# MingXiangL/AttentionShift

Measured on AMD Instinct MI355X. Metric: images/sec (1024^2, ViT-B) hot path: backbone attention fwd + attention-shift pseudo-labels, higher is better.
Workload: dtype bf16

## Files before the change

attentionshift_amd/_lib.py:

```python
import ctypes
import os

_HERE = os.path.dirname(os.path.abspath(__file__))
LIB_PATH = os.path.join(_HERE, "libattnshift_hip.so")

AS_F32, AS_BF16 = 0, 1

_c_void_p, _c_int, _c_float, _c_size_t = ctypes.c_void_p, ctypes.c_int, ctypes.c_float, ctypes.c_size_t
_c_double = ctypes.c_double

SIGNATURES = {
    "as_version": (_c_int, []),
    "as_last_error": (ctypes.c_char_p, []),
    "as_npad": (_c_int, [_c_int]),
    "as_linear_fwd": (_c_int, [_c_void_p] * 4 + [_c_int] * 5 + [_c_void_p]),
    "as_linear_small_fwd": (_c_int, [_c_void_p, _c_int, _c_void_p, _c_void_p, _c_void_p] + [_c_int] * 5 + [_c_void_p]),
    "as_linear_sk_workspace_bytes": (_c_size_t, [_c_int] * 3),
    "as_linear_sk_fwd": (_c_int, [_c_void_p] * 4 + [_c_int] * 5 + [_c_void_p, _c_size_t, _c_void_p]),
    "as_linear_gelu_fwd": (_c_int, [_c_void_p] * 5 + [_c_int] * 4 + [_c_void_p]),
    "as_linear_dgelu_fwd": (_c_int, [_c_void_p] * 4 + [_c_int] * 4 + [_c_void_p]),
    "as_deconv2x2_fwd": (_c_int, [_c_void_p] * 4 + [_c_int] * 6 + [_c_void_p]),
    "as_qkv_fwd": (_c_int, [_c_void_p] * 6 + [_c_int] * 5 + [_c_void_p]),
    "as_sdpa_fwd_workspace_bytes": (_c_size_t, [_c_int] * 4),
    "as_sdpa_fwd": (_c_int, [_c_void_p] * 6 + [_c_size_t] + [_c_int] * 4 + [_c_void_p]),
    "as_sdpa_bwd_workspace_bytes": (_c_size_t, [_c_int] * 4),
    "as_sdpa_bwd": (_c_int, [_c_void_p] * 8 + [_c_size_t] + [_c_int] * 4 + [_c_void_p]),
    "as_attn_bwd_workspace_bytes": (_c_size_t, [_c_int] * 5),
    "as_attn_bwd": (_c_int, [_c_void_p] * 15 + [_c_size_t] + [_c_int] * 5 + [_c_void_p]),
    "as_window_attn_fwd": (_c_int, [_c_void_p] * 5 + [_c_int] * 8 + [_c_void_p]),
    "as_add_layernorm_bwd_workspace_bytes": (_c_size_t, [_c_int] * 2),
    "as_add_layernorm_bwd": (_c_int, [_c_void_p] * 4 + [ctypes.c_float] + [_c_void_p] * 5 + [_c_size_t] + [_c_int] * 3 + [_c_void_p]),
    "as_add_layernorm": (_c_int, [_c_void_p] * 4 + [ctypes.c_float] + [_c_void_p] * 2 + [_c_int] * 3 + [_c_void_p]),
    "as_add_layernorm_scaled": (_c_int, [_c_void_p] * 4 + [ctypes.c_float] + [_c_void_p] * 2 + [_c_int] * 3 + [_c_void_p, _c_int, _c_void_p]),
    "as_add_layernorm_bwd_scaled": (_c_int, [_c_void_p] * 4 + [ctypes.c_float] + [_c_void_p] * 5 + [_c_size_t] + [_c_int] * 3
                                    + [_c_void_p, _c_int, _c_void_p]),
    "as_linear_splitk_workspace_bytes": (ctypes.c_size_t, [_c_int] * 3),
    "as_linear_splitk_fwd": (_c_int, [_c_void_p] * 3 + [_c_int] * 5 + [_c_void_p, ctypes.c_size_t, _c_void_p]),
    "as_linear_bwd_workspace_bytes": (ctypes.c_size_t, [_c_int] * 3),
    "as_linear_bwd": (_c_int, [_c_void_p] * 6 + [_c_int] * 5 + [_c_void_p, ctypes.c_size_t, _c_void_p]),
    "as_linear_bwd_dgelu": (_c_int, [_c_void_p] * 7 + [_c_int] * 5 + [_c_void_p, ctypes.c_size_t, _c_void_p]),
    "as_assemble_tokens": (_c_int, [_c_void_p] * 3 + [_c_int] * 5 + [_c_void_p]),
    "as_maxpool_nhwc": (_c_int, [_c_void_p] * 2 + [_c_int] * 5 + [ctypes.c_longlong, _c_void_p]),
    "as_mask_count": (_c_int, [_c_void_p] * 2 + [_c_int] * 2 + [_c_void_p]),
    "as_window_attn_bwd_workspace_bytes": (_c_size_t, [_c_int] * 5),
    "as_window_attn_bwd": (_c_int, [_c_void_p] * 8 + [_c_size_t] + [_c_int] * 8 + [_c_void_p]),
    "as_attn_fwd": (_c_int, [_c_void_p] * 12 + [_c_size_t] + [_c_int] * 5 + [_c_void_p]),
    "as_attn_mean_rows": (_c_int, [_c_void_p] * 4 + [_c_int] * 6 + [_c_void_p]),
    "as_rollout_rfrag_bytes": (_c_size_t, [_c_int] * 3),
    "as_rollout_pack": (_c_int, [_c_void_p] * 2 + [_c_int] * 4 + [_c_void_p]),
    "as_rollout_top": (_c_int, [_c_void_p] * 5 + [_c_int] * 5 + [_c_void_p]),
    "as_rollout_step_workspace_bytes": (_c_size_t, [_c_int] * 3),
    "as_rollout_step": (_c_int, [_c_void_p] * 8 + [_c_size_t] + [_c_int] * 5 + [_c_void_p]),
    "as_ccl_2d": (_c_int, [_c_void_p] * 2 + [_c_int] * 3 + [_c_void_p]),
    "as_cam_boxes_workspace_bytes": (_c_size_t, [_c_int] * 4),
    "as_cam_boxes": (_c_int, [_c_void_p] * 2 + [_c_float] * 2 + [_c_int] * 4 + [_c_void_p] * 5 + [_c_size_t, _c_void_p]),
    "as_cam_sample_masks_workspace_bytes": (_c_size_t, [_c_int] * 4),
    "as_cam_sample_masks": (_c_int, [_c_void_p] * 3 + [_c_int] * 4 + [_c_float] * 2 + [_c_void_p] * 3 + [_c_size_t, _c_void_p]),
    "as_mask_candidates_workspace_bytes": (_c_size_t, [_c_int] * 3),
    "as_mask_candidates": (_c_int, [_c_void_p] * 3 + [_c_float] * 3 + [_c_int] + [_c_void_p] * 5 + [_c_size_t]
                           + [_c_int] * 3 + [_c_void_p]),
    "as_part_select": (_c_int, [_c_void_p] * 7 + [_c_int] * 5 + [_c_void_p] * 8 + [_c_void_p]),
    "as_part_stats": (_c_int, [_c_void_p] * 3 + [_c_float] + [_c_void_p] * 4 + [_c_int] * 3 + [_c_void_p]),
    "as_filter_parts": (_c_int, [_c_void_p] * 2 + [_c_float] * 2 + [_c_void_p] + [_c_int] * 3 + [_c_void_p]),
    "as_draw_distinct": (_c_int, [_c_void_p, _c_int, _c_int] + [_c_void_p] * 5 + [_c_int] * 3 + [_c_void_p]),
    "as_mt_sample_ranks": (_c_int, [_c_void_p] * 4 + [_c_int] * 2 + [_c_void_p]),
    "as_mt_perm_ranks": (_c_int, [_c_void_p] * 4 + [_c_int] * 2 + [_c_void_p]),
    "as_small_attn_fwd": (_c_int, [_c_void_p] * 3 + [_c_int] * 5 + [_c_void_p]),
    "as_small_attn_bwd_workspace_bytes": (_c_size_t, [_c_int] * 3),
    "as_small_attn_bwd": (_c_int, [_c_void_p] * 6 + [_c_size_t] + [_c_int] * 5 + [_c_void_p]),
    "as_roi_align_fwd": (_c_int, [_c_void_p] * 3 + [_c_int] * 6 + [_c_float] + [_c_int] * 2 + [_c_void_p]),
    "as_roi_align_bwd": (_c_int, [_c_void_p] * 3 + [_c_int] * 6 + [_c_float] + [_c_int] * 2 + [_c_void_p]),
    "as_chamfer_2d_fwd": (_c_int, [_c_void_p] * 6 + [_c_int] * 3 + [_c_void_p]),
    "as_chamfer_2d_bwd": (_c_int, [_c_void_p] * 8 + [_c_int] * 3 + [_c_void_p]),
    "as_merge_plan": (_c_int, [_c_void_p] * 4 + [_c_int] * 2 + [_c_void_p]),
    "as_semantic_prestage": (_c_int, [_c_void_p, _c_float] + [_c_int] * 5 + [_c_void_p] * 4),
    "as_cosine_shift_workspace_bytes": (_c_size_t, [_c_int] * 6),
    "as_cosine_shift": (_c_int, [_c_void_p] * 5 + [_c_double] * 2 + [_c_int] + [_c_void_p] * 4 + [_c_size_t]
                        + [_c_int] * 6 + [_c_void_p]),
    "as_cosine_shift_strided": (_c_int, [_c_void_p, ctypes.c_longlong] + [_c_void_p] * 4 + [_c_double] * 2 + [_c_int] + [_c_void_p] * 4
                                + [_c_size_t] + [_c_int] * 6 + [_c_void_p]),
    "as_refine_similarity_workspace_bytes": (_c_size_t, [_c_int] * 3),
    "as_refine_similarity": (_c_int, [_c_void_p] * 3 + [_c_int] * 3 + [_c_float, _c_int] + [_c_void_p] * 3
                             + [_c_size_t] + [_c_int] * 3 + [_c_void_p]),
    "as_instance_maps_workspace_bytes": (_c_size_t, [_c_int] * 2),
    "as_crop_threshold_erode_workspace_bytes": (_c_size_t, [_c_int] * 3),
    "as_crop_threshold_erode": (_c_int, [_c_void_p] * 2 + [_c_float, _c_int, _c_int] + [_c_void_p] * 3 + [_c_size_t]
                                + [_c_int] * 3 + [_c_void_p]),
    "as_rank_select_workspace_bytes": (_c_size_t, [_c_int] * 2),
    "as_rank_select": (_c_int, [_c_void_p] * 4 + [_c_size_t] + [_c_int] * 3 + [_c_void_p]),
    "as_rank_select_xy": (_c_int, [_c_void_p] * 4 + [_c_size_t] + [_c_int] * 5 + [_c_void_p]),
    "as_merge_parts": (_c_int, [_c_void_p] * 2 + [_c_float] + [_c_void_p] * 3 + [_c_int] * 4 + [_c_void_p]),
    "as_select_median_boxes": (_c_int, [_c_void_p] * 2 + [_c_int] * 2 + [_c_void_p] * 8 + [_c_int, _c_void_p]),
    "as_rank_draw_xy": (_c_int, [_c_void_p, _c_int] + [_c_void_p] * 4 + [_c_int, _c_int, ctypes.c_int64, _c_int, _c_void_p, _c_size_t]
                        + [_c_int] * 5 + [_c_void_p]),
    "as_instance_maps": (_c_int, [_c_void_p] * 2 + [_c_int] * 6 + [_c_void_p] * 3 + [_c_size_t, _c_void_p]),
    "as_nms_workspace_bytes": (_c_size_t, [_c_int]),
    "as_nms": (_c_int, [_c_void_p, _c_int, _c_float, _c_int] + [_c_void_p] * 3 + [_c_size_t, _c_void_p]),
    "as_paste_masks": (_c_int, [_c_void_p] * 4 + [_c_int] * 8 + [_c_float, _c_void_p]),
    "as_rle_tile": (_c_int, [_c_void_p] * 2),
    "as_rle_workspace_bytes": (_c_size_t, [_c_int] * 3),
    "as_rle_count": (_c_int, [_c_void_p] + [_c_int] * 3 + [_c_void_p] * 2 + [_c_size_t, _c_void_p]),
    "as_rle_encode": (_c_int, [_c_void_p] + [_c_int] * 3 + [_c_void_p] * 2 + [_c_size_t, _c_void_p, _c_size_t, _c_void_p, _c_size_t,
                               _c_void_p, _c_void_p]),
    "as_rpn_candidates_workspace_bytes": (_c_size_t, [_c_int] * 2),
    "as_rpn_candidates": (_c_int, [_c_void_p] + [_c_int] * 3 + [_c_void_p] * 2 + [_c_int, _c_float, _c_void_p, _c_float, _c_int]
                          + [_c_void_p] * 7 + [_c_size_t, _c_void_p]),
    "as_rpn_assign_workspace_bytes": (_c_size_t, [_c_int] * 3),
    "as_rpn_assign": (_c_int, [_c_void_p] + [_c_int] * 3 + [_c_void_p] * 3 + [_c_int] * 2 + [_c_void_p] + [_c_float] * 3
                      + [_c_int] * 2 + [_c_void_p] * 4 + [_c_size_t, _c_void_p]),
    "as_rpn_sample": (_c_int, [_c_int] * 4 + [_c_void_p] * 4 + [_c_size_t, _c_void_p, _c_void_p]),
    "as_rpn_targets": (_c_int, [_c_void_p] + [_c_int] * 3 + [_c_void_p] * 3 + [_c_int] + [_c_void_p] * 2 + [_c_int] * 2
                       + [_c_void_p] * 3 + [_c_void_p]),
}


class RpnLevel(ctypes.Structure):
    _fields_ = [("cls", _c_void_p), ("reg", _c_void_p), ("H", _c_int), ("W", _c_int), ("stride_x", _c_int), ("stride_y", _c_int)]

_lib = None


class AttnShiftError(RuntimeError):
    pass


def load():
    global _lib
    if _lib is not None:
        return _lib
    if not os.path.exists(LIB_PATH):
        raise AttnShiftError(
            f"{LIB_PATH} is missing: build it with `python -m attentionshift_amd.csrc.build` "
            "(hipcc --offload-arch=gfx950).  There is no CPU fallback for the hot path.")
    lib = ctypes.CDLL(LIB_PATH)
    for name, (res, args) in SIGNATURES.items():
        fn = getattr(lib, name)
        fn.restype, fn.argtypes = res, args
    _lib = lib
    return lib


def check(rc, what):
    if rc != 0:
        msg = load().as_last_error()
        raise AttnShiftError(f"{what} failed (rc={rc}): {msg.decode() if msg else ''}")
```

attentionshift_amd/backbone.py:

```python
import math
import os

import torch
import torch.nn as nn
import torch.nn.functional as F

from . import ops
from .registry import BACKBONES


def trunc_normal_(tensor, std=0.02):
    return nn.init.trunc_normal_(tensor, std=std, a=-2 * std, b=2 * std)


class Mlp(nn.Module):
    def __init__(self, dim, hidden):
        super().__init__()
        self.fc1 = nn.Linear(dim, hidden)
        self.fc2 = nn.Linear(hidden, dim)


class Attention(nn.Module):
    def __init__(self, dim, num_heads, qkv_bias):
        super().__init__()
        self.num_heads = num_heads
        self.qkv = nn.Linear(dim, dim * 3, bias=qkv_bias)
        self.proj = nn.Linear(dim, dim)


class Block(nn.Module):

    def __init__(self, dim, num_heads, mlp_ratio, qkv_bias, eps):
        super().__init__()
        self.norm1 = nn.LayerNorm(dim, eps=eps)
        self.attn = Attention(dim, num_heads, qkv_bias)
        self.norm2 = nn.LayerNorm(dim, eps=eps)
        self.mlp = Mlp(dim, int(dim * mlp_ratio))


class PatchEmbed(nn.Module):
    def __init__(self, img_size, patch_size, in_chans, embed_dim):
        super().__init__()
        if isinstance(img_size, int):
            img_size = [img_size, img_size]
        self.num_patches = (img_size[0] // patch_size) * (img_size[1] // patch_size)
        self.patch_size = patch_size
        self.proj = nn.Conv2d(in_chans, embed_dim, kernel_size=patch_size, stride=patch_size)


class MLP(nn.Module):

    def __init__(self, input_dim, hidden_dim, output_dim, num_layers):
        super().__init__()
        self.num_layers = num_layers
        h = [hidden_dim] * (num_layers - 1)
        self.layers = nn.ModuleList(nn.Linear(n, k) for n, k in zip([input_dim] + h, h + [output_dim]))

    def forward(self, x):
        for i, layer in enumerate(self.layers):
            x = F.relu(layer(x)) if i < self.num_layers - 1 else layer(x)
        return x


class DeferredFPN:

    def __init__(self, backbone, features, taps):
        self._bb, self._features, self._taps = backbone, list(features), list(taps)
        self._out, self._event, self._joined = None, None, False

    def launch(self):
        if self._out is not None:
            return self
        bb = self._bb
        main = torch.cuda.current_stream()
        if bb._fpn_stream is None:
            bb._fpn_stream = torch.cuda.Stream()
        side = bb._fpn_stream
        side.wait_stream(main)
        with torch.cuda.stream(side):
            for t in self._features + self._taps:
                t.record_stream(side)
            self._out = tuple(bb._fpn(i, self._features[i], self._taps[i]) for i in range(len(self._features)))
            self._event = side.record_event()
        return self

    def result(self):
        self.launch()
        if not self._joined:
            main = torch.cuda.current_stream()
            main.wait_event(self._event)
            for t in self._out:
                t.record_stream(main)
            self._joined = True
            self._features, self._taps = [], []
        return self._out

    def __len__(self):
        return len(self._features) if self._out is None else len(self._out)

    def __iter__(self):
        return iter(self.result())

    def __getitem__(self, i):
        return self.result()[i]


@BACKBONES.register_module()
class VisionTransformerDet(nn.Module):
    def __init__(self, img_size, patch_size, embed_dim, in_chans=3, with_fpn=True, frozen_stages=-1,
                 out_indices=(3, 5, 7, 11), use_checkpoint=False, learnable_pos_embed=True, last_feat=False,
                 recompute_last_feat=False, point_tokens_num=100, num_classes=20, return_attention=False,
                 with_point_head=True, depth=12, num_heads=12, mlp_ratio=4., qkv_bias=False, qk_scale=None,
                 drop_rate=0., attn_drop_rate=0., drop_path_rate=0., norm_eps=1e-6, init_values=0,
                 compute_dtype=torch.bfloat16, **unused):
        super().__init__()
        assert not with_fpn or patch_size in (8, 16)
        assert not recompute_last_feat or last_feat
        if qk_scale is not None or attn_drop_rate or drop_rate or init_values:
            raise NotImplementedError("qk_scale / dropout / layer-scale are unused by every reference config")
        if embed_dim != num_heads * ops.HEAD_DIM:
            raise NotImplementedError(f"head dim must be {ops.HEAD_DIM}")
        self.embed_dim = self.num_features = embed_dim
        self.patch_size, self.depth, self.num_heads = patch_size, depth, num_heads
        self.last_feat, self.recompute_last_feat = last_feat, recompute_last_feat
        self.with_fpn, self.frozen_stages = with_fpn, frozen_stages
        self.out_indices = tuple(out_indices)
        self.use_checkpoint = use_checkpoint
        self.drop_path_rate = drop_path_rate
        self.return_attention = return_attention
        self.point_tokens_num = point_tokens_num
        self.with_point_head = with_point_head
        self.compute_dtype = compute_dtype
        self.defer_fpn = bool(unused.pop("defer_fpn", False))
        self._fpn_stream = None
        self._point_pack = None
        self.point_head_stream = bool(unused.pop("point_head_stream", False))
        self._point_stream = None

        self.patch_embed = PatchEmbed(img_size, patch_size, in_chans, embed_dim)
        n_patches = self.patch_embed.num_patches
        self.cls_token = nn.Parameter(torch.zeros(1, 1, embed_dim))
        self.pos_embed = nn.Parameter(torch.zeros(1, n_patches + 1, embed_dim), requires_grad=learnable_pos_embed)
        self.blocks = nn.ModuleList(Block(embed_dim, num_heads, mlp_ratio, qkv_bias, norm_eps) for _ in range(depth))
        if with_fpn and patch_size == 16:
            self.fpn1 = nn.Sequential(nn.ConvTranspose2d(embed_dim, embed_dim, 2, 2), nn.BatchNorm2d(embed_dim), nn.GELU(),
                                      nn.ConvTranspose2d(embed_dim, embed_dim, 2, 2))
            self.fpn2 = nn.Sequential(nn.ConvTranspose2d(embed_dim, embed_dim, 2, 2))
            self.fpn3 = nn.Identity()
            self.fpn4 = nn.MaxPool2d(2, 2)
        elif with_fpn and patch_size == 8:
            self.fpn1 = nn.Sequential(nn.ConvTranspose2d(embed_dim, embed_dim, 2, 2))
            self.fpn2 = nn.Identity()
            self.fpn3 = nn.Sequential(nn.MaxPool2d(2, 2))
            self.fpn4 = nn.Sequential(nn.MaxPool2d(4, 4))
        self.point_token = nn.Parameter(torch.zeros(1, point_tokens_num, embed_dim))
        self.point_pos_embed = nn.Parameter(torch.zeros(1, point_tokens_num, embed_dim))
        if with_point_head:
            self.class_embed = MLP(embed_dim, embed_dim, num_classes, 3)
            self.bbox_embed = MLP(embed_dim, embed_dim, 2, 3)
        trunc_normal_(self.pos_embed)
        trunc_normal_(self.cls_token)
        trunc_normal_(self.point_token)
        trunc_normal_(self.point_pos_embed)
        self.apply(self._init_weights)
        self._wcache = {}

    @staticmethod
    def _init_weights(m):
        if isinstance(m, nn.Linear):
            trunc_normal_(m.weight)
            if m.bias is not None:
                nn.init.constant_(m.bias, 0)
        elif isinstance(m, nn.LayerNorm):
            nn.init.constant_(m.bias, 0)
            nn.init.constant_(m.weight, 1.0)

    def init_weights(self, pretrained=None):
        if pretrained is not None and not isinstance(pretrained, str):
            raise TypeError("pretrained must be a str or None")
        self.apply(self._init_weights)
        if isinstance(pretrained, str):
            import os
            if os.path.isfile(pretrained):
                from .checkpoint import load_checkpoint
                load_checkpoint(self, pretrained, strict=False)
            else:
                print(f"checkpoint path {pretrained} is invalid, we skip it and initialize net randomly")
        self.invalidate_cache()

    def train(self, mode=True):
        super().train(mode)
        self._freeze_stages()
        return self

    def _freeze_stages(self):
        if self.frozen_stages >= 0:
            self.patch_embed.eval()
            for p in self.patch_embed.parameters():
                p.requires_grad = False
            self.cls_token.requires_grad = False
            self.pos_embed.requires_grad = False
        for i in range(1, self.frozen_stages + 1):
            m = self.blocks[i - 1]
            m.eval()
            for p in m.parameters():
                p.requires_grad = False

    def invalidate_cache(self):
        self._wcache = {}

    def _w(self, p):
        if p.dtype == self.compute_dtype:
            return p
        if torch.is_grad_enabled() and p.requires_grad:
            return p.to(self.compute_dtype)
        key = id(p)
        hit = self._wcache.get(key)
        if hit is None or hit[0] != p._version or hit[1].device != p.device:
            hit = (p._version, p.detach().to(self.compute_dtype).contiguous())
            self._wcache[key] = hit
        return hit[1]

    def _derived(self, p, tag, fn):
        if torch.is_grad_enabled() and p.requires_grad:
            return fn(p).to(self.compute_dtype).contiguous()
        key = (id(p), tag)
        hit = self._wcache.get(key)
        if hit is None or hit[0] != p._version or hit[1].device != p.device:
            hit = (p._version, fn(p.detach()).to(self.compute_dtype).contiguous())
            self._wcache[key] = hit
        return hit[1]

    def _deconv2x2(self, x_nhwc, conv, bn=None, act="none"):
        B, h, w, cin = x_nhwc.shape
        cout = conv.weight.shape[1]
        srcs = [conv.weight, conv.bias] + ([bn.weight, bn.bias, bn.running_mean, bn.running_var] if bn is not None else [])
        stamp = tuple(-1 if t is None else t._version for t in srcs) + (x_nhwc.device,)
        key = (id(conv), "deconv")
        hit = self._wcache.get(key)
        if hit is None or hit[0] != stamp:
            with torch.no_grad():
                wmat = conv.weight.detach().float().permute(2, 3, 1, 0).reshape(4 * cout, cin)
                bias = torch.zeros(cout, device=wmat.device) if conv.bias is None else conv.bias.detach().float()
                if bn is not None:
                    scale = bn.weight.detach().float() * torch.rsqrt(bn.running_var.float() + bn.eps)
                    wmat = wmat * scale.repeat(4)[:, None]
                    bias = (bias - bn.running_mean.float()) * scale + bn.bias.detach().float()
                hit = (stamp, wmat.to(self.compute_dtype).contiguous(), bias.repeat(4).contiguous())
            self._wcache[key] = hit
        _, wmat, bias4 = hit
        if x_nhwc.is_cuda and self.compute_dtype == torch.bfloat16 and cin % 32 == 0 and cout % 8 == 0:
            return ops.deconv2x2(x_nhwc.contiguous(), wmat, bias4, act=act)
        y = ops.linear(x_nhwc.reshape(B * h * w, cin), wmat, bias4, act=act)
        return y.reshape(B, h, w, 2, 2, cout).permute(0, 1, 3, 2, 4, 5).reshape(B, 2 * h, 2 * w, cout)

    def _deconv2x2_train(self, x_nhwc, conv):
        B, h, w, cin = x_nhwc.shape
        cout = conv.weight.shape[1]
        cd = self.compute_dtype
        from .autograd import linear_in
        wmat = conv.weight.permute(2, 3, 1, 0).reshape(4 * cout, cin)
        bias = None if conv.bias is None else conv.bias.repeat(4)
        y = linear_in(x_nhwc.reshape(B * h * w, cin), wmat, bias, cd)
        return y.reshape(B, h, w, 2, 2, cout).permute(0, 1, 3, 2, 4, 5).reshape(B, 2 * h, 2 * w, cout)

    def _fpn_train(self, i, feat_nchw, tok):
        B, D, hp, wp = feat_nchw.shape
        op = [self.fpn1, self.fpn2, self.fpn3, self.fpn4][i]
        if isinstance(op, nn.Sequential) and isinstance(op[0], nn.ConvTranspose2d):
            y = self._deconv2x2_train(tok.to(self.compute_dtype).reshape(B, hp, wp, D), op[0]).permute(0, 3, 1, 2)
            if len(op) == 4:
                y = op[2](op[1](y.float())).to(self.compute_dtype)
                y = self._deconv2x2_train(y.permute(0, 2, 3, 1), op[3]).permute(0, 3, 1, 2)
            return y
        return op(feat_nchw)

    def _fpn(self, i, feat_nchw, tok):
        B, D, hp, wp = feat_nchw.shape
        ops_ = [self.fpn1, self.fpn2, self.fpn3, self.fpn4]
        op = ops_[i]
        if isinstance(op, nn.Sequential) and isinstance(op[0], nn.ConvTranspose2d):
            x0 = tok.to(self.compute_dtype).reshape(B, hp, wp, D)
            if len(op) == 4:
                bn = op[1]
                if isinstance(bn, nn.modules.batchnorm._BatchNorm) and not bn.training and bn.running_mean is not None \
                        and isinstance(op[2], nn.GELU) and getattr(op[2], "approximate", "none") == "none":
                    y = self._deconv2x2(x0, op[0], bn=bn, act="gelu")
                else:
                    y = self._deconv2x2(x0, op[0]).permute(0, 3, 1, 2)
                    y = op[2](op[1](y.float())).to(self.compute_dtype).permute(0, 2, 3, 1)
                return self._deconv2x2(y, op[3]).permute(0, 3, 1, 2)
            return self._deconv2x2(x0, op[0]).permute(0, 3, 1, 2)
        pool = op[0] if isinstance(op, nn.Sequential) and len(op) == 1 else op
        if isinstance(pool, nn.MaxPool2d) and tok.is_cuda and tok.dtype == torch.float32 and tok.stride()[1:] == (D, 1):
            k = pool.kernel_size if isinstance(pool.kernel_size, int) else pool.kernel_size[0]
            s_ = pool.stride if isinstance(pool.stride, int) else pool.stride[0]
            if k == s_ and pool.padding in (0, (0, 0)) and not pool.ceil_mode and hp % k == 0 and wp % k == 0 and D % 4 == 0:
                return ops.maxpool_nhwc(tok.reshape(B, hp, wp, D), k).permute(0, 3, 1, 2)
        return op(feat_nchw)

    def _point_head_packable(self, x):
        ls = list(self.class_embed.layers) + list(self.bbox_embed.layers)
        return (len(self.class_embed.layers) == 3 and len(self.bbox_embed.layers) == 3 and hasattr(torch, "_addmm_activation")
                and all(l.weight.dtype == x.dtype and l.bias is not None for l in ls)
                and self.class_embed.layers[0].in_features == self.bbox_embed.layers[0].in_features)

    def _point_head_packed(self, x):
        c, b = self.class_embed.layers, self.bbox_embed.layers
        key = tuple((t.data_ptr(), t._version) for t in (c[0].weight, c[0].bias, b[0].weight, b[0].bias))
        pk = self._point_pack
        if pk is None or pk["key"] != key:
            with torch.no_grad():
                w1 = torch.cat((c[0].weight, b[0].weight)).contiguous()
                pk = dict(key=key, w1=w1, w1t=w1.t().contiguous(), b1=torch.cat((c[0].bias, b[0].bias)))
            self._point_pack = pk
        B, T, D = x.shape
        hc = c[0].out_features
        x2 = x.reshape(B * T, D)
        if ops.linear_small_applies(x2, pk["w1"]) and hc % 16 == 0 and hc >= 64:
            h1 = ops.linear_small(x2, pk["w1"], pk["b1"], act="relu")
            h2c = ops.linear_small(h1[:, :hc], c[1].weight, c[1].bias, act="relu")
            h2b = ops.linear_small(h1[:, hc:], b[1].weight, b[1].bias, act="relu")
            cls = ops.linear_small(h2c, c[2].weight, c[2].bias).reshape(B, T, -1)
            reg = ops.linear_small(h2b, b[2].weight, b[2].bias, act="sigmoid").reshape(B, T, -1)
            return cls, reg
        h1 = torch._addmm_activation(pk["b1"], x2, pk["w1t"])
        h2c = torch._addmm_activation(c[1].bias, h1[:, :hc], c[1].weight.t())
        h2b = torch._addmm_activation(b[1].bias, h1[:, hc:], b[1].weight.t())
        cls = torch.addmm(c[2].bias, h2c, c[2].weight.t()).reshape(B, T, -1)
        reg = torch.addmm(b[2].bias, h2b, b[2].weight.t()).reshape(B, T, -1).sigmoid()
        return cls, reg

    def interpolate_pos_encoding(self, n_patch_tokens, w, h):
        n0 = self.pos_embed.shape[1] - 1
        if n_patch_tokens == n0 and w == h:
            return self.pos_embed
        dim = self.pos_embed.shape[-1]
        w0, h0 = w // self.patch_size + 0.1, h // self.patch_size + 0.1
        s = int(math.sqrt(n0))
        grid = self.pos_embed[:, 1:].reshape(1, s, s, dim).permute(0, 3, 1, 2)
        grid = F.interpolate(grid, scale_factor=(w0 / math.sqrt(n0), h0 / math.sqrt(n0)), mode="bicubic")
        assert int(w0) == grid.shape[-2] and int(h0) == grid.shape[-1]
        return torch.cat((self.pos_embed[:, :1], grid.permute(0, 2, 3, 1).reshape(1, -1, dim)), dim=1)

    def prepare_tokens(self, img):
        B, C, w, h = img.shape
        ps = self.patch_size
        hp, wp = w // ps, h // ps
        patches = torch.empty(B, hp, wp, C, ps, ps, device=img.device, dtype=self.compute_dtype)
        patches.copy_(img.reshape(B, C, hp, ps, wp, ps).permute(0, 2, 4, 1, 3, 5))
        wmat = self._derived(self.patch_embed.proj.weight, "patch", lambda t: t.reshape(self.embed_dim, -1))
        emb = ops.linear(patches.view(B, hp * wp, C * ps * ps), wmat, self.patch_embed.proj.bias.float())
        return ops.assemble_tokens(emb, self._token_table(hp * wp, w, h))

    def _token_table(self, Np, w, h):
        srcs = (self.pos_embed, self.cls_token, self.point_token, self.point_pos_embed)
        stamp = tuple(t._version for t in srcs) + (Np, w, h, self.pos_embed.device)
        hit = self._wcache.get("token_table")
        if hit is None or hit[0] != stamp:
            with torch.no_grad():
                pos = self.interpolate_pos_encoding(Np, w, h)
                table = torch.cat((self.cls_token + pos[:, :1], pos[:, 1:], self.point_token + self.point_pos_embed), dim=1)
            hit = (stamp, table[0].float().contiguous())
            self._wcache["token_table"] = hit
        return hit[1]

    def _block(self, blk, x, delta, keep_state, need_x, on_full=None, full_out=None, x_out=None):
        cd = self.compute_dtype
        x, y = ops.add_layernorm(x, delta, blk.norm1.weight, blk.norm1.bias, blk.norm1.eps, cd,
                                 x_out=full_out if delta is not None else None)
        if on_full is not None:
            on_full(x)
        a, st = ops.attention_fwd(y, self._w(blk.attn.qkv.weight),
                                  None if blk.attn.qkv.bias is None else blk.attn.qkv.bias.float(),
                                  self._w(blk.attn.proj.weight), blk.attn.proj.bias.float(), self.num_heads,
                                  keep_state=keep_state)
        x, z = ops.add_layernorm(x, a, blk.norm2.weight, blk.norm2.bias, blk.norm2.eps, cd)
        z = ops.linear(z, self._w(blk.mlp.fc1.weight), blk.mlp.fc1.bias.float(), act="gelu")
        z = ops.linear(z, self._w(blk.mlp.fc2.weight), blk.mlp.fc2.bias.float())
        if need_x:
            x, _ = ops.add_layernorm(x, z, None, None, 0.0, cd, want_y=False, x_out=x_out)
            z = None
        return x, z, st

    def _grad_path(self):
        return torch.is_grad_enabled() and self.training and any(p.requires_grad for p in self.blocks.parameters())

    def _drop_path(self, x, i):
        rate = self.drop_path_rate * i / max(self.depth - 1, 1)
        if rate == 0.0 or not self.training:
            return x
        keep = 1.0 - rate
        mask = torch.rand(x.shape[0], 1, 1, device=x.device, dtype=x.dtype).add_(keep).floor_()
        return x / keep * mask

    def _drop_scale(self, batch, i, device):
        rate = self.drop_path_rate * i / max(self.depth - 1, 1)
        if rate == 0.0 or not self.training:
            return None
        keep = 1.0 - rate
        return torch.rand(batch, device=device, dtype=torch.float32).add_(keep).floor_().div_(keep)

    def _prepare_tokens_train(self, img):
        B, C, w, h = img.shape
        ps = self.patch_size
        hp, wp = w // ps, h // ps
        cd = self.compute_dtype
        patches = img.reshape(B, C, hp, ps, wp, ps).permute(0, 2, 4, 1, 3, 5).reshape(B, hp * wp, C * ps * ps)
        from .autograd import linear_in
        x = linear_in(patches.to(cd), self.patch_embed.proj.weight.reshape(self.embed_dim, -1), self.patch_embed.proj.bias,
                      cd).float()
        x = torch.cat((self.cls_token.expand(B, -1, -1), x), dim=1)
        x = x + self.interpolate_pos_encoding(x.shape[1] - 1, w, h)
        pt = (self.point_token + self.point_pos_embed).expand(B, -1, -1)
        return torch.cat((x, pt), dim=1)

    def _block_train(self, blk, x, delta, i, sink, delta_scale=None):
        from . import autograd as AG
        cd = self.compute_dtype
        sh = self._train_shadow
        w = lambda p: sh[id(p)] if id(p) in sh else p.to(cd)
        x, y = AG.add_layernorm(x, delta, blk.norm1.weight, blk.norm1.bias, blk.norm1.eps, cd, delta_scale)
        a = AG.attention(y, w(blk.attn.qkv.weight), None if blk.attn.qkv.bias is None else blk.attn.qkv.bias.float(),
                         w(blk.attn.proj.weight), blk.attn.proj.bias.float(), self.num_heads, sink)
        x, z = AG.add_layernorm(x, a, blk.norm2.weight, blk.norm2.bias, blk.norm2.eps, cd, self._drop_scale(x.shape[0], i, x.device))
        if AG.mlp_applies(z, w(blk.mlp.fc1.weight), w(blk.mlp.fc2.weight)):
            z = AG.mlp(z, w(blk.mlp.fc1.weight), blk.mlp.fc1.bias, w(blk.mlp.fc2.weight), blk.mlp.fc2.bias)
        elif AG.linear_applies(z, w(blk.mlp.fc1.weight)):
            z = F.gelu(AG.linear(z, w(blk.mlp.fc1.weight), blk.mlp.fc1.bias))
            z = AG.linear(z, w(blk.mlp.fc2.weight), blk.mlp.fc2.bias)
        else:
            z = F.gelu(F.linear(z, w(blk.mlp.fc1.weight), w(blk.mlp.fc1.bias)))
            z = F.linear(z, w(blk.mlp.fc2.weight), w(blk.mlp.fc2.bias))
        return x, z, self._drop_scale(x.shape[0], i, x.device)

    def forward(self, x):
        B, _, H, W = x.shape
        hp, wp = H // self.patch_size, W // self.patch_size
        T = self.point_tokens_num
        grad_path = self._grad_path()
        x = self._prepare_tokens_train(x) if grad_path else self.prepare_tokens(x)
        if self.recompute_last_feat:
            last_feat = x
        features, taps, attns = [], [], []
        store = []
        delta = None
        dscale = None
        if not grad_path:
            x = x.contiguous()

        def take_tap(xf):
            taps.append(xf[:, 1:-T])
            tap = xf[:, 1:, :][:, :-T].permute(0, 2, 1).unflatten(2, (hp, wp))
            if grad_path:
                features.append(tap if os.environ.get("AS_TAP_VIEW", "1") != "0" else tap.contiguous())
                return
            if xf.data_ptr() != tap_slot(len(features)).data_ptr():
                tap_slot(len(features)).copy_(xf)
            features.append(store[0][len(features)][:, 1:-T].unflatten(1, (hp, wp)).permute(0, 3, 1, 2))

        def tap_slot(k):
            if not store:
                store.append(torch.empty(len(self.out_indices), *x.shape, device=x.device, dtype=torch.float32))
            return store[0][k]

        tap_due = False
        nblk = len(self.blocks)
        self._train_shadow = {}
        if grad_path and self.compute_dtype != torch.float32 and not os.environ.get("AS_NO_PARAM_SHADOW"):
            from .autograd import cast_params
            from . import autograd as _AG
            lib_mlp = _AG._LIBRARY_LINEAR or self.embed_dim % 32 != 0
            ps = []
            for blk in self.blocks:
                ps += [blk.attn.qkv.weight, blk.attn.proj.weight, blk.mlp.fc1.weight, blk.mlp.fc2.weight]
                if lib_mlp:
                    ps += [blk.mlp.fc1.bias, blk.mlp.fc2.bias]
            self._train_shadow = cast_params([p for p in ps if p.dtype != self.compute_dtype], self.compute_dtype)
        for i, blk in enumerate(self.blocks):
            if grad_path:
                sink = [] if self.return_attention else None
                x, delta, dscale = self._block_train(blk, x.float() if x.dtype != torch.float32 else x, delta, i, sink, dscale)
                if i in self.out_indices or i == nblk - 1:
                    x = x + (delta if dscale is None else delta * dscale[:, None, None])
                    delta, dscale = None, None
                st = sink[0] if sink else None
                if i in self.out_indices:
                    take_tap(x)
            else:
                last_tap = i in self.out_indices and i == nblk - 1
                x, delta, st = self._block(blk, x, delta, self.return_attention, i == nblk - 1,
                                           take_tap if tap_due else None,
                                           full_out=tap_slot(len(features)) if tap_due and x.dtype == torch.float32 else None,
                                           x_out=tap_slot(len(features) + int(tap_due)) if last_tap and x.dtype == torch.float32
                                           else None)
                tap_due = i in self.out_indices and i != nblk - 1
                if i in self.out_indices and i == nblk - 1:
                    take_tap(x)
            if self.return_attention:
                attns.append(st)
            if self.last_feat and not self.recompute_last_feat and i == nblk - 1:
                last_feat = x[:, :-T]
        self._train_shadow = {}
        org_features = store[0][:, :, 1:-T].unflatten(2, (hp, wp)).permute(1, 0, 4, 2, 3) if store else None
        if org_features is None:
            org_features = torch.stack(features, dim=1)
        if self.with_fpn and grad_path:
            features = [self._fpn_train(i, features[i], taps[i]) for i in range(len(features))]
        elif self.with_fpn and self.defer_fpn and x.is_cuda:
            features = DeferredFPN(self, features, taps)
        elif self.with_fpn:
            features = [self._fpn(i, features[i], taps[i]) for i in range(len(features))]
        point_tokens = x[:, -T:]
        out = dict(org_feats=org_features, feature=features if isinstance(features, DeferredFPN) else tuple(features),
                   point_tokens=point_tokens)
        if self.with_point_head and not grad_path and point_tokens.is_cuda and self._point_head_packable(point_tokens):
            if self.point_head_stream:
                if self._point_stream is None:
                    self._point_stream = torch.cuda.Stream()
                main = torch.cuda.current_stream()
                self._point_stream.wait_stream(main)
                with torch.cuda.stream(self._point_stream):
                    cls, reg = self._point_head_packed(point_tokens)
                    out["point_head_ready"] = self._point_stream.record_event()
                for t in (point_tokens, cls, reg):
                    t.record_stream(main)
                    t.record_stream(self._point_stream)
            else:
                cls, reg = self._point_head_packed(point_tokens)
            out.update(outputs_class=cls, outputs_coord=reg)
        elif self.with_point_head:
            out.update(outputs_class=self.class_embed(point_tokens), outputs_coord=self.bbox_embed(point_tokens).sigmoid())
        if self.return_attention and self.last_feat:
            out.update(attns=attns)
        if self.last_feat:
            out.update(last_feat=last_feat)
        return out
```

attentionshift_amd/csrc/layernorm.hip:

```cpp
#include "common.h"

namespace {

template <typename T, int VPL>
__global__ __launch_bounds__(256) void add_layernorm_kernel(const float* __restrict__ x_in, const T* __restrict__ delta,
                                                            const float* __restrict__ gamma, const float* __restrict__ beta,
                                                            float* __restrict__ x_out, T* __restrict__ y_out, int M, int D,
                                                            float eps, const float* __restrict__ dscale, int rps) {
  const int row = blockIdx.x * 4 + (threadIdx.x >> 6), lane = threadIdx.x & 63;
  if (row >= M) return;
  const size_t base = (size_t)row * D;
  const float ds = dscale != nullptr ? dscale[row / rps] : 1.0f;
  float v[VPL][4];
  float s = 0.0f;
#pragma unroll
  for (int i = 0; i < VPL; ++i) {
    const int c = (i * 64 + lane) * 4;
    if (c < D) {
      const float4 a = *reinterpret_cast<const float4*>(x_in + base + c);
      v[i][0] = a.x; v[i][1] = a.y; v[i][2] = a.z; v[i][3] = a.w;
      if (delta != nullptr) {
#pragma unroll
        for (int t = 0; t < 4; ++t) v[i][t] = dscale != nullptr ? fmaf(ds, to_f32<T>(delta[base + c + t]), v[i][t])
                                                                     : v[i][t] + to_f32<T>(delta[base + c + t]);
      }
      s += (v[i][0] + v[i][1]) + (v[i][2] + v[i][3]);
    } else {
      v[i][0] = v[i][1] = v[i][2] = v[i][3] = 0.0f;
    }
  }
  const float mean = wave_sum(s) / (float)D;
  float q = 0.0f;
#pragma unroll
  for (int i = 0; i < VPL; ++i) {
    const int c = (i * 64 + lane) * 4;
    if (c < D) {
#pragma unroll
      for (int t = 0; t < 4; ++t) {
        const float d = v[i][t] - mean;
        q = fmaf(d, d, q);
      }
    }
  }
  const float rstd = rsqrtf(wave_sum(q) / (float)D + eps);
#pragma unroll
  for (int i = 0; i < VPL; ++i) {
    const int c = (i * 64 + lane) * 4;
    if (c < D) {
      if (x_out != nullptr) *reinterpret_cast<float4*>(x_out + base + c) = make_float4(v[i][0], v[i][1], v[i][2], v[i][3]);
      if (y_out != nullptr) {
        const float4 g = *reinterpret_cast<const float4*>(gamma + c);
        const float4 b = *reinterpret_cast<const float4*>(beta + c);
        const float y0 = (v[i][0] - mean) * rstd * g.x + b.x, y1 = (v[i][1] - mean) * rstd * g.y + b.y;
        const float y2 = (v[i][2] - mean) * rstd * g.z + b.z, y3 = (v[i][3] - mean) * rstd * g.w + b.w;
        T* yp = y_out + base + c;
        yp[0] = from_f32<T>(y0); yp[1] = from_f32<T>(y1); yp[2] = from_f32<T>(y2); yp[3] = from_f32<T>(y3);
      }
    }
  }
}

template <typename T>
int launch_add_ln(const float* x_in, const void* delta, const float* gamma, const float* beta, float* x_out, void* y_out,
                  int M, int D, float eps, const float* dscale, int rps, hipStream_t s) {
  const int vpl = as_ceil_div(D, 256);
  dim3 grid(as_ceil_div(M, 4));
#define AS_LN(V)                                                                                                   \
  hipLaunchKernelGGL((add_layernorm_kernel<T, V>), grid, dim3(256), 0, s, x_in, (const T*)delta, gamma, beta, x_out, \
                     (T*)y_out, M, D, eps, dscale, rps)
  switch (vpl) {
    case 1: AS_LN(1); break;
    case 2: AS_LN(2); break;
    case 3: AS_LN(3); break;
    case 4: AS_LN(4); break;
    case 5: AS_LN(5); break;
    case 6: AS_LN(6); break;
    case 7: AS_LN(7); break;
    case 8: AS_LN(8); break;
    case 9: case 10: AS_LN(10); break;
    case 11: case 12: AS_LN(12); break;
    default: AS_REQUIRE(false, AS_E_UNSUPPORTED, "as_add_layernorm: D=%d (max 3072)", D);
  }
#undef AS_LN
  AS_CHECK_LAUNCH("add_layernorm");
  return AS_OK;
}

}

namespace {

template <typename T, int VPL>
__global__ __launch_bounds__(256) void add_layernorm_bwd_kernel(const float* __restrict__ x, const T* __restrict__ dy,
                                                                const float* __restrict__ dx_res,
                                                                const float* __restrict__ gamma, float* __restrict__ dx_out,
                                                                T* __restrict__ ddelta_out, float* __restrict__ part, int M,
                                                                int D, float eps, const float* __restrict__ dscale, int rps) {
  __shared__ float red[2][4][VPL * 256];
  const int wave = threadIdx.x >> 6, lane = threadIdx.x & 63;
  float dg[VPL][4], db[VPL][4], gm[VPL][4];
#pragma unroll
  for (int i = 0; i < VPL; ++i) {
    const int c = (i * 64 + lane) * 4;
#pragma unroll
    for (int t = 0; t < 4; ++t) { dg[i][t] = 0.0f; db[i][t] = 0.0f; gm[i][t] = (gamma != nullptr && c < D) ? gamma[c + t] : 1.0f; }
  }
  for (int row = blockIdx.x * 4 + wave; row < M; row += gridDim.x * 4) {
    const size_t base = (size_t)row * D;
    float v[VPL][4], g[VPL][4];
    float s = 0.0f;
#pragma unroll
    for (int i = 0; i < VPL; ++i) {
      const int c = (i * 64 + lane) * 4;
      if (c < D) {
        const float4 a = *reinterpret_cast<const float4*>(x + base + c);
        v[i][0] = a.x; v[i][1] = a.y; v[i][2] = a.z; v[i][3] = a.w;
        if (dy == nullptr) {
#pragma unroll
          for (int t = 0; t < 4; ++t) g[i][t] = 0.0f;
        } else if constexpr (sizeof(T) == 2) {
          const bf16x4 d4 = *reinterpret_cast<const bf16x4*>(dy + base + c);
#pragma unroll
          for (int t = 0; t < 4; ++t) g[i][t] = (float)d4[t];
        } else {
          const float4 d4 = *reinterpret_cast<const float4*>(dy + base + c);
          g[i][0] = d4.x; g[i][1] = d4.y; g[i][2] = d4.z; g[i][3] = d4.w;
        }
        s += (v[i][0] + v[i][1]) + (v[i][2] + v[i][3]);
      } else {
#pragma unroll
        for (int t = 0; t < 4; ++t) { v[i][t] = 0.0f; g[i][t] = 0.0f; }
      }
    }
    const float mean = wave_sum(s) / (float)D;
    float q = 0.0f;
#pragma unroll
    for (int i = 0; i < VPL; ++i) {
      const int c = (i * 64 + lane) * 4;
      if (c < D) {
#pragma unroll
        for (int t = 0; t < 4; ++t) { const float d = v[i][t] - mean; q = fmaf(d, d, q); }
      }
    }
    const float rstd = rsqrtf(wave_sum(q) / (float)D + eps);
    float sg = 0.0f, sgx = 0.0f;
#pragma unroll
    for (int i = 0; i < VPL; ++i) {
      const int c = (i * 64 + lane) * 4;
      if (c < D) {
#pragma unroll
        for (int t = 0; t < 4; ++t) {
          const float xh = (v[i][t] - mean) * rstd;
          dg[i][t] = fmaf(g[i][t], xh, dg[i][t]);
          db[i][t] += g[i][t];
          const float gg = g[i][t] * gm[i][t];
          g[i][t] = gg;
          v[i][t] = xh;
          sg += gg;
          sgx = fmaf(gg, xh, sgx);
        }
      }
    }
    const float mg = wave_sum(sg) / (float)D, mgx = wave_sum(sgx) / (float)D;
#pragma unroll
    for (int i = 0; i < VPL; ++i) {
      const int c = (i * 64 + lane) * 4;
      if (c < D) {
        float o[4];
        float4 r4 = make_float4(0.0f, 0.0f, 0.0f, 0.0f);
        if (dx_res != nullptr) r4 = *reinterpret_cast<const float4*>(dx_res + base + c);
        const float r[4] = {r4.x, r4.y, r4.z, r4.w};
#pragma unroll
        for (int t = 0; t < 4; ++t) {
          o[t] = rstd * (g[i][t] - mg - v[i][t] * mgx);
          if (dx_res != nullptr) o[t] += r[t];
        }
        if (dx_out != nullptr) *reinterpret_cast<float4*>(dx_out + base + c) = make_float4(o[0], o[1], o[2], o[3]);
        if (ddelta_out != nullptr) {
          const float ds = dscale != nullptr ? dscale[row / rps] : 1.0f;
          if constexpr (sizeof(T) == 2) {
            bf16x4 w4;
#pragma unroll
            for (int t = 0; t < 4; ++t) w4[t] = (__bf16)(ds * o[t]);
            *reinterpret_cast<bf16x4*>(ddelta_out + base + c) = w4;
          } else {
            *reinterpret_cast<float4*>(ddelta_out + base + c) = make_float4(ds * o[0], ds * o[1], ds * o[2], ds * o[3]);
          }
        }
      }
    }
  }
#pragma unroll
  for (int i = 0; i < VPL; ++i)
#pragma unroll
    for (int t = 0; t < 4; ++t) {
      red[0][wave][(i * 64 + lane) * 4 + t] = dg[i][t];
      red[1][wave][(i * 64 + lane) * 4 + t] = db[i][t];
    }
  __syncthreads();
  for (int c = threadIdx.x; c < D; c += 256) {
    part[((size_t)blockIdx.x * 2 + 0) * D + c] = ((red[0][0][c] + red[0][1][c]) + red[0][2][c]) + red[0][3][c];
    part[((size_t)blockIdx.x * 2 + 1) * D + c] = ((red[1][0][c] + red[1][1][c]) + red[1][2][c]) + red[1][3][c];
  }
}

__global__ __launch_bounds__(1024) void add_layernorm_bwd_reduce_kernel(const float* __restrict__ part,
                                                                        float* __restrict__ dgamma, float* __restrict__ dbeta,
                                                                        int nblk, int D) {
  __shared__ float red[16][64];
  const int cl = threadIdx.x & 63, grp = threadIdx.x >> 6, c = blockIdx.x * 64 + cl, which = blockIdx.y;
  float a0 = 0.0f, a1 = 0.0f, a2 = 0.0f, a3 = 0.0f;
  if (c < D) {
    int i = grp;
    for (; i + 48 < nblk; i += 64) {
      a0 += part[((size_t)i * 2 + which) * D + c];
      a1 += part[((size_t)(i + 16) * 2 + which) * D + c];
      a2 += part[((size_t)(i + 32) * 2 + which) * D + c];
      a3 += part[((size_t)(i + 48) * 2 + which) * D + c];
    }
    for (; i < nblk; i += 16) a0 += part[((size_t)i * 2 + which) * D + c];
  }
  red[grp][cl] = (a0 + a1) + (a2 + a3);
  __syncthreads();
  if (grp != 0 || c >= D) return;
  float t = 0.0f;
#pragma unroll
  for (int g = 0; g < 16; ++g) t += red[g][cl];
  float* dst = which == 0 ? dgamma : dbeta;
  if (dst != nullptr) dst[c] = t;
}

constexpr int LNB_BLOCKS = 1024;

template <typename T>
int launch_add_ln_bwd(const float* x, const void* dy, const float* dx_res, const float* gamma, float* dx_out, void* ddelta,
                      float* dgamma, float* dbeta, float* part, int M, int D, float eps, const float* dscale, int rps,
                      hipStream_t s) {
  const int vpl = as_ceil_div(D, 256);
  const int nblk = as_ceil_div(M, 4) < LNB_BLOCKS ? as_ceil_div(M, 4) : LNB_BLOCKS;
#define AS_LNB(V)                                                                                                    \
  hipLaunchKernelGGL((add_layernorm_bwd_kernel<T, V>), dim3(nblk), dim3(256), 0, s, x, (const T*)dy, dx_res, gamma, dx_out, \
                     (T*)ddelta, part, M, D, eps, dscale, rps)
  switch (vpl) {
    case 1: AS_LNB(1); break;
    case 2: AS_LNB(2); break;
    case 3: AS_LNB(3); break;
    case 4: AS_LNB(4); break;
    case 5: AS_LNB(5); break;
    case 6: AS_LNB(6); break;
    case 7: AS_LNB(7); break;
    case 8: AS_LNB(8); break;
    default: AS_REQUIRE(false, AS_E_UNSUPPORTED, "as_add_layernorm_bwd: D=%d (max 2048)", D);
  }
#undef AS_LNB
  AS_CHECK_LAUNCH("add_layernorm_bwd");
  if (dgamma != nullptr || dbeta != nullptr) {
    hipLaunchKernelGGL(add_layernorm_bwd_reduce_kernel, dim3(as_ceil_div(D, 64), 2), dim3(1024), 0, s, (const float*)part,
                       dgamma, dbeta, nblk, D);
    AS_CHECK_LAUNCH("add_layernorm_bwd_reduce");
  }
  return AS_OK;
}

}

extern "C" size_t as_add_layernorm_bwd_workspace_bytes(int M, int D) {
  if (M <= 0 || D <= 0) return 0;
  return (size_t)LNB_BLOCKS * 2 * D * sizeof(float);
}

extern "C" int as_add_layernorm_bwd(const float* x, const void* dy, const float* dx_res, const float* gamma, float eps,
                                    float* dx_out, void* ddelta_out, float* dgamma, float* dbeta, void* workspace,
                                    size_t workspace_bytes, int M, int D, int dtype, as_stream_t stream) {
  return as_add_layernorm_bwd_scaled(x, dy, dx_res, gamma, eps, dx_out, ddelta_out, dgamma, dbeta, workspace, workspace_bytes,
                                     M, D, dtype, nullptr, 1, stream);
}

extern "C" int as_add_layernorm_bwd_scaled(const float* x, const void* dy, const float* dx_res, const float* gamma, float eps,
                                           float* dx_out, void* ddelta_out, float* dgamma, float* dbeta, void* workspace,
                                           size_t workspace_bytes, int M, int D, int dtype, const float* delta_scale,
                                           int rows_per_scale, as_stream_t stream) {
  AS_REQUIRE(x && (dy || dx_res) && (dx_out || ddelta_out) && workspace, AS_E_BADARG, "as_add_layernorm_bwd: null pointer");
  AS_REQUIRE(rows_per_scale > 0, AS_E_BADARG, "as_add_layernorm_bwd: rows_per_scale must be positive");
  AS_REQUIRE(M > 0 && D > 0 && D % 4 == 0, AS_E_BADARG, "as_add_layernorm_bwd: need M > 0 and D %% 4 == 0 (D=%d)", D);
  AS_REQUIRE(workspace_bytes >= as_add_layernorm_bwd_workspace_bytes(M, D), AS_E_WORKSPACE,
             "as_add_layernorm_bwd: workspace too small");
  hipStream_t s = (hipStream_t)stream;
  if (dtype == AS_BF16)
    return launch_add_ln_bwd<__bf16>(x, dy, dx_res, gamma, dx_out, ddelta_out, dgamma, dbeta, (float*)workspace, M, D, eps,
                                     delta_scale, rows_per_scale, s);
  if (dtype == AS_F32)
    return launch_add_ln_bwd<float>(x, dy, dx_res, gamma, dx_out, ddelta_out, dgamma, dbeta, (float*)workspace, M, D, eps,
                                    delta_scale, rows_per_scale, s);
  AS_REQUIRE(false, AS_E_UNSUPPORTED, "as_add_layernorm_bwd: dtype %d", dtype);
}

extern "C" int as_add_layernorm(const float* x_in, const void* delta, const float* gamma, const float* beta, float eps,
                                float* x_out, void* y_out, int M, int D, int dtype, as_stream_t stream) {
  return as_add_layernorm_scaled(x_in, delta, gamma, beta, eps, x_out, y_out, M, D, dtype, nullptr, 1, stream);
}

extern "C" int as_add_layernorm_scaled(const float* x_in, const void* delta, const float* gamma, const float* beta, float eps,
                                       float* x_out, void* y_out, int M, int D, int dtype, const float* delta_scale,
                                       int rows_per_scale, as_stream_t stream) {
  AS_REQUIRE(x_in && (x_out || y_out), AS_E_BADARG, "as_add_layernorm: null pointer");
  AS_REQUIRE(rows_per_scale > 0 && (!delta_scale || delta), AS_E_BADARG, "as_add_layernorm: delta_scale needs delta, rows_per_scale > 0");
  AS_REQUIRE(!y_out || (gamma && beta), AS_E_BADARG, "as_add_layernorm: y_out needs gamma and beta");
  AS_REQUIRE(M > 0 && D > 0 && D % 4 == 0, AS_E_BADARG, "as_add_layernorm: need M > 0 and D %% 4 == 0 (D=%d)", D);
  hipStream_t s = (hipStream_t)stream;
  if (dtype == AS_BF16) return launch_add_ln<__bf16>(x_in, delta, gamma, beta, x_out, y_out, M, D, eps, delta_scale, rows_per_scale, s);
  if (dtype == AS_F32) return launch_add_ln<float>(x_in, delta, gamma, beta, x_out, y_out, M, D, eps, delta_scale, rows_per_scale, s);
  AS_REQUIRE(false, AS_E_UNSUPPORTED, "as_add_layernorm: dtype %d", dtype);
}


namespace {
__global__ __launch_bounds__(256) void maxpool_nhwc_kernel(const float* __restrict__ x, float* __restrict__ out, int B, int H,
                                                           int W, int C, int k, size_t xbs) {
  const int Ho = H / k, Wo = W / k, C4 = C >> 2;
  const size_t total = (size_t)B * Ho * Wo * C4;
  for (size_t i = (size_t)blockIdx.x * blockDim.x + threadIdx.x; i < total; i += (size_t)gridDim.x * blockDim.x) {
    const int c4 = (int)(i % C4);
    size_t r = i / C4;
    const int ow = (int)(r % Wo);
    r /= Wo;
    const int oh = (int)(r % Ho), b = (int)(r / Ho);
    const float* src = x + (size_t)b * xbs + (((size_t)oh * k) * W + (size_t)ow * k) * C + c4 * 4;
    float4 m = *reinterpret_cast<const float4*>(src);
    for (int dy = 0; dy < k; ++dy)
      for (int dx = 0; dx < k; ++dx) {
        const float4 v = *reinterpret_cast<const float4*>(src + ((size_t)dy * W + dx) * C);
        m.x = (v.x > m.x || v.x != v.x) ? v.x : m.x; m.y = (v.y > m.y || v.y != v.y) ? v.y : m.y;
        m.z = (v.z > m.z || v.z != v.z) ? v.z : m.z; m.w = (v.w > m.w || v.w != v.w) ? v.w : m.w;
      }
    *reinterpret_cast<float4*>(out + i * 4) = m;
  }
}
}

extern "C" int as_maxpool_nhwc(const float* x, float* out, int B, int H, int W, int C, int k, long long x_batch_stride,
                               as_stream_t stream) {
  AS_REQUIRE(x && out, AS_E_BADARG, "as_maxpool_nhwc: null pointer");
  AS_REQUIRE(B > 0 && H > 0 && W > 0 && C > 0 && k > 0, AS_E_BADARG, "as_maxpool_nhwc: bad sizes");
  AS_REQUIRE(x_batch_stride >= (long long)H * W * C && x_batch_stride % 4 == 0, AS_E_BADARG,
             "as_maxpool_nhwc: batch stride %lld (elements) must be >= H*W*C and a multiple of 4", x_batch_stride);
  AS_REQUIRE(C % 4 == 0 && H % k == 0 && W % k == 0, AS_E_UNSUPPORTED,
             "as_maxpool_nhwc: C %% 4 == 0 and H, W multiples of k only (C=%d H=%d W=%d k=%d)", C, H, W, k);
  const size_t total = (size_t)B * (H / k) * (W / k) * (C / 4);
  const int grid = (int)((total + 255) / 256 < 4096 ? (total + 255) / 256 : 4096);
  hipLaunchKernelGGL(maxpool_nhwc_kernel, dim3(grid), dim3(256), 0, (hipStream_t)stream, x, out, B, H, W, C, k,
                     (size_t)x_batch_stride);
  AS_CHECK_LAUNCH("maxpool_nhwc");
  return AS_OK;
}

namespace {
template <typename T>
__global__ __launch_bounds__(256) void assemble_tokens_kernel(const T* __restrict__ emb, const float* __restrict__ table,
                                                              float* __restrict__ out, int B, int Np, int N, int D) {
  const int D4 = D >> 2;
  const size_t total = (size_t)B * N * D4;
  for (size_t i = (size_t)blockIdx.x * blockDim.x + threadIdx.x; i < total; i += (size_t)gridDim.x * blockDim.x) {
    const int c = (int)(i % D4) * 4;
    const size_t r = i / D4;
    const int n = (int)(r % N), b = (int)(r / N);
    float4 v = *reinterpret_cast<const float4*>(table + (size_t)n * D + c);
    if (n >= 1 && n <= Np) {
      const T* e = emb + ((size_t)b * Np + (n - 1)) * D + c;
      if (sizeof(T) == 2) {
        const bf16x4 e4 = *reinterpret_cast<const bf16x4*>(e);
        v.x = (float)e4[0] + v.x; v.y = (float)e4[1] + v.y; v.z = (float)e4[2] + v.z; v.w = (float)e4[3] + v.w;
      } else {
        const float4 e4 = *reinterpret_cast<const float4*>(e);
        v.x = e4.x + v.x; v.y = e4.y + v.y; v.z = e4.z + v.z; v.w = e4.w + v.w;
      }
    }
    *reinterpret_cast<float4*>(out + i * 4) = v;
  }
}
}

extern "C" int as_assemble_tokens(const void* emb, const float* table, float* out, int B, int Np, int N, int D, int dtype,
                                  as_stream_t stream) {
  AS_REQUIRE(emb && table && out, AS_E_BADARG, "as_assemble_tokens: null pointer");
  AS_REQUIRE(B > 0 && Np > 0 && N > Np && D > 0 && D % 4 == 0, AS_E_BADARG, "as_assemble_tokens: B=%d Np=%d N=%d D=%d", B, Np, N, D);
  const size_t total = (size_t)B * N * (D / 4);
  const int grid = (int)((total + 255) / 256 < 8192 ? (total + 255) / 256 : 8192);
  if (dtype == AS_BF16)
    hipLaunchKernelGGL(assemble_tokens_kernel<__bf16>, dim3(grid), dim3(256), 0, (hipStream_t)stream, (const __bf16*)emb, table, out,
                       B, Np, N, D);
  else if (dtype == AS_F32)
    hipLaunchKernelGGL(assemble_tokens_kernel<float>, dim3(grid), dim3(256), 0, (hipStream_t)stream, (const float*)emb, table, out,
                       B, Np, N, D);
  else
    AS_REQUIRE(false, AS_E_UNSUPPORTED, "as_assemble_tokens: dtype %d", dtype);
  AS_CHECK_LAUNCH("assemble_tokens");
  return AS_OK;
}
```

attentionshift_amd/csrc/linear_small.hip:

```cpp
#include "common.h"

namespace {

constexpr int LS_BM = 32, LS_BN = 64, LS_NT = 256;

template <int ACT> __device__ __forceinline__ float ls_act(float v) {
  if constexpr (ACT == 1) return 0.5f * v * (1.0f + erff(v * 0.70710678118654752440f));
  else if constexpr (ACT == 4) return fmaxf(v, 0.0f);
  else if constexpr (ACT == 5) return 1.0f / (1.0f + expf(-v));
  else return v;
}

template <int ACT>
__global__ __launch_bounds__(LS_NT) void linear_small_kernel(const float* __restrict__ x, int ldx, const float* __restrict__ W,
                                                             const float* __restrict__ bias, float* __restrict__ out, int ldo,
                                                             int M, int Nout, int K) {
  __shared__ float part[4][LS_BM][LS_BN + 1];
  const int tid = threadIdx.x, lane = tid & 63, wave = tid >> 6;
  const int li = lane & 31, half = lane >> 5;
  const int m0 = blockIdx.x * LS_BM, n0 = blockIdx.y * LS_BN;
  const int steps = K / 16, per = steps / 4;
  const int s_beg = wave * per, s_end = wave == 3 ? steps : s_beg + per;
  const float* pa = x + (size_t)min(m0 + li, M - 1) * ldx + 8 * half;
  const float* pb0 = W + (size_t)min(n0 + li, Nout - 1) * K + 8 * half;
  const float* pb1 = W + (size_t)min(n0 + 32 + li, Nout - 1) * K + 8 * half;
  f32x16 acc0, acc1;
#pragma unroll
  for (int r = 0; r < 16; ++r) { acc0[r] = 0.0f; acc1[r] = 0.0f; }
#pragma unroll 2
  for (int s = s_beg; s < s_end; ++s) {
    Frag<float> fa, fb0, fb1;
    fa.load16B(pa + 16 * s);
    fb0.load16B(pb0 + 16 * s);
    fb1.load16B(pb1 + 16 * s);
    acc0 = mma32(fa, fb0, acc0);
    acc1 = mma32(fa, fb1, acc1);
  }
#pragma unroll
  for (int r = 0; r < 16; ++r) {
    part[wave][acc_row(r, half)][li] = acc0[r];
    part[wave][acc_row(r, half)][32 + li] = acc1[r];
  }
  __syncthreads();
  const int row = tid >> 3, c0 = (tid & 7) * 8;
  if (m0 + row >= M) return;
#pragma unroll
  for (int c = 0; c < 8; ++c) {
    const int col = n0 + c0 + c;
    if (col >= Nout) break;
    float v = ((part[0][row][c0 + c] + part[1][row][c0 + c]) + part[2][row][c0 + c]) + part[3][row][c0 + c];
    if (bias != nullptr) v += bias[col];
    out[(size_t)(m0 + row) * ldo + col] = ls_act<ACT>(v);
  }
}

}

extern "C" int as_linear_small_fwd(const float* x, int ldx, const float* W, const float* bias, float* out, int ldo, int M, int Nout,
                                   int K, int act, as_stream_t stream) {
  AS_REQUIRE(x && W && out, AS_E_BADARG, "as_linear_small_fwd: null pointer");
  AS_REQUIRE(M > 0 && Nout > 0 && K >= 64 && K % 16 == 0 && ldx >= K && ldo >= Nout && ldx % 4 == 0, AS_E_BADARG,
             "as_linear_small_fwd: need M, Nout > 0, K %% 16 == 0, K >= 64, ldx >= K (ldx %% 4 == 0), ldo >= Nout (M=%d N=%d K=%d ldx=%d ldo=%d)",
             M, Nout, K, ldx, ldo);
  AS_REQUIRE(act == 0 || act == 1 || act == 4 || act == 5, AS_E_BADARG, "as_linear_small_fwd: act must be 0, 1 (GELU), 4 (ReLU) or 5 (sigmoid)");
  AS_REQUIRE(((size_t)x % 16 == 0) && ((size_t)W % 16 == 0) && K % 4 == 0, AS_E_BADARG, "as_linear_small_fwd: operands must be 16-byte aligned");
  const dim3 grid(as_ceil_div(M, LS_BM), as_ceil_div(Nout, LS_BN));
  hipStream_t s = (hipStream_t)stream;
  switch (act) {
    case 1: hipLaunchKernelGGL(linear_small_kernel<1>, grid, dim3(LS_NT), 0, s, x, ldx, W, bias, out, ldo, M, Nout, K); break;
    case 4: hipLaunchKernelGGL(linear_small_kernel<4>, grid, dim3(LS_NT), 0, s, x, ldx, W, bias, out, ldo, M, Nout, K); break;
    case 5: hipLaunchKernelGGL(linear_small_kernel<5>, grid, dim3(LS_NT), 0, s, x, ldx, W, bias, out, ldo, M, Nout, K); break;
    default: hipLaunchKernelGGL(linear_small_kernel<0>, grid, dim3(LS_NT), 0, s, x, ldx, W, bias, out, ldo, M, Nout, K); break;
  }
  AS_CHECK_LAUNCH("linear_small");
  return AS_OK;
}
```

attentionshift_amd/csrc/rollout.hip:

```cpp
#include <stdlib.h>
#include "common.h"
#include "lds_asm.h"
#include "launch.h"

namespace {

constexpr int HD = 64, RO_NT = 256;
constexpr float LOG2E = 1.44269504088896340736f;

template <typename T> struct KjCfg { static constexpr int PITCH = HD * (int)sizeof(T) + 16; };

__device__ __forceinline__ size_t rf_slot(int b, int nkb, int i, int k) {
  const int rem = k & 31, s2 = rem >> 4, r16 = rem & 15;
  const int lane = (i & 31) + 32 * ((r16 & 7) >> 2), t = (r16 >> 3) * 4 + (r16 & 3);
  return ((((((size_t)b * nkb + (k >> 5)) * 4 + (i >> 5)) * 2 + s2) * 64) + lane) * 8 + t;
}
__device__ __forceinline__ size_t rf_frag(int b, int nkb, int kb, int ib, int s2, int lane) {
  return ((((((size_t)b * nkb + kb) * 4 + ib) * 2 + s2) * 64) + lane) * 8;
}

template <typename T>
__device__ __forceinline__ f32x16 pbar_tile(const T* __restrict__ q, const T* __restrict__ k,
                                            const float* __restrict__ lse, const char* kj_lds, int b, int h,
                                            int N, int Npad, int i0, int j0, int li, int half) {
  f32x16 pbar;
#pragma unroll
  for (int r = 0; r < 16; ++r) pbar[r] = 0.0f;
  const int irow = min(i0 + li, N - 1);
  const int jrow = min(j0 + li, N - 1);
  for (int hh = 0; hh < h; ++hh) {
    const size_t bh = (size_t)b * h + hh;
    f32x16 s;
#pragma unroll
    for (int r = 0; r < 16; ++r) s[r] = 0.0f;
#pragma unroll
    for (int ks = 0; ks < 4; ++ks) {
      Frag<T> fa, fb;
      fa.load16B(q + qf_frag(bh, Npad, irow, ks, half));
      if (kj_lds != nullptr)
        fb.load16B(reinterpret_cast<const T*>(kj_lds + ((size_t)hh * 32 + li) * KjCfg<T>::PITCH) + ks * 16 + half * 8);
      else
        fb.load16B(k + (bh * Npad + jrow) * HD + ks * 16 + half * 8);
      s = mma32(fa, fb, s);
    }
    const float* lrow = lse + bh * N;
#pragma unroll
    for (int r = 0; r < 16; ++r) {
      const int row = min(i0 + acc_row(r, half), N - 1);
      pbar[r] += __builtin_amdgcn_exp2f(s[r] - lrow[row] * LOG2E);
    }
  }
  const float inv_h = 1.0f / (float)h;
#pragma unroll
  for (int r = 0; r < 16; ++r) pbar[r] *= inv_h;
  return pbar;
}

template <typename T, bool TOP>
__global__ __launch_bounds__(RO_NT) void attn_mean_rows_kernel(const T* __restrict__ q, const T* __restrict__ k,
                                                               const float* __restrict__ lse,
                                                               float* __restrict__ out, T* __restrict__ rf_out, int B,
                                                               int N, int Npad, int h, int row0, int nrows) {
  const int lane = threadIdx.x & 63, wave = threadIdx.x >> 6;
  const int li = lane & 31, half = lane >> 5;
  const int jb = blockIdx.x * 4 + wave, ib = blockIdx.y, b = blockIdx.z;
  const int j0 = jb * 32, i0 = ib * 32;
  if (j0 >= N) return;
  const f32x16 p = pbar_tile<T>(q, k, lse, nullptr, b, h, N, Npad, row0 + i0, j0, li, half);
  const int j = j0 + li;
  const int nkb = (N + 31) / 32;
#pragma unroll
  for (int r = 0; r < 16; ++r) {
    const int i = i0 + acc_row(r, half);
    float v = p[r];
    if (TOP) v = 0.5f * (v + ((row0 + i) == j ? 1.0f : 0.0f));
    const bool live = i < nrows && j < N;
    if (live) out[((size_t)b * nrows + i) * N + j] = v;
    if (rf_out != nullptr && i < 128) rf_out[rf_slot(b, nkb, i, j)] = from_f32<T>(live ? v : 0.0f);
  }
}

template <typename T> struct Kj2 {
  static constexpr int PITCH = sizeof(T) == 2 ? 128 : (HD * 4 + 16);
  __device__ static __forceinline__ int off(int row, int elem) {
    if (sizeof(T) == 2) return row * 128 + ((((elem >> 3) ^ (row & 7))) << 4);
    return row * PITCH + elem * 4;
  }
};

template <typename T, int HPW>
__global__ __launch_bounds__(RO_NT) void rollout_step2_kernel(const T* __restrict__ q, const T* __restrict__ k,
                                                              const float* __restrict__ lse,
                                                              const float* __restrict__ Rin, const T* __restrict__ rf_in,
                                                              float* __restrict__ Rout, T* __restrict__ rf_out,
                                                              float* __restrict__ part, int B, int N, int Npad, int h,
                                                              int Trows, int nsplit, int xbufs) {
  extern __shared__ __attribute__((aligned(16))) char smem[];
  constexpr bool PREFETCH = sizeof(T) == 2;
  const int tid = threadIdx.x, lane = tid & 63, wave = tid >> 6;
  const int li = lane & 31, half = lane >> 5;
  const int j0 = blockIdx.x * 32, b = blockIdx.y, split = blockIdx.z;
  char* kj = smem;
  float4* xchg = reinterpret_cast<float4*>(smem + (size_t)h * 32 * Kj2<T>::PITCH);

  {
    constexpr int CPR = HD * (int)sizeof(T) / 16;
    const int total = h * 32 * CPR;
    for (int c = tid; c < total; c += RO_NT) {
      const int hh = c / (32 * CPR), rem = c % (32 * CPR);
      const int jr = rem / CPR, ch = rem % CPR;
      const int jrow = min(j0 + jr, N - 1);
      const uint4 u = *reinterpret_cast<const uint4*>(
          reinterpret_cast<const char*>(k + (((size_t)b * h + hh) * Npad + jrow) * HD) + ch * 16);
      const int elem = ch * (16 / (int)sizeof(T));
      const int base = Kj2<T>::off(hh * 32 + jr, elem & ~7);
      *reinterpret_cast<uint4*>(kj + base + (elem & 7) * (int)sizeof(T)) = u;
    }
  }
  __syncthreads();

  const int nkb = (N + 31) / 32;
  const float inv_h = 1.0f / (float)h;
  const bool own_rows = wave * 32 < Trows;

  f32x16 acc;
#pragma unroll
  for (int r = 0; r < 16; ++r) acc[r] = 0.0f;

  struct Fetch {
    Frag<T> fq[HPW][4];
    float l8[HPW];
    Frag<T> fr[2];
  };
  auto fetch = [&](int kb, Fetch& f) {
    const int row = min(kb * 32 + li, N - 1);
#pragma unroll
    for (int t = 0; t < HPW; ++t) {
      const int hh = min(wave + 4 * t, h - 1);
#pragma unroll
      for (int ks = 0; ks < 4; ++ks) f.fq[t][ks].load16B(q + qf_frag((size_t)b * h + hh, Npad, row, ks, half));
      f.l8[t] = -LOG2E * lse[((size_t)b * h + hh) * N + row];
    }
    if (own_rows) {
#pragma unroll
      for (int s2 = 0; s2 < 2; ++s2) f.fr[s2].load16B(rf_in + rf_frag(b, nkb, kb, wave, s2, lane));
    }
  };
  const int kb0 = (int)((long long)nkb * split / nsplit), kb1 = (int)((long long)nkb * (split + 1) / nsplit);
  Fetch cur, nxt;
  if (PREFETCH && kb0 < kb1) fetch(kb0, nxt);

  for (int kb = kb0; kb < kb1; ++kb) {
    const int k0 = kb * 32;
    if (PREFETCH) {
      cur = nxt;
      if (kb + 1 < kb1) fetch(kb + 1, nxt);
    } else {
      fetch(kb, cur);
    }

    f32x16 pbar;
#pragma unroll
    for (int r = 0; r < 16; ++r) pbar[r] = 0.0f;
#pragma unroll
    for (int t = 0; t < HPW; ++t) {
      const int hh = wave + 4 * t;
      if (hh < h) {
        const float l8 = cur.l8[t];
        f32x16 sc;
#pragma unroll
        for (int r = 0; r < 16; ++r) sc[r] = 0.0f;
        sc = __builtin_amdgcn_mfma_f32_32x32x2f32(half == 0 ? l8 : 0.0f, 1.0f, sc, 0, 0, 0);
#pragma unroll
        for (int ks = 0; ks < 4; ++ks) {
          Frag<T> fk;
          fk.load16B(reinterpret_cast<const T*>(kj + Kj2<T>::off(hh * 32 + li, ks * 16 + half * 8)));
          sc = mma32(cur.fq[t][ks], fk, sc);
        }
#pragma unroll
        for (int r = 0; r < 16; ++r) pbar[r] += __builtin_amdgcn_exp2f(sc[r]);
      }
    }
    float4* slab = xchg + (size_t)(xbufs == 2 ? (kb - kb0) & 1 : 0) * 4 * 4 * 64;
#pragma unroll
    for (int g = 0; g < 4; ++g)
      slab[(wave * 4 + g) * 64 + lane] = make_float4(pbar[4 * g], pbar[4 * g + 1], pbar[4 * g + 2], pbar[4 * g + 3]);
    __syncthreads();
    if (own_rows) {
      Frag<T> fp[2];
#pragma unroll
      for (int g = 0; g < 4; ++g) {
        float4 v = slab[(0 * 4 + g) * 64 + lane];
#pragma unroll
        for (int w = 1; w < 4; ++w) {
          const float4 u = slab[(w * 4 + g) * 64 + lane];
          v.x += u.x; v.y += u.y; v.z += u.z; v.w += u.w;
        }
        const float e[4] = {v.x, v.y, v.z, v.w};
#pragma unroll
        for (int x = 0; x < 4; ++x) {
          const int r = 4 * g + x;
          const bool live = k0 + acc_row(r, half) < N;
          fp[r >> 3].set(r & 7, live ? e[x] * inv_h : 0.0f);
        }
      }
#pragma unroll
      for (int s2 = 0; s2 < 2; ++s2) acc = mma32(cur.fr[s2], fp[s2], acc);
    }
    if (xbufs == 1) __syncthreads();
  }

  if (own_rows) {
    const int j = j0 + li;
#pragma unroll
    for (int r = 0; r < 16; ++r) {
      const int i = wave * 32 + acc_row(r, half);
      const bool live = i < Trows && j < N;
      if (nsplit > 1) {
        if (live) part[(((size_t)split * B + b) * Trows + i) * N + j] = acc[r];
        continue;
      }
      float v = 0.0f;
      if (live) {
        const size_t idx = ((size_t)b * Trows + i) * N + j;
        v = 0.5f * (acc[r] + Rin[idx]);
        Rout[idx] = v;
      }
      if (rf_out != nullptr) rf_out[rf_slot(b, nkb, i, j)] = from_f32<T>(v);
    }
  }
}

#ifndef AS_ROLLOUT_ABLATE
#define AS_ROLLOUT_ABLATE 0
#endif
template <typename T> __device__ __forceinline__ f32x16 inject_rows(float x, int half);
template <> __device__ __forceinline__ f32x16 inject_rows<float>(float x, int half) {
  f32x16 z;
#pragma unroll
  for (int r = 0; r < 16; ++r) z[r] = 0.0f;
  return __builtin_amdgcn_mfma_f32_32x32x2f32(half == 0 ? x : 0.0f, 1.0f, z, 0, 0, 0);
}
template <> __device__ __forceinline__ f32x16 inject_rows<__bf16>(float x, int half) {
  f32x16 z;
#pragma unroll
  for (int r = 0; r < 16; ++r) z[r] = 0.0f;
  x = half == 0 ? x : 0.0f;
  const __bf16 hi = (__bf16)x;
  const float r1 = x - (float)hi;
  const __bf16 mid = (__bf16)r1;
  const __bf16 lo = (__bf16)(r1 - (float)mid);
  const __bf16 zero = (__bf16)0.0f, one = (__bf16)1.0f;
  Frag<__bf16> fa, fb;
  fa.v = bf16x8{hi, mid, lo, zero, zero, zero, zero, zero};
  fb.v = bf16x8{one, one, one, zero, zero, zero, zero, zero};
  return mma32(fa, fb, z);
}

template <typename T>
__global__ __launch_bounds__(RO_NT, 3) void rollout_step3_kernel(const T* __restrict__ q, const T* __restrict__ k,
                                                                 const float* __restrict__ lse,
                                                                 const float* __restrict__ Rin, const T* __restrict__ rf_in,
                                                                 float* __restrict__ Rout, T* __restrict__ rf_out,
                                                                 float* __restrict__ part, int B, int N, int Npad, int h,
                                                                 int Trows, int nsplit) {
  extern __shared__ __attribute__((aligned(16))) char smem[];
  const int tid = threadIdx.x, lane = tid & 63, wave = tid >> 6;
  const int li = lane & 31, half = lane >> 5;
  const int j0 = blockIdx.x * 32, b = blockIdx.y, split = blockIdx.z;
  char* kj = smem;
  {
    constexpr int CPR = HD * (int)sizeof(T) / 16;
    const int total = h * 32 * CPR;
    for (int c = tid; c < total; c += RO_NT) {
      const int hh = c / (32 * CPR), rem = c % (32 * CPR);
      const int jr = rem / CPR, ch = rem % CPR;
      const int jrow = min(j0 + jr, N - 1);
      const uint4 u = *reinterpret_cast<const uint4*>(
          reinterpret_cast<const char*>(k + (((size_t)b * h + hh) * Npad + jrow) * HD) + ch * 16);
      const int elem = ch * (16 / (int)sizeof(T));
      const int base = Kj2<T>::off(hh * 32 + jr, elem & ~7);
      *reinterpret_cast<uint4*>(kj + base + (elem & 7) * (int)sizeof(T)) = u;
    }
  }
  __syncthreads();

  const int nkb = (N + 31) / 32;
  const int nib = (Trows + 31) / 32;
  const float inv_h = 1.0f / (float)h;
  const int kb0 = (int)((long long)nkb * split / nsplit), kb1 = (int)((long long)nkb * (split + 1) / nsplit);

  f32x16 acc[4];
#pragma unroll
  for (int ib = 0; ib < 4; ++ib)
#pragma unroll
    for (int r = 0; r < 16; ++r) acc[ib][r] = 0.0f;

  for (int kb = kb0 + wave; kb < kb1; kb += 4) {
    const int k0 = kb * 32;
    const int row = min(k0 + li, N - 1);
    Frag<T> fq[4];
    float l8;
#pragma unroll
    for (int ks = 0; ks < 4; ++ks) fq[ks].load16B(q + qf_frag((size_t)b * h, Npad, row, ks, half));
    l8 = -LOG2E * lse[((size_t)b * h) * N + row];
    f32x16 pbar;
#pragma unroll
    for (int r = 0; r < 16; ++r) pbar[r] = 0.0f;
    auto head = [&](int hh) {
      f32x16 sc = inject_rows<T>(AS_ROLLOUT_ABLATE == 3 ? 0.0f : l8, half);
#pragma unroll
      for (int ks = 0; ks < 4; ++ks) {
        Frag<T> fk;
        fk.load16B(reinterpret_cast<const T*>(kj + Kj2<T>::off(hh * 32 + li, ks * 16 + half * 8)));
        if (AS_ROLLOUT_ABLATE != 4) sc = mma32(fq[ks], fk, sc);
        else sc[ks] += (float)fk.v[0];
      }
#pragma unroll
      for (int r = 0; r < 16; ++r) pbar[r] += AS_ROLLOUT_ABLATE == 2 ? sc[r] : __builtin_amdgcn_exp2f(sc[r]);
    };
    for (int hh = 0; hh + 1 < h; ++hh) {
      Frag<T> fn[4];
#pragma unroll
      for (int ks = 0; ks < 4; ++ks) {
        if (AS_ROLLOUT_ABLATE == 1) fn[ks] = fq[ks];
        else fn[ks].load16B(q + qf_frag((size_t)b * h + hh + 1, Npad, row, ks, half));
      }
      const float l8n = AS_ROLLOUT_ABLATE == 1 ? l8 : -LOG2E * lse[((size_t)b * h + hh + 1) * N + row];
      head(hh);
#pragma unroll
      for (int ks = 0; ks < 4; ++ks) fq[ks] = fn[ks];
      l8 = l8n;
    }
    Frag<T> fr[4][2];
#pragma unroll
    for (int ib = 0; ib < 4; ++ib) {
      const int ibc = min(ib, nib - 1);
#pragma unroll
      for (int s2 = 0; s2 < 2; ++s2) fr[ib][s2].load16B(rf_in + rf_frag(b, nkb, kb, ibc, s2, lane));
    }
    head(h - 1);
    Frag<T> fp[2];
#pragma unroll
    for (int r = 0; r < 16; ++r) {
      const bool live = k0 + acc_row(r, half) < N;
      fp[r >> 3].set(r & 7, live ? pbar[r] * inv_h : 0.0f);
    }
#pragma unroll
    for (int ib = 0; ib < 4; ++ib)
      if (ib < nib) {
#pragma unroll
        for (int s2 = 0; s2 < 2; ++s2) acc[ib] = mma32(fr[ib][s2], fp[s2], acc[ib]);
      }
  }

  float* red = reinterpret_cast<float*>(smem);
  f32x16 mine;
#pragma unroll
  for (int r = 0; r < 16; ++r) mine[r] = 0.0f;
#pragma unroll
  for (int pass = 0; pass < 2; ++pass) {
    __syncthreads();
#pragma unroll
    for (int x = 0; x < 2; ++x)
#pragma unroll
      for (int r = 0; r < 16; ++r) red[((wave * 2 + x) * 16 + r) * 64 + lane] = acc[pass * 2 + x][r];
    __syncthreads();
    if ((wave >> 1) == pass) {
      const int x = wave & 1;
#pragma unroll
      for (int r = 0; r < 16; ++r)
        mine[r] = ((red[((0 * 2 + x) * 16 + r) * 64 + lane] + red[((1 * 2 + x) * 16 + r) * 64 + lane]) +
                   red[((2 * 2 + x) * 16 + r) * 64 + lane]) + red[((3 * 2 + x) * 16 + r) * 64 + lane];
    }
  }
  if (wave * 32 < Trows) {
    const int j = j0 + li;
#pragma unroll
    for (int r = 0; r < 16; ++r) {
      const int i = wave * 32 + acc_row(r, half);
      const bool live = i < Trows && j < N;
      if (nsplit > 1) {
        if (live) part[(((size_t)split * B + b) * Trows + i) * N + j] = mine[r];
        continue;
      }
      float v = 0.0f;
      if (live) {
        const size_t idx = ((size_t)b * Trows + i) * N + j;
        v = 0.5f * (mine[r] + Rin[idx]);
        Rout[idx] = v;
      }
      if (rf_out != nullptr) rf_out[rf_slot(b, nkb, i, j)] = from_f32<T>(v);
    }
  }
}

constexpr int R4_HPG = 4;
constexpr int R4_QBYTES = R4_HPG * 4 * 1024;
constexpr int R4_LSE = R4_QBYTES + 8 * 1024;
constexpr int R4_STAGE = R4_LSE + 1024;
#ifndef AS_R4_OCC1
#define AS_R4_OCC1 3
#endif
template <int NIB> struct R4Cfg { static constexpr int NSTAGE = NIB == 1 ? 2 : 3, OCC = NIB == 1 ? AS_R4_OCC1 : 2; };


template <int NIB>
__global__ __launch_bounds__(RO_NT, R4Cfg<NIB>::OCC) void rollout_step4_kernel(const __bf16* __restrict__ q, const __bf16* __restrict__ k,
                                                                 const float* __restrict__ lse, const __bf16* __restrict__ rf_in,
                                                                 float* __restrict__ part, int B, int N, int Npad, int h,
                                                                 int Trows, int ksplit) {
  extern __shared__ __attribute__((aligned(16))) char smem[];
  constexpr int R4_NSTAGE = R4Cfg<NIB>::NSTAGE;
  const int tid = threadIdx.x, lane = tid & 63, wave = __builtin_amdgcn_readfirstlane(tid >> 6);
  const int li = lane & 31, half = lane >> 5;
  const int ngroups = h / R4_HPG;
  const int j0 = blockIdx.x * 128 + wave * 32, b = blockIdx.y;
  const int hg = blockIdx.z % ngroups, split = blockIdx.z / ngroups;
  const int nkb = (N + 31) / 32;
  const int nib = min((Trows + 31) / 32, NIB);
  const int kb0 = (int)((long long)nkb * split / ksplit), kb1 = (int)((long long)nkb * (split + 1) / ksplit);
  const int nblk = kb1 - kb0;
  const size_t bh0 = (size_t)b * h + hg * R4_HPG;

  Frag<__bf16> fk[R4_HPG][4];
  {
    const int jrow = min(j0 + li, N - 1);
#pragma unroll
    for (int hh = 0; hh < R4_HPG; ++hh)
#pragma unroll
      for (int ks = 0; ks < 4; ++ks) fk[hh][ks].load16B(k + ((bh0 + hh) * Npad + jrow) * HD + ks * 16 + half * 8);
  }
  const int ibw = min(wave, nib - 1);
  const unsigned smem_u = lds_addr(smem);
  const unsigned voff = lane * 16;
  const char* q_w = reinterpret_cast<const char*>(q) + ((bh0 + wave) * (size_t)(Npad >> 5)) * 4096;
  const char* r_w = reinterpret_cast<const char*>(rf_in) + rf_frag(b, nkb, 0, ibw, 0, 0) * sizeof(__bf16);
  const char* l_w = reinterpret_cast<const char*>(lse + (bh0 + wave) * N);
  auto stage = [&](int kb, int buf) {
    const unsigned base = smem_u + buf * R4_STAGE;
    const char* qs = q_w + (size_t)kb * 4096;
#pragma unroll
    for (int ks = 0; ks < 4; ++ks) lds_dma16(voff, qs + ks * 1024, base + (wave * 4 + ks) * 1024);
    if (NIB == 4 || wave == 0) {
      const char* rs = r_w + (size_t)kb * (4 * 2 * 1024);
#pragma unroll
      for (int s2 = 0; s2 < 2; ++s2) lds_dma16(voff, rs + s2 * 1024, base + R4_QBYTES + (wave * 2 + s2) * 1024);
    }
    lds_dma4((unsigned)min(kb * 32 + li, N - 1) * 4u, l_w, base + R4_LSE + wave * 256);
  };

  f32x16 acc[NIB];
#pragma unroll
  for (int ib = 0; ib < NIB; ++ib)
#pragma unroll
    for (int r = 0; r < 16; ++r) acc[ib][r] = 0.0f;
  const float inv_h = 1.0f / (float)h;
  const unsigned lbase = lds_addr(smem) + lane * 16;

  if (nblk > 0) stage(kb0, 0);
  if (R4_NSTAGE > 2 && nblk > 1) stage(kb0 + 1, 1);

  for (int it = 0; it < nblk; ++it) {
    const int kb = kb0 + it, buf = it % R4_NSTAGE;
    if (AS_ROLLOUT_ABLATE != 11) {
      if (R4_NSTAGE == 2 || it + 1 >= nblk) asm volatile("s_waitcnt vmcnt(0)" ::: "memory");
      else if (NIB == 4 || wave == 0) asm volatile("s_waitcnt vmcnt(7)" ::: "memory");
      else asm volatile("s_waitcnt vmcnt(5)" ::: "memory");
    }
    {
      float own;
      const unsigned a_own = lds_addr(smem) + buf * R4_STAGE + R4_LSE + wave * 256 + lane * 4;
      asm volatile("ds_read_b32 %0, %1\n\ts_waitcnt lgkmcnt(0)" : "=v"(own) : "v"(a_own) : "memory");
      own *= -LOG2E;
      asm volatile("ds_write_b32 %0, %1\n\ts_waitcnt lgkmcnt(0)" :: "v"(a_own), "v"(own) : "memory");
    }
    if (AS_ROLLOUT_ABLATE != 14) __builtin_amdgcn_s_barrier();
    if (AS_ROLLOUT_ABLATE != 11 && it + R4_NSTAGE - 1 < nblk) stage(kb + R4_NSTAGE - 1, (it + R4_NSTAGE - 1) % R4_NSTAGE);
    const unsigned sb = lbase + buf * R4_STAGE;
    const unsigned cb = lds_addr(smem) + buf * R4_STAGE + R4_LSE + half * 16;
    u32x4 fc[2][4];
    auto read_c = [&](int hh, u32x4 (&c)[4]) {
      const unsigned a = cb + hh * 256;
      lds_read128(c[0], a);
      lds_read128_i<32>(c[1], a);
      lds_read128_i<64>(c[2], a);
      lds_read128_i<96>(c[3], a);
    };
    f32x16 pbar;
#pragma unroll
    for (int r = 0; r < 16; ++r) pbar[r] = 0.0f;
    u32x4 fa[2][4];
    read_c(0, fc[0]);
    lds_read128(fa[0][0], sb);
    lds_read128_i<1024>(fa[0][1], sb);
    lds_read128_i<2048>(fa[0][2], sb);
    lds_read128_i<3072>(fa[0][3], sb);
    {
      const unsigned a1 = sb + 4096;
      read_c(1, fc[1]);
      lds_read128(fa[1][0], a1);
      lds_read128_i<1024>(fa[1][1], a1);
      lds_read128_i<2048>(fa[1][2], a1);
      lds_read128_i<3072>(fa[1][3], a1);
    }
    lds_wait<8>(fa[0][0], fa[0][1], fa[0][2], fa[0][3], fc[0][0], fc[0][1], fc[0][2], fc[0][3]);
    auto qk = [&](int hh, u32x4 (&f)[4], u32x4 (&c)[4]) {
      f32x16 sc;
#pragma unroll
      for (int r = 0; r < 16; ++r) sc[r] = __uint_as_float(c[r >> 2][r & 3]);
#pragma unroll
      for (int ks = 0; ks < 4; ++ks) {
        Frag<__bf16> fq;
        fq.v = *reinterpret_cast<bf16x8*>(&f[ks]);
        if (AS_ROLLOUT_ABLATE != 13) sc = mma32(fq, fk[hh][ks], sc);
        else sc[ks] += (float)fq.v[0];
      }
      return sc;
    };
    f32x16 sc_cur = qk(0, fa[0], fc[0]);
    u32x4 fr[NIB][2];
#pragma unroll
    for (int hh = 0; hh < R4_HPG; ++hh) {
      f32x16 sc_next;
      if (hh + 1 < R4_HPG) {
        const int nx = (hh + 1) & 1;
        lds_wait<0>(fa[nx][0], fa[nx][1], fa[nx][2], fa[nx][3], fc[nx][0], fc[nx][1], fc[nx][2], fc[nx][3]);
        sc_next = qk(hh + 1, fa[nx], fc[nx]);
        if (hh + 2 < R4_HPG) {
          const unsigned a2 = sb + (hh + 2) * 4096;
          read_c(hh + 2, fc[hh & 1]);
          lds_read128(fa[hh & 1][0], a2);
          lds_read128_i<1024>(fa[hh & 1][1], a2);
          lds_read128_i<2048>(fa[hh & 1][2], a2);
          lds_read128_i<3072>(fa[hh & 1][3], a2);
        }
      } else {
#pragma unroll
        for (int ib = 0; ib < NIB; ++ib) {
          const unsigned a = sb + R4_QBYTES + min(ib, nib - 1) * 2048;
          lds_read128(fr[ib][0], a);
          lds_read128_i<1024>(fr[ib][1], a);
        }
      }
#pragma unroll
      for (int r = 0; r < 16; ++r) pbar[r] += AS_ROLLOUT_ABLATE == 12 ? sc_cur[r] : __builtin_amdgcn_exp2f(sc_cur[r]);
      if (hh + 1 < R4_HPG) sc_cur = sc_next;
    }
    Frag<__bf16> fp[2];
    if (kb * 32 + 32 <= N) {
#pragma unroll
      for (int r = 0; r < 16; ++r) fp[r >> 3].set(r & 7, pbar[r]);
    } else {
#pragma unroll
      for (int r = 0; r < 16; ++r) fp[r >> 3].set(r & 7, kb * 32 + acc_row(r, half) < N ? pbar[r] : 0.0f);
    }
    if constexpr (NIB == 1) lds_wait<0>(fr[0][0], fr[0][1]);
    else lds_wait<0>(fr[0][0], fr[0][1], fr[1][0], fr[1][1], fr[2][0], fr[2][1], fr[3][0], fr[3][1]);
#pragma unroll
    for (int s2 = 0; s2 < 2; ++s2)
#pragma unroll
      for (int ib = 0; ib < NIB; ++ib)
        if (ib < nib) {
          Frag<__bf16> f;
          f.v = *reinterpret_cast<bf16x8*>(&fr[ib][s2]);
          if (AS_ROLLOUT_ABLATE != 15) acc[ib] = mma32(f, fp[s2], acc[ib]);
          else acc[ib][0] += (float)f.v[0] + (float)fp[s2].v[0];
        }
  }

  const int pidx = split * ngroups + hg;
  const int j = j0 + li;
  if (j < N) {
#pragma unroll
    for (int ib = 0; ib < NIB; ++ib)
#pragma unroll
      for (int r = 0; r < 16; ++r) {
        const int i = ib * 32 + acc_row(r, half);
        if (i < Trows) part[(((size_t)pidx * B + b) * Trows + i) * N + j] = acc[ib][r] * inv_h;
      }
  }
}

bool rollout_force_v3() {
  static const bool v = getenv("AS_ROLLOUT_V3") != nullptr;
  return v;
}

constexpr int R4_MAXPARTS = 16;
int rollout4_ksplit(int B, int N, int h, int slots) {
  static const int forced = [] { const char* e = getenv("AS_R4_KS"); return e ? atoi(e) : 0; }();
  if (forced > 0 && forced * (h / R4_HPG) <= 16) return forced;
  const int units = as_ceil_div(N, 128) * B * (h / R4_HPG);
  int best = 1;
  float best_eff = 0.0f;
  for (int ks = 1; ks * (h / R4_HPG) <= R4_MAXPARTS && ks <= 8; ++ks) {
    const int wgs = units * ks;
    const float eff = (float)wgs / (float)(as_ceil_div(wgs, slots) * slots);
    if (eff > best_eff + 0.02f) { best_eff = eff; best = ks; }
  }
  return best;
}

template <typename T>
__global__ __launch_bounds__(64) void rollout_finish_kernel(const float* __restrict__ part, const float* __restrict__ Rin,
                                                            float* __restrict__ Rout, T* __restrict__ rf_out, int B, int N,
                                                            int Trows, int nsplit) {
  const int nkb = (N + 31) / 32;
  const int j = blockIdx.x * 64 + threadIdx.x, i = blockIdx.y, b = blockIdx.z;
  if (j >= nkb * 32) return;
  float v = 0.0f;
  if (i < Trows && j < N) {
    const size_t idx = ((size_t)b * Trows + i) * N + j;
    float a = 0.0f;
    for (int sp = 0; sp < nsplit; ++sp) a += part[(size_t)sp * B * Trows * N + idx];
    v = 0.5f * (a + Rin[idx]);
    Rout[idx] = v;
  }
  if (rf_out != nullptr) rf_out[rf_slot(b, nkb, i, j)] = from_f32<T>(v);
}

template <typename T>
int launch_rollout_step2(const void* q, const void* k, const float* lse, const float* Rin, const void* rf_in, float* Rout,
                         void* rf_out, float* part, int nsplit, int B, int N, int h, int Trows, hipStream_t s) {
  const int Npad = as_round_up(N, 64);
  const int hpw = as_ceil_div(h, 4);
  dim3 grid(as_ceil_div(N, 32), B, nsplit);
  const size_t kbytes = (size_t)h * 32 * Kj2<T>::PITCH, slab = 4 * 4 * 64 * sizeof(float4);
  const int xbufs = kbytes + 2 * slab <= 160 * 1024 ? 2 : 1;
  const size_t lds = kbytes + xbufs * slab;
  AS_REQUIRE(lds <= 160 * 1024, AS_E_UNSUPPORTED, "rollout_step: LDS %zu B exceeds 160 KiB (h=%d)", lds, h);
#define AS_RO2(HPW)                                                                                            \
  do {                                                                                                         \
    as_lds_optin<rollout_step2_kernel<T, HPW>>(lds);                                                           \
    hipLaunchKernelGGL((rollout_step2_kernel<T, HPW>), grid, dim3(RO_NT), lds, s, (const T*)q, (const T*)k, lse, Rin, \
                       (const T*)rf_in, Rout, (T*)rf_out, part, B, N, Npad, h, Trows, nsplit, xbufs);          \
  } while (0)
  if (sizeof(T) == 2 && h % R4_HPG == 0 && part != nullptr && nsplit == R4_MAXPARTS && !rollout_force_v3()) {
    const int ng = h / R4_HPG;
    const int ks = rollout4_ksplit(B, N, h, 512);
    const size_t lds4 = (size_t)(Trows <= 32 ? R4Cfg<1>::NSTAGE : R4Cfg<4>::NSTAGE) * R4_STAGE;
    if (Trows <= 32) {
      as_lds_optin<rollout_step4_kernel<1>>(lds4);
      hipLaunchKernelGGL(rollout_step4_kernel<1>, dim3(as_ceil_div(N, 128), B, ks * ng), dim3(RO_NT), lds4, s, (const __bf16*)q,
                         (const __bf16*)k, lse, (const __bf16*)rf_in, part, B, N, Npad, h, Trows, ks);
    } else {
      as_lds_optin<rollout_step4_kernel<4>>(lds4);
      hipLaunchKernelGGL(rollout_step4_kernel<4>, dim3(as_ceil_div(N, 128), B, ks * ng), dim3(RO_NT), lds4, s, (const __bf16*)q,
                         (const __bf16*)k, lse, (const __bf16*)rf_in, part, B, N, Npad, h, Trows, ks);
    }
    AS_CHECK_LAUNCH("rollout_step4");
    dim3 fg(as_ceil_div(as_ceil_div(N, 32) * 32, 64), as_round_up(Trows, 32), B);
    hipLaunchKernelGGL((rollout_finish_kernel<T>), fg, dim3(64), 0, s, (const float*)part, Rin, Rout, (T*)rf_out, B, N,
                       Trows, ks * ng);
    AS_CHECK_LAUNCH("rollout_finish");
    return AS_OK;
  }
  if (sizeof(T) == 2 && h >= 8 && (getenv("AS_ROLLOUT_V2") == nullptr)) {
    const size_t lds3 = (size_t)h * 32 * Kj2<T>::PITCH;
    as_lds_optin<rollout_step3_kernel<T>>(lds3);
    hipLaunchKernelGGL((rollout_step3_kernel<T>), grid, dim3(RO_NT), lds3, s, (const T*)q, (const T*)k, lse, Rin,
                       (const T*)rf_in, Rout, (T*)rf_out, part, B, N, Npad, h, Trows, nsplit);
  } else {
  switch (hpw) {
    case 1: AS_RO2(1); break;
    case 2: AS_RO2(2); break;
    case 3: AS_RO2(3); break;
    case 4: AS_RO2(4); break;
    default: AS_REQUIRE(false, AS_E_UNSUPPORTED, "rollout_step: h=%d heads (max 16)", h);
  }
  }
#undef AS_RO2
  AS_CHECK_LAUNCH("rollout_step2");
  if (nsplit > 1) {
    dim3 fg(as_ceil_div(as_ceil_div(N, 32) * 32, 64), as_round_up(Trows, 32), B);
    hipLaunchKernelGGL((rollout_finish_kernel<T>), fg, dim3(64), 0, s, (const float*)part, Rin, Rout, (T*)rf_out, B, N,
                       Trows, nsplit);
    AS_CHECK_LAUNCH("rollout_finish");
  }
  return AS_OK;
}

int rollout_nsplit(int B, int N) {
  const int wgs = as_ceil_div(N, 32) * B;
  int ns = 1;
  while (ns < 16 && wgs * ns < 2048) ns *= 2;
  return wgs >= 2048 ? 1 : ns;
}

template <typename T>
int launch_mean_rows(const void* q, const void* k, const float* lse, float* out, void* rf_out, int B, int N, int h,
                     int row0, int nrows, bool top, hipStream_t s) {
  const int Npad = as_round_up(N, 64);
  dim3 grid(as_ceil_div(as_ceil_div(N, 32), 4), as_ceil_div(nrows, 32), B);
  if (top)
    hipLaunchKernelGGL((attn_mean_rows_kernel<T, true>), grid, dim3(RO_NT), 0, s, (const T*)q, (const T*)k, lse,
                       out, (T*)rf_out, B, N, Npad, h, row0, nrows);
  else
    hipLaunchKernelGGL((attn_mean_rows_kernel<T, false>), grid, dim3(RO_NT), 0, s, (const T*)q, (const T*)k, lse,
                       out, (T*)rf_out, B, N, Npad, h, row0, nrows);
  AS_CHECK_LAUNCH("attn_mean_rows");
  return AS_OK;
}

}

extern "C" size_t as_rollout_rfrag_bytes(int B, int N, int dtype) {
  if (B <= 0 || N <= 0) return 0;
  return (size_t)B * as_ceil_div(N, 32) * 4 * 2 * 64 * 8 * (dtype == AS_BF16 ? 2 : 4);
}

extern "C" int as_attn_mean_rows(const void* q, const void* k, const float* lse, float* out, int B, int N, int h,
                                 int row0, int nrows, int dtype, as_stream_t stream) {
  AS_REQUIRE(q && k && lse && out, AS_E_BADARG, "as_attn_mean_rows: null pointer");
  AS_REQUIRE(B > 0 && N > 0 && h > 0 && row0 >= 0 && nrows > 0 && row0 + nrows <= N, AS_E_BADARG,
             "as_attn_mean_rows: bad row range %d+%d of %d", row0, nrows, N);
  hipStream_t s = (hipStream_t)stream;
  if (dtype == AS_BF16) return launch_mean_rows<__bf16>(q, k, lse, out, nullptr, B, N, h, row0, nrows, false, s);
  if (dtype == AS_F32) return launch_mean_rows<float>(q, k, lse, out, nullptr, B, N, h, row0, nrows, false, s);
  AS_REQUIRE(false, AS_E_UNSUPPORTED, "as_attn_mean_rows: dtype %d", dtype);
}

extern "C" int as_rollout_top(const void* q, const void* k, const float* lse, float* R_out, void* rf_out, int B, int N,
                              int h, int T, int dtype, as_stream_t stream) {
  AS_REQUIRE(q && k && lse && R_out, AS_E_BADARG, "as_rollout_top: null pointer");
  AS_REQUIRE(B > 0 && h > 0 && T > 0 && T <= N && T <= 128, AS_E_BADARG, "as_rollout_top: bad sizes N=%d T=%d", N, T);
  hipStream_t s = (hipStream_t)stream;
  if (dtype == AS_BF16) return launch_mean_rows<__bf16>(q, k, lse, R_out, rf_out, B, N, h, N - T, T, true, s);
  if (dtype == AS_F32) return launch_mean_rows<float>(q, k, lse, R_out, rf_out, B, N, h, N - T, T, true, s);
  AS_REQUIRE(false, AS_E_UNSUPPORTED, "as_rollout_top: dtype %d", dtype);
}

namespace {
template <typename T>
__global__ __launch_bounds__(64) void rollout_pack_kernel(const float* __restrict__ R, T* __restrict__ rf, int B, int N, int Trows) {
  const int nkb = (N + 31) / 32;
  const int j = blockIdx.x * 64 + threadIdx.x, i = blockIdx.y, b = blockIdx.z;
  if (j >= nkb * 32) return;
  const float v = (i < Trows && j < N) ? R[((size_t)b * Trows + i) * N + j] : 0.0f;
  rf[rf_slot(b, nkb, i, j)] = from_f32<T>(v);
}
}

extern "C" int as_rollout_pack(const float* R, void* rf, int B, int N, int T, int dtype, as_stream_t stream) {
  AS_REQUIRE(R && rf, AS_E_BADARG, "as_rollout_pack: null pointer");
  AS_REQUIRE(B > 0 && N > 0 && T > 0 && T <= 128, AS_E_BADARG, "as_rollout_pack: bad sizes N=%d T=%d", N, T);
  dim3 grid(as_ceil_div(as_ceil_div(N, 32) * 32, 64), as_round_up(T, 32), B);
  if (dtype == AS_BF16)
    hipLaunchKernelGGL(rollout_pack_kernel<__bf16>, grid, dim3(64), 0, (hipStream_t)stream, R, (__bf16*)rf, B, N, T);
  else if (dtype == AS_F32)
    hipLaunchKernelGGL(rollout_pack_kernel<float>, grid, dim3(64), 0, (hipStream_t)stream, R, (float*)rf, B, N, T);
  else
    AS_REQUIRE(false, AS_E_UNSUPPORTED, "as_rollout_pack: dtype %d", dtype);
  AS_CHECK_LAUNCH("rollout_pack");
  return AS_OK;
}

extern "C" size_t as_rollout_step_workspace_bytes(int B, int N, int T) {
  if (B <= 0 || N <= 0 || T <= 0) return 0;
  return (size_t)R4_MAXPARTS * B * T * N * sizeof(float);
}

extern "C" int as_rollout_step(const void* q, const void* k, const float* lse, const float* R_in, const void* rf_in,
                               float* R_out, void* rf_out, void* workspace, size_t workspace_bytes, int B, int N, int h,
                               int T, int dtype, as_stream_t stream) {
  AS_REQUIRE(q && k && lse && R_in && rf_in && R_out && R_in != R_out && rf_in != rf_out, AS_E_BADARG,
             "as_rollout_step: null/aliased pointer");
  AS_REQUIRE(B > 0 && h > 0 && h <= 16 && T > 0 && T <= N && T <= 128, AS_E_BADARG,
             "as_rollout_step: bad sizes N=%d T=%d h=%d", N, T, h);
  hipStream_t s = (hipStream_t)stream;
  const size_t need = as_rollout_step_workspace_bytes(B, N, T);
  const bool have_ws = workspace != nullptr && workspace_bytes >= need && need > 0;
  const bool stream4 = have_ws && dtype == AS_BF16 && h % R4_HPG == 0 && !rollout_force_v3();
  const int ns = stream4 ? R4_MAXPARTS : (have_ws ? rollout_nsplit(B, N) : 1);
  float* part = ns > 1 ? (float*)workspace : nullptr;
  if (dtype == AS_BF16)
    return launch_rollout_step2<__bf16>(q, k, lse, R_in, rf_in, R_out, rf_out, part, ns, B, N, h, T, s);
  if (dtype == AS_F32) return launch_rollout_step2<float>(q, k, lse, R_in, rf_in, R_out, rf_out, part, ns, B, N, h, T, s);
  AS_REQUIRE(false, AS_E_UNSUPPORTED, "as_rollout_step: dtype %d", dtype);
}
```

attentionshift_amd/ops.py:

```python
import ctypes
import os

import threading

import numpy as np
import torch

from . import _lib
from ._lib import AS_BF16, AS_F32, AttnShiftError

HEAD_DIM = 64


def _dt(t):
    if t.dtype == torch.float32:
        return AS_F32
    if t.dtype == torch.bfloat16:
        return AS_BF16
    raise AttnShiftError(f"unsupported dtype {t.dtype} (float32 or bfloat16)")


def _chk(*tensors, dtype=None):
    for t in tensors:
        if t is None:
            continue
        if not t.is_cuda:
            raise AttnShiftError("hot-path ops need device (HBM) tensors; there is no CPU fallback")
        if not t.is_contiguous():
            raise AttnShiftError("hot-path ops need contiguous row-major tensors")
        if dtype is not None and t.dtype != dtype:
            raise AttnShiftError(f"expected {dtype}, got {t.dtype}")


def _p(t):
    return 0 if t is None else t.data_ptr()


_RAW_STREAM = getattr(torch._C, "_cuda_getCurrentRawStream", None)
_DEV = [None]


def _stream():
    if _RAW_STREAM is None:
        return torch.cuda.current_stream().cuda_stream
    d = _DEV[0]
    if d is None:
        d = _DEV[0] = torch.cuda.current_device()
    return _RAW_STREAM(d)


_TIMED = None


def enable_timing(names):
    global _TIMED
    _TIMED = {n: [] for n in names}


def disable_timing():
    global _TIMED
    _TIMED = None


def collect_timing():
    out = {}
    for n, evs in (_TIMED or {}).items():
        if n.endswith(":bytes"):
            out[n] = (len(evs), float(sum(evs)) / max(len(evs), 1))
        elif evs:
            ms = [a.elapsed_time(b) for a, b in evs]
            out[n] = (len(ms), sum(ms) / len(ms))
    return out


class _timed:
    def __init__(self, name):
        self.on = _TIMED is not None and name in _TIMED
        self.name = name

    def __enter__(self):
        if self.on:
            self.a, self.b = torch.cuda.Event(enable_timing=True), torch.cuda.Event(enable_timing=True)
            self.a.record(torch.cuda.current_stream())

    def __exit__(self, *exc):
        if self.on:
            self.b.record(torch.cuda.current_stream())
            _TIMED[self.name].append((self.a, self.b))


def npad(n):
    return _lib.load().as_npad(int(n))


_SK_BYTES = {}
_SK_WS = {}


def _sk_bytes(lib, M, Nout, K):
    key = (M, Nout, K, os.environ.get("AS_GEMM_SK"))
    v = _SK_BYTES.get(key)
    if v is None:
        v = _SK_BYTES[key] = int(lib.as_linear_sk_workspace_bytes(M, Nout, K))
    return v


def _sk_workspace(device, nbytes):
    key = (device, torch.cuda.current_stream(device).cuda_stream)
    ws = _SK_WS.get(key)
    if ws is None or ws.numel() < nbytes:
        ws = _SK_WS[key] = torch.empty(nbytes, device=device, dtype=torch.uint8)
    return ws


def linear(x, weight, bias=None, act="none"):
    lib = _lib.load()
    K = x.shape[-1]
    x2 = x.reshape(-1, K)
    _chk(x2, weight)
    if bias is not None:
        _chk(bias, dtype=torch.float32)
    if weight.dtype != x.dtype or weight.shape[1] != K:
        raise AttnShiftError("linear: weight must be [Nout, K] in the dtype of x")
    out = torch.empty(x2.shape[0], weight.shape[0], device=x.device, dtype=x.dtype)
    code = {"none": 0, "gelu": 1, "relu": 4}[act]
    M, Nout = x2.shape[0], weight.shape[0]
    need = _sk_bytes(lib, M, Nout, K) if x.dtype == torch.bfloat16 else 0
    if need:
        ws = _sk_workspace(x.device, need)
        _lib.check(lib.as_linear_sk_fwd(_p(x2), _p(weight), _p(bias), _p(out), M, Nout, K, _dt(x), code, _p(ws), ws.numel(),
                                        _stream()), "as_linear_sk_fwd")
    else:
        _lib.check(lib.as_linear_fwd(_p(x2), _p(weight), _p(bias), _p(out), M, Nout, K, _dt(x), code, _stream()), "as_linear_fwd")
    return out.reshape(*x.shape[:-1], Nout)


def linear_small(x, weight, bias=None, act="none", out=None):
    lib = _lib.load()
    if x.dim() != 2 or x.dtype != torch.float32 or weight.dtype != torch.float32 or x.stride(1) != 1 or not weight.is_contiguous():
        raise AttnShiftError("linear_small: x [M, K] fp32 with unit column stride, weight [Nout, K] fp32 contiguous")
    M, K = x.shape
    Nout = weight.shape[0]
    if weight.shape[1] != K:
        raise AttnShiftError("linear_small: weight must be [Nout, K]")
    if bias is not None:
        _chk(bias, dtype=torch.float32)
    if out is None:
        out = torch.empty(M, Nout, device=x.device, dtype=torch.float32)
    elif out.shape != (M, Nout) or out.dtype != torch.float32 or out.stride(1) != 1:
        raise AttnShiftError("linear_small: out must be [M, Nout] fp32 with unit column stride")
    code = {"none": 0, "gelu": 1, "relu": 4, "sigmoid": 5}[act]
    _lib.check(lib.as_linear_small_fwd(_p(x), x.stride(0), _p(weight), _p(bias), _p(out), out.stride(0), M, Nout, K, code, _stream()),
               "as_linear_small_fwd")
    return out


def linear_small_applies(x, weight):
    return (x.is_cuda and x.dtype == torch.float32 and weight.dtype == torch.float32 and x.dim() == 2 and 0 < x.shape[0] <= 1024
            and x.shape[1] >= 64 and x.shape[1] % 16 == 0 and x.stride(1) == 1 and x.stride(0) % 4 == 0 and weight.is_contiguous()
            and x.data_ptr() % 16 == 0 and weight.data_ptr() % 16 == 0)


def linear_gelu(x, weight, bias=None):
    lib = _lib.load()
    _chk(x, weight, dtype=torch.bfloat16)
    if bias is not None:
        _chk(bias, dtype=torch.float32)
    M, K = x.shape
    Nout = weight.shape[0]
    if weight.shape[1] != K:
        raise AttnShiftError("linear_gelu: weight must be [Nout, K]")
    out = torch.empty(M, Nout, device=x.device, dtype=torch.bfloat16)
    pre = torch.empty_like(out)
    _lib.check(lib.as_linear_gelu_fwd(_p(x), _p(weight), _p(bias), _p(out), _p(pre), M, Nout, K, AS_BF16, _stream()),
               "as_linear_gelu_fwd")
    return out, pre


def linear_gelu_applies(x, weight):
    return x.is_cuda and x.numel() > 0 and weight.shape[0] % 32 == 0 and weight.shape[1] % 32 == 0


def linear_splitk(x, weight, out_dtype=None):
    lib = _lib.load()
    _chk(x, weight, dtype=torch.bfloat16)
    M, K = x.shape
    Nout = weight.shape[0]
    if weight.shape[1] != K:
        raise AttnShiftError("linear_splitk: weight must be [Nout, K]")
    out_dtype = out_dtype or torch.bfloat16
    out = torch.empty(M, Nout, device=x.device, dtype=out_dtype)
    nbytes = int(lib.as_linear_splitk_workspace_bytes(M, Nout, K))
    ws = torch.empty(max(nbytes, 4) // 4, device=x.device, dtype=torch.float32)
    _lib.check(lib.as_linear_splitk_fwd(_p(x), _p(weight), _p(out), M, Nout, K, AS_BF16, 1 if out_dtype == torch.float32 else 0,
                                        _p(ws), nbytes, _stream()), "as_linear_splitk_fwd")
    return out


_LINEAR_BWD_WS = {}


def linear_bwd(x, weight, dy, need_dx=True, need_dw=True, need_db=True, dw_dtype=None, gelu_pre=None):
    lib = _lib.load()
    _chk(x, weight, dy, dtype=torch.bfloat16)
    M, K = x.shape
    Nout = weight.shape[0]
    if weight.shape[1] != K or tuple(dy.shape) != (M, Nout):
        raise AttnShiftError("linear_bwd: shapes must be x [M,K], weight [Nout,K], dy [M,Nout]")
    dw_dtype = dw_dtype or torch.bfloat16
    dx = torch.empty(M, K, device=x.device, dtype=torch.bfloat16) if need_dx else None
    dW = torch.empty(Nout, K, device=x.device, dtype=dw_dtype) if need_dw else None
    db = torch.empty(Nout, device=x.device, dtype=torch.float32) if need_db else None
    nbytes = int(lib.as_linear_bwd_workspace_bytes(M, Nout, K))
    key = (x.device, torch.cuda.current_stream(x.device).cuda_stream)
    ws = _LINEAR_BWD_WS.get(key)
    if ws is None or ws.numel() * 4 < nbytes:
        ws = _LINEAR_BWD_WS[key] = torch.empty((nbytes + 3) // 4, device=x.device, dtype=torch.float32)
    if gelu_pre is not None:
        _chk(gelu_pre, dtype=torch.bfloat16)
        if tuple(gelu_pre.shape) != (M, K) or not need_dx:
            raise AttnShiftError("linear_bwd: gelu_pre must be [M,K] and needs dx")
        _lib.check(lib.as_linear_bwd_dgelu(_p(x), _p(weight), _p(dy), _p(gelu_pre), _p(dx), _p(dW), _p(db), M, Nout, K, AS_BF16,
                                           1 if dw_dtype == torch.float32 else 0, _p(ws), nbytes, _stream()), "as_linear_bwd_dgelu")
        return dx, dW, db
    _lib.check(lib.as_linear_bwd(_p(x), _p(weight), _p(dy), _p(dx), _p(dW), _p(db), M, Nout, K, AS_BF16,
                                 1 if dw_dtype == torch.float32 else 0, _p(ws), nbytes, _stream()), "as_linear_bwd")
    return dx, dW, db


def deconv2x2(x_nhwc, w4, bias4=None, act="none"):
    lib = _lib.load()
    B, h, w, cin = x_nhwc.shape
    cout = w4.shape[0] // 4
    _chk(x_nhwc, w4)
    if bias4 is not None:
        _chk(bias4, dtype=torch.float32)
    out = torch.empty(B, 2 * h, 2 * w, cout, device=x_nhwc.device, dtype=x_nhwc.dtype)
    _lib.check(lib.as_deconv2x2_fwd(_p(x_nhwc), _p(w4), _p(bias4), _p(out), B * h * w, w, cin, cout, _dt(x_nhwc),
                                    1 if act == "gelu" else 0, _stream()), "as_deconv2x2_fwd")
    return out


def _scale_arg(delta_scale, x, delta):
    if delta_scale is None:
        return None, 1
    if delta is None or x.dim() != 3 or delta_scale.numel() != x.shape[0]:
        raise AttnShiftError("add_layernorm: delta_scale needs delta and x [B, N, D] with one scale per image")
    _chk(delta_scale, dtype=torch.float32)
    return delta_scale, x.shape[1]


def add_layernorm(x, delta, gamma, beta, eps, out_dtype, want_x=True, want_y=True, delta_scale=None, x_out=None):
    lib = _lib.load()
    D = x.shape[-1]
    x2 = x.reshape(-1, D)
    _chk(x2, dtype=torch.float32)
    _chk(delta)
    _chk(gamma, beta, dtype=torch.float32)
    if delta is not None and delta.dtype != out_dtype:
        raise AttnShiftError("add_layernorm: delta must have the output dtype")
    if x_out is not None:
        if not (want_x and delta is not None) or x_out.shape != x.shape:
            raise AttnShiftError("add_layernorm: x_out needs want_x, a delta and x's shape")
        _chk(x_out, dtype=torch.float32)
        x_out = x_out.view(-1, D)
    else:
        x_out = torch.empty_like(x2) if (want_x and delta is not None) else None
    y = torch.empty(x2.shape, device=x.device, dtype=out_dtype) if want_y else None
    dt = AS_BF16 if out_dtype == torch.bfloat16 else AS_F32
    sc, rps = _scale_arg(delta_scale, x, delta)
    _lib.check(lib.as_add_layernorm_scaled(_p(x2), _p(delta), _p(gamma), _p(beta), float(eps), _p(x_out), _p(y), x2.shape[0], D,
                                           dt, _p(sc), rps, _stream()), "as_add_layernorm")
    xo = x if (delta is None or not want_x) else x_out.reshape(x.shape)
    return (xo if want_x else None), (None if y is None else y.reshape(x.shape))


def assemble_tokens(emb, table):
    lib = _lib.load()
    emb = emb.contiguous()
    _chk(emb)
    _chk(table, dtype=torch.float32)
    B, Np, D = emb.shape
    N = table.shape[0]
    x = torch.empty(B, N, D, device=emb.device, dtype=torch.float32)
    _lib.check(lib.as_assemble_tokens(_p(emb), _p(table), _p(x), B, Np, N, D, _dt(emb), _stream()), "as_assemble_tokens")
    return x


def maxpool_nhwc(x_nhwc, k):
    lib = _lib.load()
    B, H, W, C = x_nhwc.shape
    if not (x_nhwc.is_cuda and x_nhwc.dtype == torch.float32):
        raise AttnShiftError("maxpool_nhwc: fp32 device tensor expected")
    if x_nhwc.stride()[1:] != (W * C, C, 1) or (B > 1 and x_nhwc.stride(0) % 4):
        x_nhwc = x_nhwc.contiguous()
    bs = x_nhwc.stride(0) if B > 1 else H * W * C
    out = torch.empty(B, H // k, W // k, C, device=x_nhwc.device, dtype=torch.float32)
    _lib.check(lib.as_maxpool_nhwc(_p(x_nhwc), _p(out), B, H, W, C, int(k), int(bs), _stream()), "as_maxpool_nhwc")
    return out


def add_layernorm_bwd(x_out, dy, dx_res, gamma, eps, dtype, want_dx=True, want_ddelta=True, want_affine=True, delta_scale=None):
    lib = _lib.load()
    D = x_out.shape[-1]
    x2 = x_out.reshape(-1, D)
    _chk(x2, dx_res, gamma, dtype=torch.float32)
    _chk(dy, dtype=dtype)
    M = x2.shape[0]
    dev = x_out.device
    scratch = not want_dx and not want_ddelta
    dx = torch.empty_like(x2) if (want_dx or scratch) else None
    dd = torch.empty(x2.shape, device=dev, dtype=dtype) if want_ddelta else None
    affine = want_affine and dy is not None
    dg = torch.empty(D, device=dev, dtype=torch.float32) if affine else None
    db = torch.empty(D, device=dev, dtype=torch.float32) if affine else None
    nbytes = lib.as_add_layernorm_bwd_workspace_bytes(M, D)
    ws = torch.empty(nbytes, device=dev, dtype=torch.uint8)
    dt = AS_BF16 if dtype == torch.bfloat16 else AS_F32
    sc, rps = (None, 1) if delta_scale is None else (delta_scale, x_out.shape[1] if x_out.dim() == 3 else 1)
    if sc is not None and (x_out.dim() != 3 or sc.numel() != x_out.shape[0]):
        raise AttnShiftError("add_layernorm_bwd: delta_scale needs x_out [B, N, D] with one scale per image")
    _lib.check(lib.as_add_layernorm_bwd_scaled(_p(x2), _p(dy), _p(dx_res), _p(gamma), float(eps), _p(dx), _p(dd), _p(dg), _p(db),
                                               _p(ws), nbytes, M, D, dt, _p(sc), rps, _stream()), "as_add_layernorm_bwd")
    return (None if dx is None or scratch else dx.reshape(x_out.shape), None if dd is None else dd.reshape(x_out.shape), dg, db)


class AttnLayerState:

    __slots__ = ("q", "k", "vt", "lse", "B", "N", "h", "dtype", "o")

    def __init__(self, q, k, vt, lse, B, N, h, dtype, o=None):
        self.q, self.k, self.vt, self.lse, self.B, self.N, self.h, self.dtype = q, k, vt, lse, B, N, h, dtype
        self.o = o


def _sdpa_ws(lib, B, N, h, like):
    n = lib.as_sdpa_fwd_workspace_bytes(B, N, h, _dt(like))
    return (torch.empty(n, device=like.device, dtype=torch.uint8), n) if n else (None, 0)


def attention_fwd(x, w_qkv, b_qkv, w_proj, b_proj, num_heads, keep_state=True, keep_o=False):
    lib = _lib.load()
    B, N, D = x.shape
    _chk(x, w_qkv, w_proj)
    if D != num_heads * HEAD_DIM:
        raise AttnShiftError(f"head dim must be {HEAD_DIM} (D={D}, heads={num_heads})")
    Np_ = npad(N)
    dev, dt = x.device, x.dtype
    q = torch.empty(B, num_heads, Np_, HEAD_DIM, device=dev, dtype=dt)
    k = torch.empty_like(q)
    vt = torch.empty(B, num_heads, HEAD_DIM, Np_, device=dev, dtype=dt)
    o = torch.empty(B, N, D, device=dev, dtype=dt)
    out = torch.empty(B, N, D, device=dev, dtype=dt)
    lse = torch.empty(B, num_heads, N, device=dev, dtype=torch.float32)
    ws, wbytes = _sdpa_ws(lib, B, N, num_heads, x)
    if _TIMED is None:
        _lib.check(lib.as_attn_fwd(_p(x), _p(w_qkv), _p(b_qkv), _p(w_proj), _p(b_proj), _p(out), _p(lse), _p(q), _p(k),
                                   _p(vt), _p(o), _p(ws), wbytes, B, N, D, num_heads, _dt(x), _stream()), "as_attn_fwd")
    else:
        with _timed("qkv_gemm"):
            _lib.check(lib.as_qkv_fwd(_p(x), _p(w_qkv), _p(b_qkv), _p(q), _p(k), _p(vt), B, N, D, num_heads, _dt(x),
                                      _stream()), "as_qkv_fwd")
        with _timed("sdpa_fwd"):
            _lib.check(lib.as_sdpa_fwd(_p(q), _p(k), _p(vt), _p(o), _p(lse), _p(ws), wbytes, B, N, num_heads, _dt(x),
                                       _stream()), "as_sdpa_fwd")
        with _timed("proj_gemm"):
            _lib.check(lib.as_linear_fwd(_p(o), _p(w_proj), _p(b_proj), _p(out), B * N, D, D, _dt(x), 0, _stream()),
                       "as_linear_fwd")
    return out, (AttnLayerState(q, k, vt, lse, B, N, num_heads, dt, o if keep_o else None) if keep_state else None)


def attention_bwd(x, w_qkv, w_proj, dout, state, want_bias=(True, True)):
    lib = _lib.load()
    B, N, D = x.shape
    if state.o is None:
        raise AttnShiftError("attention_bwd needs the forward's pre-projection output: call attention_fwd(keep_o=True)")
    _chk(x, w_qkv, w_proj, dout, state.q, state.k, state.vt, state.o, state.lse)
    dev, dt = x.device, x.dtype
    dx = torch.empty_like(x)
    dwqkv = torch.empty_like(w_qkv)
    dwproj = torch.empty_like(w_proj)
    dbqkv = torch.empty(3 * D, device=dev, dtype=torch.float32) if want_bias[0] else None
    dbproj = torch.empty(D, device=dev, dtype=torch.float32) if want_bias[1] else None
    nbytes = lib.as_attn_bwd_workspace_bytes(B, N, D, state.h, _dt(x))
    ws = torch.empty(nbytes, device=dev, dtype=torch.uint8)
    with _timed("attn_bwd"):
        _lib.check(lib.as_attn_bwd(_p(x), _p(w_qkv), _p(w_proj), _p(dout), _p(state.q), _p(state.k), _p(state.vt),
                                   _p(state.o), _p(state.lse), _p(dx), _p(dwqkv), _p(dbqkv), _p(dwproj), _p(dbproj),
                                   _p(ws), nbytes, B, N, D, state.h, _dt(x), _stream()), "as_attn_bwd")
    return dx, dwqkv, dbqkv, dwproj, dbproj


QSCALE = 0.125 * 1.4426950408889634
LN2 = 0.6931471805599453


def q_to_fragment_major(q_rows):
    B, h, Np_, d = q_rows.shape
    t = q_rows.reshape(B, h, Np_ // 32, 32, 4, 2, 8)
    return t.permute(0, 1, 2, 4, 5, 3, 6).contiguous().reshape(B, h, Np_, d)


def q_from_fragment_major(q_frag):
    B, h, Np_, d = q_frag.shape
    t = q_frag.reshape(B, h, Np_ // 32, 4, 2, 32, 8)
    return t.permute(0, 1, 2, 5, 3, 4, 6).contiguous().reshape(B, h, Np_, d)


def qkv_fwd(x, w_qkv, b_qkv, num_heads):
    lib = _lib.load()
    B, N, D = x.shape
    _chk(x, w_qkv)
    Np_ = npad(N)
    q = torch.empty(B, num_heads, Np_, HEAD_DIM, device=x.device, dtype=x.dtype)
    k = torch.empty_like(q)
    vt = torch.empty(B, num_heads, HEAD_DIM, Np_, device=x.device, dtype=x.dtype)
    _lib.check(lib.as_qkv_fwd(_p(x), _p(w_qkv), _p(b_qkv), _p(q), _p(k), _p(vt), B, N, D, num_heads, _dt(x), _stream()),
               "as_qkv_fwd")
    return q, k, vt


def sdpa_fwd(q, k, vt, N):
    lib = _lib.load()
    B, h = q.shape[0], q.shape[1]
    _chk(q, k, vt)
    o = torch.empty(B, N, h * HEAD_DIM, device=q.device, dtype=q.dtype)
    lse = torch.empty(B, h, N, device=q.device, dtype=torch.float32)
    ws, wbytes = _sdpa_ws(lib, B, N, h, q)
    _lib.check(lib.as_sdpa_fwd(_p(q), _p(k), _p(vt), _p(o), _p(lse), _p(ws), wbytes, B, N, h, _dt(q), _stream()),
               "as_sdpa_fwd")
    return o, lse


def sdpa_bwd(q, k, vt, o, d_o, lse, N):
    lib = _lib.load()
    B, h = q.shape[0], q.shape[1]
    _chk(q, k, vt, o, d_o, lse)
    dqkv = torch.empty(B, N, 3 * h * HEAD_DIM, device=q.device, dtype=q.dtype)
    nbytes = lib.as_sdpa_bwd_workspace_bytes(B, N, h, _dt(q))
    ws = torch.empty(nbytes, device=q.device, dtype=torch.uint8)
    _lib.check(lib.as_sdpa_bwd(_p(q), _p(k), _p(vt), _p(o), _p(d_o), _p(lse), _p(dqkv), _p(ws), nbytes, B, N, h,
                               _dt(q), _stream()), "as_sdpa_bwd")
    return dqkv


def window_attention_fwd(qkv, b_qkv, table, num_heads, ws, shift, return_attn=False):
    lib = _lib.load()
    B, H, W, C3 = qkv.shape
    C = C3 // 3
    _chk(qkv)
    _chk(b_qkv, table, dtype=torch.float32)
    out = torch.empty(B, H, W, C, device=qkv.device, dtype=qkv.dtype)
    nW = -(-H // ws) * -(-W // ws)
    attn = torch.empty(B * nW, num_heads, ws * ws, ws * ws, device=qkv.device, dtype=torch.float32) if return_attn else None
    with _timed("window_attn_fwd"):
        _lib.check(lib.as_window_attn_fwd(_p(qkv), _p(b_qkv), _p(table), _p(out), _p(attn), B, H, W, C, num_heads, int(ws),
                                          int(shift), _dt(qkv), _stream()), "as_window_attn_fwd")
    if _TIMED is not None and "window_attn_fwd" in _TIMED:
        _TIMED.setdefault("window_attn_fwd:bytes", []).append(qkv.numel() * qkv.element_size() + out.numel() * out.element_size())
    return out, attn


def window_attention_bwd(qkv, b_qkv, table, d_out, num_heads, ws, shift):
    lib = _lib.load()
    B, H, W, C3 = qkv.shape
    C = C3 // 3
    _chk(qkv, d_out)
    _chk(b_qkv, table, dtype=torch.float32)
    dqkv = torch.zeros_like(qkv)
    dtable = torch.empty_like(table)
    dpad = torch.empty(C3, device=qkv.device, dtype=torch.float32)
    nbytes = lib.as_window_attn_bwd_workspace_bytes(B, H, W, num_heads, int(ws))
    wsbuf = torch.empty(nbytes, device=qkv.device, dtype=torch.uint8)
    _lib.check(lib.as_window_attn_bwd(_p(qkv), _p(b_qkv), _p(table), _p(d_out), _p(dqkv), _p(dtable), _p(dpad), _p(wsbuf),
                                      nbytes, B, H, W, C, num_heads, int(ws), int(shift), _dt(qkv), _stream()),
               "as_window_attn_bwd")
    return dqkv, dtable, dpad


def attn_mean_rows(state, row0, nrows):
    lib = _lib.load()
    out = torch.empty(state.B, nrows, state.N, device=state.q.device, dtype=torch.float32)
    _lib.check(lib.as_attn_mean_rows(_p(state.q), _p(state.k), _p(state.lse), _p(out), state.B, state.N, state.h,
                                     int(row0), int(nrows), _dt(state.q), _stream()), "as_attn_mean_rows")
    return out


def rollout_rows(states, num_point_tokens, rows=None, use_workspace=True):
    lib = _lib.load()
    top = states[-1]
    T = int(num_point_tokens)
    dev, dt = top.q.device, _dt(top.q)
    nbytes = lib.as_rollout_rfrag_bytes(top.B, top.N, dt)
    outs = []
    R = torch.empty(top.B, T, top.N, device=dev, dtype=torch.float32)
    lower = list(reversed(states[:-1]))
    subset = rows is not None and len(lower) > 0
    rf = torch.empty(nbytes, device=dev, dtype=torch.uint8) if not subset else None
    _lib.check(lib.as_rollout_top(_p(top.q), _p(top.k), _p(top.lse), _p(R), _p(rf), top.B, top.N, top.h, T, dt, _stream()),
               "as_rollout_top")
    if rows is not None:
        R = torch.gather(R, 1, rows[:, :, None].expand(-1, -1, top.N)).contiguous()
        T = R.shape[1]
        if subset:
            rf = torch.empty(nbytes, device=dev, dtype=torch.uint8)
            _lib.check(lib.as_rollout_pack(_p(R), _p(rf), top.B, top.N, T, dt, _stream()), "as_rollout_pack")
    outs.append(R)
    wbytes = lib.as_rollout_step_workspace_bytes(top.B, top.N, T) if (lower and use_workspace) else 0
    ws = torch.empty(wbytes, device=dev, dtype=torch.uint8) if wbytes else None
    for n, st in enumerate(lower):
        Rn = torch.empty_like(R)
        rfn = torch.empty_like(rf) if n + 1 < len(lower) else None
        _lib.check(lib.as_rollout_step(_p(st.q), _p(st.k), _p(st.lse), _p(R), _p(rf), _p(Rn), _p(rfn), _p(ws), wbytes,
                                       st.B, st.N, st.h, T, dt, _stream()), "as_rollout_step")
        outs.append(Rn)
        R, rf = Rn, rfn
    return torch.stack(outs, dim=1)


def rollout_rows_dense(states, num_point_tokens, rows=None):
    T = int(num_point_tokens)
    run, outs = None, []
    for st in reversed(states):
        a = attn_mean_rows(st, 0, st.N)
        a.diagonal(dim1=1, dim2=2).add_(1.0)
        a /= a.sum(-1, keepdim=True)
        if run is None:
            run = a[:, st.N - T:, :]
            if rows is not None:
                run = torch.gather(run, 1, rows[:, :, None].expand(-1, -1, st.N))
        else:
            run = torch.bmm(run, a)
        outs.append(run.contiguous())
        del a
    return torch.stack(outs, dim=1)


def ccl_2d(binary):
    lib = _lib.load()
    squeeze = binary.dim() == 2
    img = binary[None] if squeeze else binary
    _chk(img, dtype=torch.uint8)
    M, H, W = img.shape
    labels = torch.empty(M, H, W, device=img.device, dtype=torch.int32)
    _lib.check(lib.as_ccl_2d(_p(img), _p(labels), M, H, W, _stream()), "as_ccl_2d")
    return labels[0] if squeeze else labels


def cam_boxes(cams, points, cam_thr, area_ratio, up=16, return_upsampled=False, return_minmax=False):
    lib = _lib.load()
    _chk(cams, points, dtype=torch.float32)
    M, Hp, Wp = cams.shape
    boxes = torch.empty(M, 4, device=cams.device, dtype=torch.float32)
    status = torch.empty(M, device=cams.device, dtype=torch.int32)
    cams_up = torch.empty(M, Hp * up, Wp * up, device=cams.device, dtype=torch.float32) if return_upsampled else None
    minmax = torch.empty(M, 2, device=cams.device, dtype=torch.float32) if (return_upsampled or return_minmax) else None
    nbytes = lib.as_cam_boxes_workspace_bytes(M, Hp, Wp, up)
    ws = torch.empty(nbytes, device=cams.device, dtype=torch.uint8)
    _lib.check(lib.as_cam_boxes(_p(cams), _p(points), float(cam_thr), float(area_ratio), M, Hp, Wp, up, _p(boxes),
                                _p(status), _p(cams_up), _p(minmax), _p(ws), nbytes, _stream()), "as_cam_boxes")
    if return_upsampled:
        return boxes, status, cams_up, minmax
    return (boxes, status, minmax) if return_minmax else (boxes, status)


def cam_sample_masks(cams, map_idx, minmax, thr_bg, thr_fg, up=16, want_counts=True):
    lib = _lib.load()
    _chk(cams, minmax, dtype=torch.float32)
    _chk(map_idx, dtype=torch.int32)
    M, Hp, Wp = cams.shape
    G = map_idx.shape[0]
    masks = torch.empty(2 * G + 1, Hp * up, Wp * up, device=cams.device, dtype=torch.uint8)
    counts = torch.empty(2 * G + 1, device=cams.device, dtype=torch.int32) if want_counts else None
    nbytes = lib.as_cam_sample_masks_workspace_bytes(G, Hp, Wp, up)
    ws = torch.empty(nbytes, device=cams.device, dtype=torch.uint8) if nbytes else None
    _lib.check(lib.as_cam_sample_masks(_p(cams), _p(map_idx), _p(minmax), G, Hp, Wp, up, float(thr_bg), float(thr_fg),
                                       _p(masks), _p(counts), _p(ws), nbytes, _stream()), "as_cam_sample_masks")
    return masks, counts


def semantic_prestage(map_fg, thr, k=11, up=16, want_counts=True):
    lib = _lib.load()
    _chk(map_fg, dtype=torch.float32)
    G, H, W = map_fg.shape
    hp, wp = H // up, W // up
    fg_inter = torch.empty(G, hp, wp, device=map_fg.device, dtype=torch.float32)
    mask = torch.empty(G, hp, wp, device=map_fg.device, dtype=torch.uint8)
    counts = torch.empty(G, device=map_fg.device, dtype=torch.int32) if want_counts else None
    _lib.check(lib.as_semantic_prestage(_p(map_fg), float(thr), int(k), G, hp, wp, up, _p(fg_inter), _p(mask), _p(counts),
                                        _stream()), "as_semantic_prestage")
    return fg_inter, mask, counts


_shift_ws = {}
_shift_ws_lock = threading.Lock()
_SHIFT_WS_MAX_BYTES = 256 << 20


def cosine_shift(feat, box_patch, obj_img, prot, n_shift, hp, wp, tau0=0.1, temp=0.1, return_trace=False):
    lib = _lib.load()
    _chk(prot, dtype=torch.float32)
    _chk(box_patch, obj_img, dtype=torch.int32)
    B, Np_, C = feat.shape
    G, P, _ = prot.shape
    if Np_ != hp * wp:
        raise AttnShiftError("cosine_shift: Np != hp*wp")
    if not (feat.is_cuda and feat.dtype == torch.float32 and feat.stride(2) == 1 and feat.stride(1) == C
            and (B == 1 or (feat.stride(0) >= Np_ * C and feat.stride(0) % 4 == 0)) and feat.data_ptr() % 16 == 0):
        raise AttnShiftError("cosine_shift: feat must be fp32 [B,Np,C] on the device with contiguous, 16-byte aligned image blocks")
    fbs = feat.stride(0) if B > 1 else Np_ * C
    prot_out = torch.empty_like(prot)
    sim = torch.empty(G, P, Np_, device=feat.device, dtype=torch.float32)
    assign = torch.empty(max(n_shift, 1), G, Np_, device=feat.device, dtype=torch.int32) if return_trace else None
    tau = torch.empty(max(n_shift, 1), G, P, device=feat.device, dtype=torch.float32) if return_trace else None
    key = (feat.device, torch.cuda.current_stream(feat.device).cuda_stream, B, C, hp, wp, G, P)
    with _shift_ws_lock:
        ws = _shift_ws.get(key)
        if ws is None:
            nbytes = lib.as_cosine_shift_workspace_bytes(B, C, hp, wp, G, P)
            if sum(t.numel() for t in _shift_ws.values()) + nbytes > _SHIFT_WS_MAX_BYTES:
                _shift_ws.clear()
            ws = torch.empty(nbytes, device=feat.device, dtype=torch.uint8)
            _shift_ws[key] = ws
    with _timed("cosine_shift"):
        _lib.check(lib.as_cosine_shift_strided(_p(feat), int(fbs), _p(box_patch), _p(obj_img), _p(prot), _p(prot_out), float(tau0),
                                               float(temp), int(n_shift), _p(sim), _p(assign), _p(tau), _p(ws), ws.numel(), B, C,
                                               hp, wp, G, P, _stream()), "as_cosine_shift")
    if return_trace:
        return prot_out, sim, assign[:n_shift], tau[:n_shift]
    return prot_out, sim


def refine_similarity(feat, seeds, boxes_patch, num_obj, refine_times, tau, is_select, hp, wp):
    lib = _lib.load()
    _chk(feat, seeds, dtype=torch.float32)
    if boxes_patch is not None:
        _chk(boxes_patch, dtype=torch.int32)
    Np_, C = feat.shape
    Gp = seeds.shape[0]
    maps = torch.empty(refine_times + 1, Gp, Np_, device=feat.device, dtype=torch.float32)
    seeds_out = seeds if refine_times == 0 else torch.empty(Gp, C, device=feat.device, dtype=torch.float32)
    nbytes = lib.as_refine_similarity_workspace_bytes(C, Np_, Gp)
    ws = torch.empty(nbytes, device=feat.device, dtype=torch.uint8)
    n_select = (Gp if is_select else 0) if isinstance(is_select, bool) else int(is_select)
    _lib.check(lib.as_refine_similarity(_p(feat), _p(seeds), _p(boxes_patch), int(num_obj), Gp, int(refine_times),
                                        float(tau), n_select, _p(maps), _p(seeds_out), _p(ws), nbytes, C,
                                        hp, wp, _stream()), "as_refine_similarity")
    return maps, seeds_out


def instance_maps(sim_fg, sim_bg, num_obj, hp, wp, up=16):
    lib = _lib.load()
    _chk(sim_fg, sim_bg, dtype=torch.float32)
    L, Gp, _ = sim_fg.shape
    G = int(num_obj)
    H, W = hp * up, wp * up
    map_fg = torch.empty(L, G, H, W, device=sim_fg.device, dtype=torch.float32)
    map_bg = torch.empty(L, G, H, W, device=sim_fg.device, dtype=torch.float32)
    nbytes = lib.as_instance_maps_workspace_bytes(L, G)
    ws = torch.empty(nbytes, device=sim_fg.device, dtype=torch.uint8)
    _lib.check(lib.as_instance_maps(_p(sim_fg), _p(sim_bg), L, G, Gp, hp, wp, up, _p(map_fg), _p(map_bg), _p(ws), nbytes,
                                    _stream()), "as_instance_maps")
    return map_fg, map_bg


def crop_threshold_erode(maps, crops, thr, relative, k):
    lib = _lib.load()
    _chk(maps, dtype=torch.float32)
    if crops is not None:
        _chk(crops, dtype=torch.int32)
    M, H, W = maps.shape
    mask = torch.empty(M, H, W, device=maps.device, dtype=torch.uint8)
    counts = torch.empty(M, device=maps.device, dtype=torch.int32)
    nbytes = lib.as_crop_threshold_erode_workspace_bytes(M, H, W)
    ws = torch.empty(nbytes, device=maps.device, dtype=torch.uint8)
    _lib.check(lib.as_crop_threshold_erode(_p(maps), _p(crops), float(thr), 1 if relative else 0, int(k), _p(mask),
                                           _p(counts), _p(ws), nbytes, M, H, W, _stream()), "as_crop_threshold_erode")
    return mask, counts


def mask_candidates(map_fg, map_bg, crops, pos_thr, neg_thr, mask_thr, k):
    lib = _lib.load()
    _chk(map_fg, map_bg, dtype=torch.float32)
    _chk(crops, dtype=torch.int32)
    G, H, W = map_fg.shape
    pos, neg, pseudo = (torch.empty(G, H, W, device=map_fg.device, dtype=torch.uint8) for _ in range(3))
    counts = torch.empty(3, G, device=map_fg.device, dtype=torch.int32)
    nbytes = lib.as_mask_candidates_workspace_bytes(G, H, W)
    ws = torch.empty(nbytes, device=map_fg.device, dtype=torch.uint8)
    _lib.check(lib.as_mask_candidates(_p(map_fg), _p(map_bg), _p(crops), float(pos_thr), float(neg_thr), float(mask_thr),
                                      int(k), _p(pos), _p(neg), _p(pseudo), _p(counts), _p(ws), nbytes, G, H, W,
                                      _stream()), "as_mask_candidates")
    return pos, neg, pseudo, counts


def part_stats_raw(maps, rois, owner, stride=16):
    lib = _lib.load()
    maps = maps.contiguous()
    rois = rois.contiguous().float()
    own = owner.to(torch.int32).contiguous()
    _chk(maps, rois, dtype=torch.float32)
    M, hp, wp = maps.shape
    c = torch.empty(M, 2, device=maps.device, dtype=torch.float32)
    yx = torch.empty(M, 2, device=maps.device, dtype=torch.int32)
    area = torch.empty(M, device=maps.device, dtype=torch.int32)
    inside = torch.empty(M, device=maps.device, dtype=torch.uint8)
    _lib.check(lib.as_part_stats(_p(maps), _p(rois), _p(own), float(stride), _p(c), _p(yx), _p(area), _p(inside), M, hp, wp,
                                 _stream()), "as_part_stats")
    return c, yx, area, inside


def part_stats(maps, rois, owner, stride=16):
    c, yx, area, inside = part_stats_raw(maps, rois, owner, stride)
    return c, yx.long(), area.long(), inside.bool()


def part_select(area, inside, ngroups, c, yx, labels, feat_tok, G, P, wp, num_points):
    lib = _lib.load()
    _chk(c, feat_tok, dtype=torch.float32)
    _chk(area, yx, ngroups, dtype=torch.int32)
    _chk(inside, dtype=torch.uint8)
    _chk(labels, dtype=torch.int64)
    dev, M, C = c.device, G * P, feat_tok.shape[-1]
    coords = torch.empty(2, M, 2, device=dev, dtype=torch.float32)
    lab = torch.empty(3, M, device=dev, dtype=torch.int64)
    feats = torch.empty(M, C, device=dev, dtype=torch.float32)
    ints = torch.empty(M + G + 1, device=dev, dtype=torch.int32)
    _lib.check(lib.as_part_select(_p(area), _p(inside), _p(ngroups), _p(c), _p(yx), _p(labels), _p(feat_tok), G, P, C, int(wp),
                                  int(num_points), _p(coords[0]), _p(coords[1]), _p(lab[0]), _p(lab[1]), _p(lab[2]), _p(feats),
                                  _p(ints[:M]), _p(ints[M:]), _stream()), "as_part_select")
    return coords[0], coords[1], lab[0], lab[1], lab[2], feats, ints[M:]


def filter_parts(sim, fg_inter, sim_thr=0.8, pos_thr=0.85):
    lib = _lib.load()
    sim = sim.contiguous()
    fg = fg_inter.contiguous()
    _chk(sim, fg, dtype=torch.float32)
    G, P = sim.shape[:2]
    keep = torch.empty(G, P, device=sim.device, dtype=torch.uint8)
    _lib.check(lib.as_filter_parts(_p(sim), _p(fg), float(sim_thr), float(pos_thr), _p(keep), G, P, sim[0, 0].numel(),
                                   _stream()), "as_filter_parts")
    return keep.view(torch.bool)


def draw_distinct(counts, u, k, flag=None):
    lib = _lib.load()
    if counts.dtype != torch.int32:
        counts = counts.to(torch.int32)
    if tuple(counts.shape) != (u.shape[0], 2):
        raise AttnShiftError(f"draw_distinct: counts {tuple(counts.shape)} for {u.shape[0]} objects")
    sg, sk = counts.stride()
    if sg <= 0 or sk <= 0:
        counts = counts.contiguous()
        sg, sk = 2, 1
    if not counts.is_cuda:
        raise AttnShiftError("hot-path ops need device (HBM) tensors; there is no CPU fallback")
    u = u.contiguous()
    _chk(u, dtype=torch.float32)
    G, M = u.shape
    rp = torch.empty(G, k, device=u.device, dtype=torch.int32)
    rn = torch.empty(G, k, device=u.device, dtype=torch.int32)
    ip = torch.empty(G, k, device=u.device, dtype=torch.uint8)
    if flag is None:
        flag = torch.zeros(1, device=u.device, dtype=torch.int32)
    _lib.check(lib.as_draw_distinct(_p(counts), sg, sk, _p(u), _p(rp), _p(rn), _p(ip), _p(flag), G, M, int(k), _stream()),
               "as_draw_distinct")
    return rp, rn, ip.view(torch.bool), flag


def small_attention_fwd(qkv):
    lib = _lib.load()
    qkv = qkv.contiguous()
    _chk(qkv)
    Bp, N, _, h, d = qkv.shape
    out = torch.empty(Bp, N, h * d, device=qkv.device, dtype=qkv.dtype)
    lse = torch.empty(Bp, h, N, device=qkv.device, dtype=torch.float32)
    _lib.check(lib.as_small_attn_fwd(_p(qkv), _p(out), _p(lse), Bp, N, h, d, _dt(qkv), _stream()), "as_small_attn_fwd")
    return out, lse


def small_attention_bwd(qkv, out, d_out, lse):
    lib = _lib.load()
    qkv, out, d_out = qkv.contiguous(), out.contiguous(), d_out.contiguous().to(qkv.dtype)
    _chk(qkv, out, d_out)
    Bp, N, _, h, d = qkv.shape
    dqkv = torch.empty_like(qkv)
    nbytes = lib.as_small_attn_bwd_workspace_bytes(Bp, N, h)
    ws = torch.empty(nbytes, device=qkv.device, dtype=torch.uint8)
    _lib.check(lib.as_small_attn_bwd(_p(qkv), _p(out), _p(d_out), _p(lse), _p(dqkv), _p(ws), nbytes, Bp, N, h, d, _dt(qkv),
                                     _stream()), "as_small_attn_bwd")
    return dqkv


def chamfer_2d_fwd(xyz1, xyz2):
    lib = _lib.load()
# ... 379 lines not shown
```

include/attnshift.h:

```cpp
#ifndef ATTNSHIFT_H
#define ATTNSHIFT_H

#include <stddef.h>
#include <stdint.h>

#ifdef __cplusplus
extern "C" {
#endif

#define AS_VERSION 100
#define AS_OK 0
#define AS_E_BADARG (-1)
#define AS_E_UNSUPPORTED (-2)
#define AS_E_LAUNCH (-3)
#define AS_E_WORKSPACE (-4)

#define AS_F32 0
#define AS_BF16 1

#define AS_HEAD_DIM 64

typedef void* as_stream_t;

int as_version(void);
const char* as_last_error(void);


int as_npad(int N);

int as_linear_fwd(const void* x, const void* W, const float* bias, void* out, int M, int Nout, int K,
                  int dtype, int act, as_stream_t stream);

int as_linear_small_fwd(const float* x, int ldx, const float* W, const float* bias, float* out, int ldo, int M, int Nout, int K,
                        int act, as_stream_t stream);

size_t as_linear_sk_workspace_bytes(int M, int Nout, int K);
int as_linear_sk_fwd(const void* x, const void* W, const float* bias, void* out, int M, int Nout, int K, int dtype, int act,
                     void* ws, size_t ws_bytes, as_stream_t stream);

int as_deconv2x2_fwd(const void* x, const void* W4, const float* bias4, void* out, int M, int w, int cin, int cout,
                     int dtype, int act, as_stream_t stream);

int as_qkv_fwd(const void* x , const void* Wqkv , const float* bqkv ,
               void* q, void* k, void* vt, int B, int N, int D, int h, int dtype, as_stream_t stream);

size_t as_sdpa_fwd_workspace_bytes(int B, int N, int h, int dtype);
int as_sdpa_fwd(const void* q, const void* k, const void* vt, void* o, float* lse, void* workspace,
                size_t workspace_bytes, int B, int N, int h, int dtype, as_stream_t stream);

size_t as_sdpa_bwd_workspace_bytes(int B, int N, int h, int dtype);
int as_sdpa_bwd(const void* q, const void* k, const void* vt, const void* o, const void* d_o, const float* lse,
                void* dqkv, void* workspace, size_t workspace_bytes, int B, int N, int h, int dtype,
                as_stream_t stream);

int as_attn_fwd(const void* x, const void* Wqkv, const float* bqkv, const void* Wproj, const float* bproj,
                void* out , float* lse, void* q, void* k, void* vt, void* o, void* workspace,
                size_t workspace_bytes , int B, int N, int D, int h,
                int dtype, as_stream_t stream);

size_t as_attn_bwd_workspace_bytes(int B, int N, int D, int h, int dtype);
int as_attn_bwd(const void* x, const void* Wqkv, const void* Wproj, const void* dout, const void* q, const void* k,
                const void* vt, const void* o, const float* lse, void* dx, void* dWqkv, float* dbqkv, void* dWproj,
                float* dbproj, void* workspace, size_t workspace_bytes, int B, int N, int D, int h, int dtype,
                as_stream_t stream);

int as_window_attn_fwd(const void* qkv, const float* bqkv, const float* table, void* out, float* attn_out, int B, int H,
                       int W, int C, int h, int ws, int shift, int dtype, as_stream_t stream);

int as_add_layernorm(const float* x_in, const void* delta, const float* gamma, const float* beta, float eps,
                     float* x_out, void* y_out, int M, int D, int dtype, as_stream_t stream);
int as_add_layernorm_scaled(const float* x_in, const void* delta, const float* gamma, const float* beta, float eps,
                            float* x_out, void* y_out, int M, int D, int dtype, const float* delta_scale,
                            int rows_per_scale, as_stream_t stream);

int as_linear_gelu_fwd(const void* x, const void* W, const float* bias, void* out, void* pre, int M, int Nout, int K,
                       int dtype, as_stream_t stream);
int as_linear_dgelu_fwd(const void* x, const void* W, const void* pre, void* out, int M, int Nout, int K, int dtype,
                        as_stream_t stream);

size_t as_linear_splitk_workspace_bytes(int M, int Nout, int K);
int as_linear_splitk_fwd(const void* x, const void* W, void* out, int M, int Nout, int K, int dtype, int out_f32,
                         void* workspace, size_t workspace_bytes, as_stream_t stream);

size_t as_linear_bwd_workspace_bytes(int M, int Nout, int K);
int as_linear_bwd(const void* x, const void* W, const void* dy, void* dx, void* dW, float* db, int M, int Nout, int K,
                  int dtype, int dw_f32, void* workspace, size_t workspace_bytes, as_stream_t stream);
int as_linear_bwd_dgelu(const void* x, const void* W, const void* dy, const void* pre, void* dx, void* dW, float* db, int M,
                        int Nout, int K, int dtype, int dw_f32, void* workspace, size_t workspace_bytes, as_stream_t stream);

int as_maxpool_nhwc(const float* x, float* out, int B, int H, int W, int C, int k, long long x_batch_stride,
                    as_stream_t stream);

int as_assemble_tokens(const void* emb, const float* table, float* out, int B, int Np, int N, int D, int dtype,
                       as_stream_t stream);

size_t as_add_layernorm_bwd_workspace_bytes(int M, int D);
int as_add_layernorm_bwd(const float* x, const void* dy, const float* dx_res, const float* gamma, float eps, float* dx_out,
                         void* ddelta_out, float* dgamma, float* dbeta, void* workspace, size_t workspace_bytes, int M, int D,
                         int dtype, as_stream_t stream);
int as_add_layernorm_bwd_scaled(const float* x, const void* dy, const float* dx_res, const float* gamma, float eps,
                                float* dx_out, void* ddelta_out, float* dgamma, float* dbeta, void* workspace,
                                size_t workspace_bytes, int M, int D, int dtype, const float* delta_scale,
                                int rows_per_scale, as_stream_t stream);

size_t as_window_attn_bwd_workspace_bytes(int B, int H, int W, int h, int ws);
int as_window_attn_bwd(const void* qkv, const float* bqkv, const float* table, const void* d_out, void* dqkv,
                       float* dtable, float* dbqkv_pad, void* workspace, size_t workspace_bytes, int B, int H, int W,
                       int C, int h, int ws, int shift, int dtype, as_stream_t stream);

int as_attn_mean_rows(const void* q, const void* k, const float* lse, float* out, int B, int N, int h,
                      int row0, int nrows, int dtype, as_stream_t stream);

size_t as_rollout_rfrag_bytes(int B, int N, int dtype);
int as_rollout_pack(const float* R, void* rf, int B, int N, int T, int dtype, as_stream_t stream);
size_t as_rollout_step_workspace_bytes(int B, int N, int T);
int as_rollout_top(const void* q, const void* k, const float* lse, float* R_out, void* rf_out, int B, int N, int h,
                   int T, int dtype, as_stream_t stream);
int as_rollout_step(const void* q, const void* k, const float* lse, const float* R_in, const void* rf_in,
                    float* R_out, void* rf_out, void* workspace, size_t workspace_bytes, int B, int N, int h, int T,
                    int dtype, as_stream_t stream);


int as_ccl_2d(const uint8_t* img , int32_t* labels , int M, int H, int W,
              as_stream_t stream);

size_t as_cam_boxes_workspace_bytes(int M, int Hp, int Wp, int up);
int as_cam_boxes(const float* cams , const float* points , float cam_thr,
                 float area_ratio, int M, int Hp, int Wp, int up, float* boxes, int32_t* status,
                 float* cams_up, float* minmax, void* ws, size_t ws_bytes, as_stream_t stream);

size_t as_cam_sample_masks_workspace_bytes(int G, int Hp, int Wp, int up);
int as_cam_sample_masks(const float* cams , const int32_t* map_idx ,
                        const float* minmax , int G, int Hp, int Wp, int up, float thr_bg, float thr_fg,
                        uint8_t* masks, int32_t* counts, void* ws, size_t ws_bytes, as_stream_t stream);

size_t as_mask_candidates_workspace_bytes(int G, int H, int W);
int as_mask_candidates(const float* map_fg, const float* map_bg, const int32_t* crops, float pos_thr, float neg_thr,
                       float mask_thr, int k, uint8_t* pos, uint8_t* neg, uint8_t* pseudo, int32_t* counts, void* ws,
                       size_t ws_bytes, int G, int H, int W, as_stream_t stream);

int as_part_stats(const float* maps, const float* rois, const int32_t* owner, float stride, float* out_c,
                  int32_t* out_yx, int32_t* out_area, uint8_t* out_inside, int M, int Hp, int Wp, as_stream_t stream);

int as_part_select(const int32_t* area, const uint8_t* inside, const int32_t* ngroups, const float* c, const int32_t* yx,
                   const int64_t* labels, const float* feat_tok, int G, int P, int C, int Wp, int num_points, float* coords,
                   float* coords_org, int64_t* out_labels, int64_t* labels_org, int64_t* corres, float* feats,
                   int32_t* sel_slot, int32_t* split, as_stream_t stream);

int as_filter_parts(const float* sim , const float* fg_inter , float sim_thr, float pos_thr,
                    uint8_t* keep , int G, int P, int Np, as_stream_t stream);

int as_draw_distinct(const int32_t* counts, int count_stride_g, int count_stride_k, const float* u ,
                     int32_t* rank_pos , int32_t* rank_neg, uint8_t* is_pos, int32_t* flag, int G, int M, int K,
                     as_stream_t stream);

int as_mt_sample_ranks(int32_t* state , const int32_t* counts , int32_t* ranks , int32_t* flag,
                       int S, int K, as_stream_t stream);
int as_mt_perm_ranks(int32_t* state , const int32_t* counts2 , int32_t* ranks , int32_t* flag,
                     int G, int K, as_stream_t stream);

int as_merge_plan(const uint8_t* keep, const uint8_t* link, int32_t* groups, int32_t* ngroups, int G, int P,
                  as_stream_t stream);

int as_semantic_prestage(const float* map_fg, float thr, int k, int G, int Hp, int Wp, int up, float* fg_inter,
                         uint8_t* mask, int32_t* counts, as_stream_t stream);

size_t as_cosine_shift_workspace_bytes(int B, int C, int Hp, int Wp, int G, int P);
int as_cosine_shift(const float* feat, const int32_t* box_patch, const int32_t* obj_img, const float* prot_in,
                    float* prot_out, double tau0, double temp, int n_shift, float* sim_out, int32_t* assign_out,
                    float* tau_out, void* ws, size_t ws_bytes, int B, int C, int Hp, int Wp, int G, int P,
                    as_stream_t stream);
int as_cosine_shift_strided(const float* feat, long long feat_batch_stride, const int32_t* box_patch, const int32_t* obj_img,
                            const float* prot_in, float* prot_out, double tau0, double temp, int n_shift, float* sim_out,
                            int32_t* assign_out, float* tau_out, void* ws, size_t ws_bytes, int B, int C, int Hp, int Wp, int G,
                            int P, as_stream_t stream);

size_t as_refine_similarity_workspace_bytes(int C, int Np, int Gp);
int as_refine_similarity(const float* feat, const float* seeds, const int32_t* boxes, int G, int Gp,
                         int refine_times, float tau, int n_select, float* maps, float* seeds_out, void* ws,
                         size_t ws_bytes, int C, int Hp, int Wp, as_stream_t stream);

size_t as_instance_maps_workspace_bytes(int L, int G);
int as_instance_maps(const float* sim_fg, const float* sim_bg, int L, int G, int Gp, int Hp, int Wp, int up,
                     float* map_fg, float* map_bg, void* ws, size_t ws_bytes, as_stream_t stream);

size_t as_crop_threshold_erode_workspace_bytes(int M, int H, int W);
int as_crop_threshold_erode(const float* maps , const int32_t* crops, float thr, int relative, int k,
                            uint8_t* mask , int32_t* counts , void* ws, size_t ws_bytes, int M, int H,
                            int W, as_stream_t stream);

int as_mask_count(const uint8_t* mask, int32_t* counts, int M, int HW, as_stream_t stream);

size_t as_rank_select_workspace_bytes(int M, int HW);
int as_rank_select(const uint8_t* mask , const int32_t* ranks , int32_t* out , void* ws,
                   size_t ws_bytes, int M, int HW, int K, as_stream_t stream);
int as_rank_select_xy(const uint8_t* mask , const int32_t* ranks , int64_t* out_xy , void* ws,
                      size_t ws_bytes, int M, int HW, int K, int W, int yx_order, as_stream_t stream);

int as_merge_parts(const float* prot, const uint8_t* keep, float thr, float* merged , int32_t* ngroups ,
                   int32_t* flag, int G, int P, int C, int slots, as_stream_t stream);

int as_select_median_boxes(const float* boxes , const int32_t* meta , int Lc, int stride,
                           const int64_t* pick_in, int64_t* pick , float* chosen , int32_t* map_idx , int32_t* box_patch ,
                           int32_t* box_int , const int32_t* status, int32_t* bad, int n, as_stream_t stream);

int as_rank_draw_xy(const uint8_t* mask , int mode, const float* u , int32_t* flag,
                    int64_t* out_xy , int64_t* patch_out , int patch_div, int patch_w, int64_t patch_base,
                    int row_rot, void* ws, size_t ws_bytes, int M, int HW, int K, int W, int yx_order, as_stream_t stream);

int as_small_attn_fwd(const void* qkv, void* out, float* lse, int Bp, int N, int h, int d, int dtype, as_stream_t stream);
size_t as_small_attn_bwd_workspace_bytes(int Bp, int N, int h);
int as_small_attn_bwd(const void* qkv, const void* out, const void* d_out, const float* lse, void* dqkv, void* workspace,
                      size_t workspace_bytes, int Bp, int N, int h, int d, int dtype, as_stream_t stream);

int as_roi_align_fwd(const float* feat, const float* rois, float* out, int B, int H, int W, int C, int R, int out_size,
                     float spatial_scale, int sampling_ratio, int aligned, as_stream_t stream);
int as_roi_align_bwd(const float* dout, const float* rois, float* dfeat, int B, int H, int W, int C, int R, int out_size,
                     float spatial_scale, int sampling_ratio, int aligned, as_stream_t stream);

int as_chamfer_2d_fwd(const float* xyz1, const float* xyz2, float* dist1, float* dist2, int32_t* idx1, int32_t* idx2,
                      int B, int n, int m, as_stream_t stream);
int as_chamfer_2d_bwd(const float* xyz1, const float* xyz2, const float* gdist1, const float* gdist2, const int32_t* idx1,
                      const int32_t* idx2, float* gxyz1, float* gxyz2, int B, int n, int m, as_stream_t stream);


size_t as_nms_workspace_bytes(int n);
int as_nms(const float* boxes_sorted, int n, float iou_thr, int max_keep, long long* keep_idx, int* count, void* workspace,
           size_t workspace_bytes, as_stream_t stream);

int as_paste_masks(const float* src, const long long* labels, const float* boxes, void* out, int n, int K, int h, int w,
                   int H, int W, int apply_sigmoid, int out_mode, float thr, as_stream_t stream);

int as_rle_tile(int* rows_per_segment, int* cols_per_workgroup);
size_t as_rle_workspace_bytes(int n, int H, int W);
int as_rle_count(const void* masks, int n, int H, int W, uint32_t* totals, void* workspace, size_t workspace_bytes,
                 as_stream_t stream);
int as_rle_encode(const void* masks, int n, int H, int W, const uint32_t* totals, void* workspace, size_t workspace_bytes,
                  uint32_t* pos, size_t pos_capacity, void* str, size_t str_capacity, unsigned long long* lens,
                  as_stream_t stream);

typedef struct {
  const float* cls;
  const float* reg;
  int H, W, stride_x, stride_y;
} as_rpn_level;
size_t as_rpn_candidates_workspace_bytes(int B, int C);
int as_rpn_candidates(const as_rpn_level* levels, int L, int B, int A, const float* base_anchors, const float* img_shapes,
                      int nms_pre, float min_bbox_size, const float* means_stds, float max_ratio, int C, float* cand_box,
                      float* cand_nms_box, float* cand_score, int32_t* cand_level, int32_t* cand_index, int32_t* cand_count,
                      void* workspace, size_t workspace_bytes, as_stream_t stream);

size_t as_rpn_assign_workspace_bytes(int B, int T, int sum_g);
int as_rpn_assign(const as_rpn_level* levels, int L, int B, int A, const float* base_anchors, const float* gt_boxes,
                  const int32_t* gt_offsets, int sum_g, int max_g, const int32_t* shapes, float pos_iou_thr, float neg_iou_thr,
                  float min_pos_iou, int match_low_quality, int allowed_border, int32_t* assigned, float* max_iou,
                  int32_t* counts, void* workspace, size_t workspace_bytes, as_stream_t stream);
int as_rpn_sample(int B, int T, int sum_g, int num, const int32_t* assigned, const int32_t* plan, const int32_t* ranks,
                  const void* workspace, size_t workspace_bytes, int32_t* inds, as_stream_t stream);
int as_rpn_targets(const as_rpn_level* levels, int L, int B, int A, const float* base_anchors, const float* gt_boxes,
                   const int32_t* gt_offsets, int sum_g, const int32_t* assigned, const int32_t* pos_inds, int inds_stride,
                   int num, const float* means_stds, int32_t* pos_gt, float* pos_delta, as_stream_t stream);

#ifdef __cplusplus
}
#endif
#endif
```

Baseline: 321.9.

## Fuse token assembly with first layernorm, group point-head linears, and fuse rollout rows

Adds a kernel that assembles patch embeddings with the token table and applies the first block's layernorm in one pass, so block 0 skips its separate add_layernorm. It also adds a grouped small-linear kernel that runs the cls and reg head branches in a single launch, reading strided batch inputs directly. Finally, the rollout for selected rows writes each layer's result into one strided output buffer, avoiding per-layer allocation and gather. Each path sits behind an AS_CHAIN_FUSE switch that is on by default, and adds new kernels and an env-controlled code path to maintain.

```diff
diff --git a/attentionshift_amd/_lib.py b/attentionshift_amd/_lib.py
--- a/attentionshift_amd/_lib.py
+++ b/attentionshift_amd/_lib.py
@@ -15,6 +15,7 @@
     "as_npad": (_c_int, [_c_int]),
     "as_linear_fwd": (_c_int, [_c_void_p] * 4 + [_c_int] * 5 + [_c_void_p]),
     "as_linear_small_fwd": (_c_int, [_c_void_p, _c_int, _c_void_p, _c_void_p, _c_void_p] + [_c_int] * 5 + [_c_void_p]),
+    "as_linear_small_grouped_fwd": (_c_int, [_c_void_p] + [_c_int] * 4 + [_c_void_p]),
     "as_linear_sk_workspace_bytes": (_c_size_t, [_c_int] * 3),
     "as_linear_sk_fwd": (_c_int, [_c_void_p] * 4 + [_c_int] * 5 + [_c_void_p, _c_size_t, _c_void_p]),
     "as_linear_gelu_fwd": (_c_int, [_c_void_p] * 5 + [_c_int] * 4 + [_c_void_p]),
@@ -40,6 +41,7 @@
     "as_linear_bwd": (_c_int, [_c_void_p] * 6 + [_c_int] * 5 + [_c_void_p, ctypes.c_size_t, _c_void_p]),
     "as_linear_bwd_dgelu": (_c_int, [_c_void_p] * 7 + [_c_int] * 5 + [_c_void_p, ctypes.c_size_t, _c_void_p]),
     "as_assemble_tokens": (_c_int, [_c_void_p] * 3 + [_c_int] * 5 + [_c_void_p]),
+    "as_assemble_layernorm": (_c_int, [_c_void_p] * 4 + [ctypes.c_float] + [_c_void_p] * 2 + [_c_int] * 5 + [_c_void_p]),
     "as_maxpool_nhwc": (_c_int, [_c_void_p] * 2 + [_c_int] * 5 + [ctypes.c_longlong, _c_void_p]),
     "as_mask_count": (_c_int, [_c_void_p] * 2 + [_c_int] * 2 + [_c_void_p]),
     "as_window_attn_bwd_workspace_bytes": (_c_size_t, [_c_int] * 5),
@@ -51,6 +53,9 @@
     "as_rollout_top": (_c_int, [_c_void_p] * 5 + [_c_int] * 5 + [_c_void_p]),
     "as_rollout_step_workspace_bytes": (_c_size_t, [_c_int] * 3),
     "as_rollout_step": (_c_int, [_c_void_p] * 8 + [_c_size_t] + [_c_int] * 5 + [_c_void_p]),
+    "as_rollout_top_rows": (_c_int, [_c_void_p] * 5 + [ctypes.c_longlong, _c_void_p] + [_c_int] * 6 + [_c_void_p]),
+    "as_rollout_step_strided": (_c_int, [_c_void_p] * 4 + [ctypes.c_longlong] + [_c_void_p] * 2 + [ctypes.c_longlong]
+                                + [_c_void_p] * 2 + [_c_size_t] + [_c_int] * 5 + [_c_void_p]),
     "as_ccl_2d": (_c_int, [_c_void_p] * 2 + [_c_int] * 3 + [_c_void_p]),
     "as_cam_boxes_workspace_bytes": (_c_size_t, [_c_int] * 4),
     "as_cam_boxes": (_c_int, [_c_void_p] * 2 + [_c_float] * 2 + [_c_int] * 4 + [_c_void_p] * 5 + [_c_size_t, _c_void_p]),
@@ -117,6 +122,17 @@
 class RpnLevel(ctypes.Structure):
     _fields_ = [("cls", _c_void_p), ("reg", _c_void_p), ("H", _c_int), ("W", _c_int), ("stride_x", _c_int), ("stride_y", _c_int)]
 
+
+class LinearSmallGroup(ctypes.Structure):
+    _fields_ = [("x", _c_void_p), ("W", _c_void_p), ("bias", _c_void_p), ("out", _c_void_p), ("x_batch_stride", ctypes.c_longlong),
+                ("ldx", _c_int), ("ldo", _c_int), ("Nout", _c_int), ("act", _c_int)]
+
+
+_CHAIN_ITEMS = ("assemble", "head", "rollout")
+_cf = os.environ.get("AS_CHAIN_FUSE", "1").strip()
+CHAIN_FUSE = frozenset() if _cf == "0" else frozenset(_CHAIN_ITEMS) if _cf in ("", "1") else \
+    frozenset(t.strip() for t in _cf.split(",")) & frozenset(_CHAIN_ITEMS)
+
 _lib = None
 
 
diff --git a/attentionshift_amd/backbone.py b/attentionshift_amd/backbone.py
--- a/attentionshift_amd/backbone.py
+++ b/attentionshift_amd/backbone.py
@@ -6,6 +6,7 @@
 import torch.nn.functional as F
 
 from . import ops
+from ._lib import CHAIN_FUSE
 from .registry import BACKBONES
 
 
@@ -316,6 +317,13 @@
             self._point_pack = pk
         B, T, D = x.shape
         hc = c[0].out_features
+        if "head" in CHAIN_FUSE and hc % 16 == 0 and hc >= 64 and x.stride(2) == 1 and x.stride(1) % 4 == 0 \
+                and x.stride(0) % 4 == 0 and ops.linear_small_applies(x[0], pk["w1"]):
+            h1, = ops.linear_small_grouped([x], [pk["w1"]], [pk["b1"]], ["relu"])
+            h2c, h2b = ops.linear_small_grouped([h1[:, :hc], h1[:, hc:]], [c[1].weight, b[1].weight], [c[1].bias, b[1].bias],
+                                                ["relu", "relu"])
+            cls, reg = ops.linear_small_grouped([h2c, h2b], [c[2].weight, b[2].weight], [c[2].bias, b[2].bias], ["none", "sigmoid"])
+            return cls.reshape(B, T, -1), reg.reshape(B, T, -1)
         x2 = x.reshape(B * T, D)
         if ops.linear_small_applies(x2, pk["w1"]) and hc % 16 == 0 and hc >= 64:
             h1 = ops.linear_small(x2, pk["w1"], pk["b1"], act="relu")
@@ -343,7 +351,7 @@
         assert int(w0) == grid.shape[-2] and int(h0) == grid.shape[-1]
         return torch.cat((self.pos_embed[:, :1], grid.permute(0, 2, 3, 1).reshape(1, -1, dim)), dim=1)
 
-    def prepare_tokens(self, img):
+    def prepare_tokens(self, img, norm=None):
         B, C, w, h = img.shape
         ps = self.patch_size
         hp, wp = w // ps, h // ps
@@ -351,6 +359,8 @@
         patches.copy_(img.reshape(B, C, hp, ps, wp, ps).permute(0, 2, 4, 1, 3, 5))
         wmat = self._derived(self.patch_embed.proj.weight, "patch", lambda t: t.reshape(self.embed_dim, -1))
         emb = ops.linear(patches.view(B, hp * wp, C * ps * ps), wmat, self.patch_embed.proj.bias.float())
+        if norm is not None:
+            return ops.assemble_layernorm(emb, self._token_table(hp * wp, w, h), norm.weight, norm.bias, norm.eps)
         return ops.assemble_tokens(emb, self._token_table(hp * wp, w, h))
 
     def _token_table(self, Np, w, h):
@@ -365,10 +375,11 @@
             self._wcache["token_table"] = hit
         return hit[1]
 
-    def _block(self, blk, x, delta, keep_state, need_x, on_full=None, full_out=None, x_out=None):
+    def _block(self, blk, x, delta, keep_state, need_x, on_full=None, full_out=None, x_out=None, y=None):
         cd = self.compute_dtype
-        x, y = ops.add_layernorm(x, delta, blk.norm1.weight, blk.norm1.bias, blk.norm1.eps, cd,
-                                 x_out=full_out if delta is not None else None)
+        if y is None or delta is not None:
+            x, y = ops.add_layernorm(x, delta, blk.norm1.weight, blk.norm1.bias, blk.norm1.eps, cd,
+                                     x_out=full_out if delta is not None else None)
         if on_full is not None:
             on_full(x)
         a, st = ops.attention_fwd(y, self._w(blk.attn.qkv.weight),
@@ -439,7 +450,13 @@
         hp, wp = H // self.patch_size, W // self.patch_size
         T = self.point_tokens_num
         grad_path = self._grad_path()
-        x = self._prepare_tokens_train(x) if grad_path else self.prepare_tokens(x)
+        y0 = None
+        if grad_path:
+            x = self._prepare_tokens_train(x)
+        elif "assemble" in CHAIN_FUSE and x.is_cuda and self.embed_dim <= 3072:
+            x, y0 = self.prepare_tokens(x, self.blocks[0].norm1)
+        else:
+            x = self.prepare_tokens(x)
         if self.recompute_last_feat:
             last_feat = x
         features, taps, attns = [], [], []
@@ -493,7 +510,7 @@
                                            take_tap if tap_due else None,
                                            full_out=tap_slot(len(features)) if tap_due and x.dtype == torch.float32 else None,
                                            x_out=tap_slot(len(features) + int(tap_due)) if last_tap and x.dtype == torch.float32
-                                           else None)
+                                           else None, y=y0 if i == 0 else None)
                 tap_due = i in self.out_indices and i != nblk - 1
                 if i in self.out_indices and i == nblk - 1:
                     take_tap(x)
diff --git a/attentionshift_amd/csrc/layernorm.hip b/attentionshift_amd/csrc/layernorm.hip
--- a/attentionshift_amd/csrc/layernorm.hip
+++ b/attentionshift_amd/csrc/layernorm.hip
@@ -2,27 +2,39 @@
 
 namespace {
 
-template <typename T, int VPL>
+template <typename T, int VPL, bool ASM>
 __global__ __launch_bounds__(256) void add_layernorm_kernel(const float* __restrict__ x_in, const T* __restrict__ delta,
                                                             const float* __restrict__ gamma, const float* __restrict__ beta,
                                                             float* __restrict__ x_out, T* __restrict__ y_out, int M, int D,
-                                                            float eps, const float* __restrict__ dscale, int rps) {
+                                                            float eps, const float* __restrict__ dscale, int rps, int N, int Np) {
   const int row = blockIdx.x * 4 + (threadIdx.x >> 6), lane = threadIdx.x & 63;
   if (row >= M) return;
   const size_t base = (size_t)row * D;
   const float ds = dscale != nullptr ? dscale[row / rps] : 1.0f;
+  const int tn = N > 0 ? row % N : 0, tb = N > 0 ? row / N : 0;
+  const bool patch = tn >= 1 && tn <= Np;
+  const size_t pbase = ((size_t)tb * Np + (tn - 1)) * D;
   float v[VPL][4];
   float s = 0.0f;
 #pragma unroll
   for (int i = 0; i < VPL; ++i) {
     const int c = (i * 64 + lane) * 4;
     if (c < D) {
-      const float4 a = *reinterpret_cast<const float4*>(x_in + base + c);
-      v[i][0] = a.x; v[i][1] = a.y; v[i][2] = a.z; v[i][3] = a.w;
-      if (delta != nullptr) {
-#pragma unroll
-        for (int t = 0; t < 4; ++t) v[i][t] = dscale != nullptr ? fmaf(ds, to_f32<T>(delta[base + c + t]), v[i][t])
-                                                                     : v[i][t] + to_f32<T>(delta[base + c + t]);
+      if constexpr (ASM) {
+        const float4 a = *reinterpret_cast<const float4*>(x_in + (size_t)tn * D + c);
+        v[i][0] = a.x; v[i][1] = a.y; v[i][2] = a.z; v[i][3] = a.w;
+        if (patch) {
+#pragma unroll
+          for (int t = 0; t < 4; ++t) v[i][t] = to_f32<T>(delta[pbase + c + t]) + v[i][t];
+        }
+      } else {
+        const float4 a = *reinterpret_cast<const float4*>(x_in + base + c);
+        v[i][0] = a.x; v[i][1] = a.y; v[i][2] = a.z; v[i][3] = a.w;
+        if (delta != nullptr) {
+#pragma unroll
+          for (int t = 0; t < 4; ++t) v[i][t] = dscale != nullptr ? fmaf(ds, to_f32<T>(delta[base + c + t]), v[i][t])
+                                                                       : v[i][t] + to_f32<T>(delta[base + c + t]);
+        }
       }
       s += (v[i][0] + v[i][1]) + (v[i][2] + v[i][3]);
     } else {
@@ -60,14 +72,14 @@
   }
 }
 
-template <typename T>
+template <typename T, bool ASM = false>
 int launch_add_ln(const float* x_in, const void* delta, const float* gamma, const float* beta, float* x_out, void* y_out,
-                  int M, int D, float eps, const float* dscale, int rps, hipStream_t s) {
+                  int M, int D, float eps, const float* dscale, int rps, hipStream_t s, int N = 0, int Np = 0) {
   const int vpl = as_ceil_div(D, 256);
   dim3 grid(as_ceil_div(M, 4));
-#define AS_LN(V)                                                                                                   \
-  hipLaunchKernelGGL((add_layernorm_kernel<T, V>), grid, dim3(256), 0, s, x_in, (const T*)delta, gamma, beta, x_out, \
-                     (T*)y_out, M, D, eps, dscale, rps)
+#define AS_LN(V)                                                                                                        \
+  hipLaunchKernelGGL((add_layernorm_kernel<T, V, ASM>), grid, dim3(256), 0, s, x_in, (const T*)delta, gamma, beta, x_out, \
+                     (T*)y_out, M, D, eps, dscale, rps, N, Np)
   switch (vpl) {
     case 1: AS_LN(1); break;
     case 2: AS_LN(2); break;
@@ -313,7 +325,6 @@
   AS_REQUIRE(false, AS_E_UNSUPPORTED, "as_add_layernorm: dtype %d", dtype);
 }
 
-
 namespace {
 __global__ __launch_bounds__(256) void maxpool_nhwc_kernel(const float* __restrict__ x, float* __restrict__ out, int B, int H,
                                                            int W, int C, int k, size_t xbs) {
@@ -397,3 +408,16 @@
   AS_CHECK_LAUNCH("assemble_tokens");
   return AS_OK;
 }
+
+extern "C" int as_assemble_layernorm(const void* emb, const float* table, const float* gamma, const float* beta, float eps,
+                                     float* x_out, void* y_out, int B, int Np, int N, int D, int dtype, as_stream_t stream) {
+  AS_REQUIRE(emb && table && gamma && beta && x_out && y_out, AS_E_BADARG, "as_assemble_layernorm: null pointer");
+  AS_REQUIRE(B > 0 && Np > 0 && N > Np && (long long)B * N <= 0x7fffffffLL && D > 0 && D % 4 == 0, AS_E_BADARG,
+             "as_assemble_layernorm: B=%d Np=%d N=%d D=%d", B, Np, N, D);
+  hipStream_t s = (hipStream_t)stream;
+  if (dtype == AS_BF16)
+    return launch_add_ln<__bf16, true>(table, emb, gamma, beta, x_out, y_out, B * N, D, eps, nullptr, 1, s, N, Np);
+  if (dtype == AS_F32)
+    return launch_add_ln<float, true>(table, emb, gamma, beta, x_out, y_out, B * N, D, eps, nullptr, 1, s, N, Np);
+  AS_REQUIRE(false, AS_E_UNSUPPORTED, "as_assemble_layernorm: dtype %d", dtype);
+}
diff --git a/attentionshift_amd/csrc/linear_small.hip b/attentionshift_amd/csrc/linear_small.hip
--- a/attentionshift_amd/csrc/linear_small.hip
+++ b/attentionshift_amd/csrc/linear_small.hip
@@ -11,17 +11,22 @@
   else return v;
 }
 
-template <int ACT>
-__global__ __launch_bounds__(LS_NT) void linear_small_kernel(const float* __restrict__ x, int ldx, const float* __restrict__ W,
-                                                             const float* __restrict__ bias, float* __restrict__ out, int ldo,
-                                                             int M, int Nout, int K) {
-  __shared__ float part[4][LS_BM][LS_BN + 1];
+__device__ __forceinline__ float ls_act_rt(int act, float v) {
+  switch (act) {
+    case 1: return ls_act<1>(v);
+    case 4: return ls_act<4>(v);
+    case 5: return ls_act<5>(v);
+    default: return v;
+  }
+}
+
+__device__ __forceinline__ void ls_tile(float (*part)[LS_BM][LS_BN + 1], const float* __restrict__ pa, const float* __restrict__ W,
+                                        const float* __restrict__ bias, float* __restrict__ out, int ldo, int M, int Nout, int K,
+                                        int m0, int n0, int act) {
   const int tid = threadIdx.x, lane = tid & 63, wave = tid >> 6;
   const int li = lane & 31, half = lane >> 5;
-  const int m0 = blockIdx.x * LS_BM, n0 = blockIdx.y * LS_BN;
   const int steps = K / 16, per = steps / 4;
   const int s_beg = wave * per, s_end = wave == 3 ? steps : s_beg + per;
-  const float* pa = x + (size_t)min(m0 + li, M - 1) * ldx + 8 * half;
   const float* pb0 = W + (size_t)min(n0 + li, Nout - 1) * K + 8 * half;
   const float* pb1 = W + (size_t)min(n0 + 32 + li, Nout - 1) * K + 8 * half;
   f32x16 acc0, acc1;
@@ -50,8 +55,32 @@
     if (col >= Nout) break;
     float v = ((part[0][row][c0 + c] + part[1][row][c0 + c]) + part[2][row][c0 + c]) + part[3][row][c0 + c];
     if (bias != nullptr) v += bias[col];
-    out[(size_t)(m0 + row) * ldo + col] = ls_act<ACT>(v);
+    out[(size_t)(m0 + row) * ldo + col] = ls_act_rt(act, v);
   }
+}
+
+template <int ACT>
+__global__ __launch_bounds__(LS_NT) void linear_small_kernel(const float* __restrict__ x, int ldx, const float* __restrict__ W,
+                                                             const float* __restrict__ bias, float* __restrict__ out, int ldo,
+                                                             int M, int Nout, int K) {
+  __shared__ float part[4][LS_BM][LS_BN + 1];
+  const int lane = threadIdx.x & 63, li = lane & 31, half = lane >> 5;
+  const int m0 = blockIdx.x * LS_BM, n0 = blockIdx.y * LS_BN;
+  const float* pa = x + (size_t)min(m0 + li, M - 1) * ldx + 8 * half;
+  ls_tile(part, pa, W, bias, out, ldo, M, Nout, K, m0, n0, ACT);
+}
+
+struct LsGroups { as_linear_small_group g[2]; };
+
+__global__ __launch_bounds__(LS_NT) void linear_small_grouped_kernel(LsGroups gs, int M, int rows, int K) {
+  __shared__ float part[4][LS_BM][LS_BN + 1];
+  const as_linear_small_group& g = gs.g[blockIdx.z];
+  const int lane = threadIdx.x & 63, li = lane & 31, half = lane >> 5;
+  const int m0 = blockIdx.x * LS_BM, n0 = blockIdx.y * LS_BN;
+  if (n0 >= g.Nout) return;
+  const int m = min(m0 + li, M - 1);
+  const float* pa = g.x + (size_t)(m / rows) * g.x_batch_stride + (size_t)(m % rows) * g.ldx + 8 * half;
+  ls_tile(part, pa, g.W, g.bias, g.out, g.ldo, M, g.Nout, K, m0, n0, g.act);
 }
 
 }
@@ -75,3 +104,31 @@
   AS_CHECK_LAUNCH("linear_small");
   return AS_OK;
 }
+
+extern "C" int as_linear_small_grouped_fwd(const as_linear_small_group* groups, int ngroups, int M, int rows_per_batch, int K,
+                                           as_stream_t stream) {
+  AS_REQUIRE(groups && (ngroups == 1 || ngroups == 2), AS_E_BADARG, "as_linear_small_grouped_fwd: one or two groups");
+  AS_REQUIRE(M > 0 && rows_per_batch > 0 && M % rows_per_batch == 0 && K >= 64 && K % 16 == 0, AS_E_BADARG,
+             "as_linear_small_grouped_fwd: need M > 0 in whole batches, K %% 16 == 0, K >= 64 (M=%d rows=%d K=%d)", M,
+             rows_per_batch, K);
+  LsGroups gs;
+  int nmax = 0;
+  for (int i = 0; i < ngroups; ++i) {
+    const as_linear_small_group& g = groups[i];
+    AS_REQUIRE(g.x && g.W && g.out, AS_E_BADARG, "as_linear_small_grouped_fwd: null pointer (group %d)", i);
+    AS_REQUIRE(g.Nout > 0 && g.ldx >= K && g.ldo >= g.Nout && g.ldx % 4 == 0 && g.x_batch_stride >= 0 && g.x_batch_stride % 4 == 0,
+               AS_E_BADARG, "as_linear_small_grouped_fwd: group %d: N=%d ldx=%d ldo=%d batch stride %lld", i, g.Nout, g.ldx, g.ldo,
+               g.x_batch_stride);
+    AS_REQUIRE(g.act == 0 || g.act == 1 || g.act == 4 || g.act == 5, AS_E_BADARG,
+               "as_linear_small_grouped_fwd: act must be 0, 1 (GELU), 4 (ReLU) or 5 (sigmoid)");
+    AS_REQUIRE(((size_t)g.x % 16 == 0) && ((size_t)g.W % 16 == 0), AS_E_BADARG,
+               "as_linear_small_grouped_fwd: operands must be 16-byte aligned");
+    gs.g[i] = g;
+    nmax = g.Nout > nmax ? g.Nout : nmax;
+  }
+  if (ngroups == 1) gs.g[1] = gs.g[0];
+  const dim3 grid(as_ceil_div(M, LS_BM), as_ceil_div(nmax, LS_BN), ngroups);
+  hipLaunchKernelGGL(linear_small_grouped_kernel, grid, dim3(LS_NT), 0, (hipStream_t)stream, gs, M, rows_per_batch, K);
+  AS_CHECK_LAUNCH("linear_small_grouped");
+  return AS_OK;
+}
diff --git a/attentionshift_amd/csrc/rollout.hip b/attentionshift_amd/csrc/rollout.hip
--- a/attentionshift_amd/csrc/rollout.hip
+++ b/attentionshift_amd/csrc/rollout.hip
@@ -22,11 +22,16 @@
 template <typename T>
 __device__ __forceinline__ f32x16 pbar_tile(const T* __restrict__ q, const T* __restrict__ k,
                                             const float* __restrict__ lse, const char* kj_lds, int b, int h,
-                                            int N, int Npad, int i0, int j0, int li, int half) {
+                                            int N, int Npad, int i0, int j0, int li, int half,
+                                            const long long* __restrict__ rows = nullptr, int nrows = 0, int rbase = 0,
+                                            int rmax = 0) {
   f32x16 pbar;
 #pragma unroll
   for (int r = 0; r < 16; ++r) pbar[r] = 0.0f;
-  const int irow = min(i0 + li, N - 1);
+  auto tile_row = [&](int i) {
+    return rows == nullptr ? min(i0 + i, N - 1) : rbase + (int)min(max(rows[min(i0 + i, nrows - 1)], 0LL), (long long)rmax);
+  };
+  const int irow = tile_row(li);
   const int jrow = min(j0 + li, N - 1);
   for (int hh = 0; hh < h; ++hh) {
     const size_t bh = (size_t)b * h + hh;
@@ -46,7 +51,7 @@
     const float* lrow = lse + bh * N;
 #pragma unroll
     for (int r = 0; r < 16; ++r) {
-      const int row = min(i0 + acc_row(r, half), N - 1);
+      const int row = tile_row(acc_row(r, half));
       pbar[r] += __builtin_amdgcn_exp2f(s[r] - lrow[row] * LOG2E);
     }
   }
@@ -80,6 +85,31 @@
   }
 }
 
+template <typename T>
+__global__ __launch_bounds__(RO_NT) void rollout_top_rows_kernel(const T* __restrict__ q, const T* __restrict__ k,
+                                                                 const float* __restrict__ lse, const long long* __restrict__ rows,
+                                                                 float* __restrict__ out, size_t out_bs, T* __restrict__ rf_out,
+                                                                 int B, int N, int Npad, int h, int Tt, int G) {
+  const int lane = threadIdx.x & 63, wave = threadIdx.x >> 6;
+  const int li = lane & 31, half = lane >> 5;
+  const int jb = blockIdx.x * 4 + wave, ib = blockIdx.y, b = blockIdx.z;
+  const int j0 = jb * 32, i0 = ib * 32;
+  if (j0 >= N) return;
+  const long long* rb = rows + (size_t)b * G;
+  const f32x16 p = pbar_tile<T>(q, k, lse, nullptr, b, h, N, Npad, i0, j0, li, half, rb, G, N - Tt, Tt - 1);
+  const int j = j0 + li;
+  const int nkb = (N + 31) / 32;
+#pragma unroll
+  for (int r = 0; r < 16; ++r) {
+    const int i = i0 + acc_row(r, half);
+    const int row = N - Tt + (int)min(max(rb[min(i, G - 1)], 0LL), (long long)(Tt - 1));
+    const float v = 0.5f * (p[r] + (row == j ? 1.0f : 0.0f));
+    const bool live = i < G && j < N;
+    if (live) out[(size_t)b * out_bs + (size_t)i * N + j] = v;
+    if (rf_out != nullptr && i < 128) rf_out[rf_slot(b, nkb, i, j)] = from_f32<T>(live ? v : 0.0f);
+  }
+}
+
 template <typename T> struct Kj2 {
   static constexpr int PITCH = sizeof(T) == 2 ? 128 : (HD * 4 + 16);
   __device__ static __forceinline__ int off(int row, int elem) {
@@ -94,7 +124,7 @@
                                                               const float* __restrict__ Rin, const T* __restrict__ rf_in,
                                                               float* __restrict__ Rout, T* __restrict__ rf_out,
                                                               float* __restrict__ part, int B, int N, int Npad, int h,
-                                                              int Trows, int nsplit, int xbufs) {
+                                                              int Trows, int nsplit, int xbufs, size_t rin_bs, size_t rout_bs) {
   extern __shared__ __attribute__((aligned(16))) char smem[];
   constexpr bool PREFETCH = sizeof(T) == 2;
   const int tid = threadIdx.x, lane = tid & 63, wave = tid >> 6;
@@ -222,9 +252,9 @@
       }
       float v = 0.0f;
       if (live) {
-        const size_t idx = ((size_t)b * Trows + i) * N + j;
-        v = 0.5f * (acc[r] + Rin[idx]);
-        Rout[idx] = v;
+        const size_t idx = (size_t)i * N + j;
+        v = 0.5f * (acc[r] + Rin[b * rin_bs + idx]);
+        Rout[b * rout_bs + idx] = v;
       }
       if (rf_out != nullptr) rf_out[rf_slot(b, nkb, i, j)] = from_f32<T>(v);
     }
@@ -263,7 +293,7 @@
                                                                  const float* __restrict__ Rin, const T* __restrict__ rf_in,
                                                                  float* __restrict__ Rout, T* __restrict__ rf_out,
                                                                  float* __restrict__ part, int B, int N, int Npad, int h,
-                                                                 int Trows, int nsplit) {
+                                                                 int Trows, int nsplit, size_t rin_bs, size_t rout_bs) {
   extern __shared__ __attribute__((aligned(16))) char smem[];
   const int tid = threadIdx.x, lane = tid & 63, wave = tid >> 6;
   const int li = lane & 31, half = lane >> 5;
@@ -386,9 +416,9 @@
       }
       float v = 0.0f;
       if (live) {
-        const size_t idx = ((size_t)b * Trows + i) * N + j;
-        v = 0.5f * (mine[r] + Rin[idx]);
-        Rout[idx] = v;
+        const size_t idx = (size_t)i * N + j;
+        v = 0.5f * (mine[r] + Rin[b * rin_bs + idx]);
+        Rout[b * rout_bs + idx] = v;
       }
       if (rf_out != nullptr) rf_out[rf_slot(b, nkb, i, j)] = from_f32<T>(v);
     }
@@ -605,7 +635,7 @@
 template <typename T>
 __global__ __launch_bounds__(64) void rollout_finish_kernel(const float* __restrict__ part, const float* __restrict__ Rin,
                                                             float* __restrict__ Rout, T* __restrict__ rf_out, int B, int N,
-                                                            int Trows, int nsplit) {
+                                                            int Trows, int nsplit, size_t rin_bs, size_t rout_bs) {
   const int nkb = (N + 31) / 32;
   const int j = blockIdx.x * 64 + threadIdx.x, i = blockIdx.y, b = blockIdx.z;
   if (j >= nkb * 32) return;
@@ -614,15 +644,17 @@
     const size_t idx = ((size_t)b * Trows + i) * N + j;
     float a = 0.0f;
     for (int sp = 0; sp < nsplit; ++sp) a += part[(size_t)sp * B * Trows * N + idx];
-    v = 0.5f * (a + Rin[idx]);
-    Rout[idx] = v;
+    const size_t ij = (size_t)i * N + j;
+    v = 0.5f * (a + Rin[b * rin_bs + ij]);
+    Rout[b * rout_bs + ij] = v;
   }
   if (rf_out != nullptr) rf_out[rf_slot(b, nkb, i, j)] = from_f32<T>(v);
 }
 
 template <typename T>
 int launch_rollout_step2(const void* q, const void* k, const float* lse, const float* Rin, const void* rf_in, float* Rout,
-                         void* rf_out, float* part, int nsplit, int B, int N, int h, int Trows, hipStream_t s) {
+                         void* rf_out, float* part, int nsplit, int B, int N, int h, int Trows, size_t rin_bs, size_t rout_bs,
+                         hipStream_t s) {
   const int Npad = as_round_up(N, 64);
   const int hpw = as_ceil_div(h, 4);
   dim3 grid(as_ceil_div(N, 32), B, nsplit);
@@ -634,7 +666,7 @@
   do {                                                                                                         \
     as_lds_optin<rollout_step2_kernel<T, HPW>>(lds);                                                           \
     hipLaunchKernelGGL((rollout_step2_kernel<T, HPW>), grid, dim3(RO_NT), lds, s, (const T*)q, (const T*)k, lse, Rin, \
-                       (const T*)rf_in, Rout, (T*)rf_out, part, B, N, Npad, h, Trows, nsplit, xbufs);          \
+                       (const T*)rf_in, Rout, (T*)rf_out, part, B, N, Npad, h, Trows, nsplit, xbufs, rin_bs, rout_bs); \
   } while (0)
   if (sizeof(T) == 2 && h % R4_HPG == 0 && part != nullptr && nsplit == R4_MAXPARTS && !rollout_force_v3()) {
     const int ng = h / R4_HPG;
@@ -652,7 +684,7 @@
     AS_CHECK_LAUNCH("rollout_step4");
     dim3 fg(as_ceil_div(as_ceil_div(N, 32) * 32, 64), as_round_up(Trows, 32), B);
     hipLaunchKernelGGL((rollout_finish_kernel<T>), fg, dim3(64), 0, s, (const float*)part, Rin, Rout, (T*)rf_out, B, N,
-                       Trows, ks * ng);
+                       Trows, ks * ng, rin_bs, rout_bs);
     AS_CHECK_LAUNCH("rollout_finish");
     return AS_OK;
   }
@@ -660,7 +692,7 @@
     const size_t lds3 = (size_t)h * 32 * Kj2<T>::PITCH;
     as_lds_optin<rollout_step3_kernel<T>>(lds3);
     hipLaunchKernelGGL((rollout_step3_kernel<T>), grid, dim3(RO_NT), lds3, s, (const T*)q, (const T*)k, lse, Rin,
-                       (const T*)rf_in, Rout, (T*)rf_out, part, B, N, Npad, h, Trows, nsplit);
+                       (const T*)rf_in, Rout, (T*)rf_out, part, B, N, Npad, h, Trows, nsplit, rin_bs, rout_bs);
   } else {
   switch (hpw) {
     case 1: AS_RO2(1); break;
@@ -675,7 +707,7 @@
   if (nsplit > 1) {
     dim3 fg(as_ceil_div(as_ceil_div(N, 32) * 32, 64), as_round_up(Trows, 32), B);
     hipLaunchKernelGGL((rollout_finish_kernel<T>), fg, dim3(64), 0, s, (const float*)part, Rin, Rout, (T*)rf_out, B, N,
-                       Trows, nsplit);
+                       Trows, nsplit, rin_bs, rout_bs);
     AS_CHECK_LAUNCH("rollout_finish");
   }
   return AS_OK;
@@ -764,18 +796,53 @@
 extern "C" int as_rollout_step(const void* q, const void* k, const float* lse, const float* R_in, const void* rf_in,
                                float* R_out, void* rf_out, void* workspace, size_t workspace_bytes, int B, int N, int h,
                                int T, int dtype, as_stream_t stream) {
+  return as_rollout_step_strided(q, k, lse, R_in, (long long)T * N, rf_in, R_out, (long long)T * N, rf_out, workspace,
+                                 workspace_bytes, B, N, h, T, dtype, stream);
+}
+
+extern "C" int as_rollout_step_strided(const void* q, const void* k, const float* lse, const float* R_in,
+                                       long long r_in_batch_stride, const void* rf_in, float* R_out,
+                                       long long r_out_batch_stride, void* rf_out, void* workspace, size_t workspace_bytes,
+                                       int B, int N, int h, int T, int dtype, as_stream_t stream) {
   AS_REQUIRE(q && k && lse && R_in && rf_in && R_out && R_in != R_out && rf_in != rf_out, AS_E_BADARG,
              "as_rollout_step: null/aliased pointer");
   AS_REQUIRE(B > 0 && h > 0 && h <= 16 && T > 0 && T <= N && T <= 128, AS_E_BADARG,
              "as_rollout_step: bad sizes N=%d T=%d h=%d", N, T, h);
+  AS_REQUIRE(r_in_batch_stride >= (long long)T * N && r_out_batch_stride >= (long long)T * N, AS_E_BADARG,
+             "as_rollout_step: batch strides %lld / %lld (elements) must be >= T * N", r_in_batch_stride, r_out_batch_stride);
   hipStream_t s = (hipStream_t)stream;
   const size_t need = as_rollout_step_workspace_bytes(B, N, T);
   const bool have_ws = workspace != nullptr && workspace_bytes >= need && need > 0;
   const bool stream4 = have_ws && dtype == AS_BF16 && h % R4_HPG == 0 && !rollout_force_v3();
   const int ns = stream4 ? R4_MAXPARTS : (have_ws ? rollout_nsplit(B, N) : 1);
   float* part = ns > 1 ? (float*)workspace : nullptr;
+  const size_t ibs = (size_t)r_in_batch_stride, obs = (size_t)r_out_batch_stride;
   if (dtype == AS_BF16)
-    return launch_rollout_step2<__bf16>(q, k, lse, R_in, rf_in, R_out, rf_out, part, ns, B, N, h, T, s);
-  if (dtype == AS_F32) return launch_rollout_step2<float>(q, k, lse, R_in, rf_in, R_out, rf_out, part, ns, B, N, h, T, s);
+    return launch_rollout_step2<__bf16>(q, k, lse, R_in, rf_in, R_out, rf_out, part, ns, B, N, h, T, ibs, obs, s);
+  if (dtype == AS_F32)
+    return launch_rollout_step2<float>(q, k, lse, R_in, rf_in, R_out, rf_out, part, ns, B, N, h, T, ibs, obs, s);
   AS_REQUIRE(false, AS_E_UNSUPPORTED, "as_rollout_step: dtype %d", dtype);
 }
+
+extern "C" int as_rollout_top_rows(const void* q, const void* k, const float* lse, const long long* rows, float* R_out,
+                                   long long r_out_batch_stride, void* rf_out, int B, int N, int h, int T, int G, int dtype,
+                                   as_stream_t stream) {
+  AS_REQUIRE(q && k && lse && rows && R_out, AS_E_BADARG, "as_rollout_top_rows: null pointer");
+  AS_REQUIRE(B > 0 && h > 0 && T > 0 && T <= N && T <= 128 && G > 0 && G <= 128, AS_E_BADARG,
+             "as_rollout_top_rows: bad sizes N=%d T=%d G=%d", N, T, G);
+  AS_REQUIRE(r_out_batch_stride >= (long long)G * N, AS_E_BADARG,
+             "as_rollout_top_rows: batch stride %lld (elements) must be >= G * N", r_out_batch_stride);
+  const int Npad = as_round_up(N, 64);
+  dim3 grid(as_ceil_div(as_ceil_div(N, 32), 4), as_ceil_div(G, 32), B);
+  hipStream_t s = (hipStream_t)stream;
+  if (dtype == AS_BF16)
+    hipLaunchKernelGGL(rollout_top_rows_kernel<__bf16>, grid, dim3(RO_NT), 0, s, (const __bf16*)q, (const __bf16*)k, lse, rows, R_out,
+                       (size_t)r_out_batch_stride, (__bf16*)rf_out, B, N, Npad, h, T, G);
+  else if (dtype == AS_F32)
+    hipLaunchKernelGGL(rollout_top_rows_kernel<float>, grid, dim3(RO_NT), 0, s, (const float*)q, (const float*)k, lse, rows, R_out,
+                       (size_t)r_out_batch_stride, (float*)rf_out, B, N, Npad, h, T, G);
+  else
+    AS_REQUIRE(false, AS_E_UNSUPPORTED, "as_rollout_top_rows: dtype %d", dtype);
+  AS_CHECK_LAUNCH("rollout_top_rows");
+  return AS_OK;
+}
diff --git a/attentionshift_amd/ops.py b/attentionshift_amd/ops.py
--- a/attentionshift_amd/ops.py
+++ b/attentionshift_amd/ops.py
@@ -153,6 +153,33 @@
     _lib.check(lib.as_linear_small_fwd(_p(x), x.stride(0), _p(weight), _p(bias), _p(out), out.stride(0), M, Nout, K, code, _stream()),
                "as_linear_small_fwd")
     return out
+
+
+def linear_small_grouped(xs, weights, biases, acts):
+    lib = _lib.load()
+    n = len(xs)
+    if n not in (1, 2) or not (len(weights) == len(biases) == len(acts) == n):
+        raise AttnShiftError("linear_small_grouped: one or two groups, one weight / bias / act each")
+    K = xs[0].shape[-1]
+    B, T = (xs[0].shape[0], xs[0].shape[1]) if xs[0].dim() == 3 else (1, xs[0].shape[0])
+    M = B * T
+    arr = (_lib.LinearSmallGroup * n)()
+    outs = []
+    for i, (x, w, b, act) in enumerate(zip(xs, weights, biases, acts)):
+        shape = (B, T, K) if x.dim() == 3 else (M, K)
+        if tuple(x.shape) != shape or x.dtype != torch.float32 or not x.is_cuda or x.stride(-1) != 1:
+            raise AttnShiftError("linear_small_grouped: every x fp32 on the device, the same rows and K, unit column stride")
+        if w.dtype != torch.float32 or w.dim() != 2 or w.shape[1] != K or not w.is_contiguous():
+            raise AttnShiftError("linear_small_grouped: weight [Nout, K] fp32 contiguous")
+        if b is not None:
+            _chk(b, dtype=torch.float32)
+        out = torch.empty(M, w.shape[0], device=x.device, dtype=torch.float32)
+        outs.append(out)
+        bs = x.stride(0) if (x.dim() == 3 and B > 1) else 0
+        arr[i] = _lib.LinearSmallGroup(_p(x), _p(w), _p(b), _p(out), int(bs), int(x.stride(-2)), out.stride(0), w.shape[0],
+                                       {"none": 0, "gelu": 1, "relu": 4, "sigmoid": 5}[act])
+    _lib.check(lib.as_linear_small_grouped_fwd(ctypes.addressof(arr), n, M, T, K, _stream()), "as_linear_small_grouped_fwd")
+    return outs
 
 
 def linear_small_applies(x, weight):
@@ -285,6 +312,20 @@
     x = torch.empty(B, N, D, device=emb.device, dtype=torch.float32)
     _lib.check(lib.as_assemble_tokens(_p(emb), _p(table), _p(x), B, Np, N, D, _dt(emb), _stream()), "as_assemble_tokens")
     return x
+
+
+def assemble_layernorm(emb, table, gamma, beta, eps):
+    lib = _lib.load()
+    emb = emb.contiguous()
+    _chk(emb)
+    _chk(table, gamma, beta, dtype=torch.float32)
+    B, Np, D = emb.shape
+    N = table.shape[0]
+    x = torch.empty(B, N, D, device=emb.device, dtype=torch.float32)
+    y = torch.empty(B, N, D, device=emb.device, dtype=emb.dtype)
+    _lib.check(lib.as_assemble_layernorm(_p(emb), _p(table), _p(gamma), _p(beta), float(eps), _p(x), _p(y), B, Np, N, D, _dt(emb),
+                                         _stream()), "as_assemble_layernorm")
+    return x, y
 
 
 def maxpool_nhwc(x_nhwc, k):
@@ -486,12 +527,32 @@
     return out
 
 
-def rollout_rows(states, num_point_tokens, rows=None, use_workspace=True):
+def rollout_rows(states, num_point_tokens, rows=None, use_workspace=True, fused=None):
     lib = _lib.load()
     top = states[-1]
     T = int(num_point_tokens)
     dev, dt = top.q.device, _dt(top.q)
     nbytes = lib.as_rollout_rfrag_bytes(top.B, top.N, dt)
+    if rows is not None and ("rollout" in _lib.CHAIN_FUSE if fused is None else fused):
+        rows = rows.contiguous()
+        _chk(rows, dtype=torch.int64)
+        B, N, G, Lc = top.B, top.N, rows.shape[1], len(states)
+        if rows.shape != (B, G) or not 0 < G <= 128:
+            raise AttnShiftError("rollout_rows: rows must be [B, G] with 0 < G <= 128")
+        out = torch.empty(B, Lc, G, N, device=dev, dtype=torch.float32)
+        bs, esz = Lc * G * N, out.element_size()
+        rf = torch.empty(nbytes, device=dev, dtype=torch.uint8) if Lc > 1 else None
+        _lib.check(lib.as_rollout_top_rows(_p(top.q), _p(top.k), _p(top.lse), _p(rows), _p(out), bs, _p(rf), B, N, top.h, T, G, dt,
+                                           _stream()), "as_rollout_top_rows")
+        wbytes = lib.as_rollout_step_workspace_bytes(B, N, G) if (Lc > 1 and use_workspace) else 0
+        ws = torch.empty(wbytes, device=dev, dtype=torch.uint8) if wbytes else None
+        for n, st in enumerate(reversed(states[:-1])):
+            rfn = torch.empty_like(rf) if n + 2 < Lc else None
+            _lib.check(lib.as_rollout_step_strided(_p(st.q), _p(st.k), _p(st.lse), _p(out) + n * G * N * esz, bs, _p(rf),
+                                                   _p(out) + (n + 1) * G * N * esz, bs, _p(rfn), _p(ws), wbytes, st.B, st.N, st.h,
+                                                   G, dt, _stream()), "as_rollout_step_strided")
+            rf = rfn
+        return out
     outs = []
     R = torch.empty(top.B, T, top.N, device=dev, dtype=torch.float32)
     lower = list(reversed(states[:-1]))
diff --git a/include/attnshift.h b/include/attnshift.h
--- a/include/attnshift.h
+++ b/include/attnshift.h
@@ -34,6 +34,17 @@
 int as_linear_small_fwd(const float* x, int ldx, const float* W, const float* bias, float* out, int ldo, int M, int Nout, int K,
                         int act, as_stream_t stream);
 
+typedef struct {
+  const float* x;
+  const float* W;
+  const float* bias;
+  float* out;
+  long long x_batch_stride;
+  int ldx, ldo, Nout, act;
+} as_linear_small_group;
+int as_linear_small_grouped_fwd(const as_linear_small_group* groups, int ngroups, int M, int rows_per_batch, int K,
+                                as_stream_t stream);
+
 size_t as_linear_sk_workspace_bytes(int M, int Nout, int K);
 int as_linear_sk_fwd(const void* x, const void* W, const float* bias, void* out, int M, int Nout, int K, int dtype, int act,
                      void* ws, size_t ws_bytes, as_stream_t stream);
@@ -93,6 +104,8 @@
 
 int as_assemble_tokens(const void* emb, const float* table, float* out, int B, int Np, int N, int D, int dtype,
                        as_stream_t stream);
+int as_assemble_layernorm(const void* emb, const float* table, const float* gamma, const float* beta, float eps,
+                          float* x_out, void* y_out, int B, int Np, int N, int D, int dtype, as_stream_t stream);
 
 size_t as_add_layernorm_bwd_workspace_bytes(int M, int D);
 int as_add_layernorm_bwd(const float* x, const void* dy, const float* dx_res, const float* gamma, float eps, float* dx_out,
@@ -119,6 +132,12 @@
 int as_rollout_step(const void* q, const void* k, const float* lse, const float* R_in, const void* rf_in,
                     float* R_out, void* rf_out, void* workspace, size_t workspace_bytes, int B, int N, int h, int T,
                     int dtype, as_stream_t stream);
+int as_rollout_top_rows(const void* q, const void* k, const float* lse, const long long* rows, float* R_out,
+                        long long r_out_batch_stride, void* rf_out, int B, int N, int h, int T, int G, int dtype,
+                        as_stream_t stream);
+int as_rollout_step_strided(const void* q, const void* k, const float* lse, const float* R_in, long long r_in_batch_stride,
+                            const void* rf_in, float* R_out, long long r_out_batch_stride, void* rf_out, void* workspace,
+                            size_t workspace_bytes, int B, int N, int h, int T, int dtype, as_stream_t stream);
 
 
 int as_ccl_2d(const uint8_t* img , int32_t* labels , int M, int H, int W,
```

Measured after the change: 323.3, median of 2. About the same (+0.4%).
